# OATML-Markslab/ProteinGym

Measured on AMD Instinct MI355X. Metric: mutants scored/sec (ESM-1v 650M masked-marginal), higher is better.
Workload: dtype f16x3 (fp32 operands split into 2 fp16 planes, 3 fp16 MFMAs per product, fp32 accumulate)

## Files before the change

### proteingym_amd/csrc/api_esm.hip

```cpp
#include "model.h"

namespace pgmi {

int create_esm(pgmi_model* m, const pgmi_config* cfg, const float* w, int64_t n_weights) {
    const size_t D = cfg->embed_dim, F = cfg->ffn_dim, V = cfg->vocab, dh = m->dh, Da = m->Da;
    BlobCursor c(m, w, n_weights);
    c.upload(&m->embed_tokens, V * D);
    if (cfg->arch == PGMI_ARCH_ESM1B) c.upload(&m->embed_positions, (size_t)(cfg->max_positions + 2) * D);
    if (cfg->emb_layer_norm_before) {
        c.upload(&m->lnb_w, D);
        c.upload(&m->lnb_b, D);
    }
    auto slot = [&](size_t col) -> size_t { return rotate_half_slot(col, dh); };
    const float qscale = 1.0f / sqrtf((float)dh);
    m->layers.resize(cfg->layers);
    std::vector<float> wq(3 * Da * D, 0.0f), bq(3 * Da, 0.0f), wo_r(D * Da, 0.0f);
    for (int l = 0; l < cfg->layers; ++l) {
        Layer& L = m->layers[l];
        c.upload(&L.ln1_w, D);
        c.upload(&L.ln1_b, D);
        pack_qkv_slots(c.take(3 * (D * D + D)), D, Da, slot, qscale, wq.data(), bq.data());
        c.linear(&L.wqkv, &L.wqkv16, wq.data(), wq.size(), D);
        c.upload(&L.bqkv, bq.data(), bq.size());
        pack_out_cols(c.take(D * D), D, Da, slot, wo_r.data());
        c.linear(&L.wo, &L.wo16, wo_r.data(), wo_r.size(), Da);
        c.upload(&L.bo, D);
        c.upload(&L.ln2_w, D);
        c.upload(&L.ln2_b, D);
        c.linear(&L.w1, &L.w116, F * D, D);
        c.upload(&L.b1, F);
        c.linear(&L.w2, &L.w216, D * F, F);
        c.upload(&L.b2, D);
    }
    c.upload(&m->lna_w, D);
    c.upload(&m->lna_b, D);
    c.linear(&m->hd_w, &m->hd16, D * D, D);
    c.upload(&m->hd_b, D);
    c.upload(&m->hln_w, D);
    c.upload(&m->hln_b, D);
    c.upload(&m->head_b, V);
    m->head_w = m->embed_tokens;
    return c.finish();
}

int ensure_rotary(pgmi_model* m, int T) {
    if ((m->cfg.arch != PGMI_ARCH_ESM2 && m->cfg.arch != PGMI_ARCH_ESMC) || T <= m->rot_len) return PGMI_OK;
    return upload_rotate_half(m, std::max(T, 1026));
}

int upload_rotate_half(pgmi_model* m, int n) {
    const int rh = m->rot_halves;
    float inv[64];
    const int half = m->dh / 2;
    for (int i = 0; i < half; ++i) inv[i] = 1.0f / powf(10000.0f, (float)(2 * i) / (float)m->dh);
    return upload_rotary(m, n, rh, [&](int t, int g, int i) {
        const int j = (rh == 1) ? i : 32 * g + i;
        return j < half ? (float)t * inv[j] : 0.0f;
    });
}

int run_encoder(pgmi_model* m, int B, int T, const int32_t* keep, int n_keep, bool* compacted) {
    const pgmi_config& c = m->cfg;
    const int M = B * T, D = c.embed_dim, F = c.ffn_dim, N1 = m->fc1_cols, H = c.heads, Da = m->Da;
    hipStream_t s = m->stream;
    if (c.arch == PGMI_ARCH_ESM1B && T > c.max_positions) {
        set_error("Sequence length %d above maximum sequence length of %d", T, c.max_positions);
        return PGMI_EINVAL;
    }
    int rc = ensure_rotary(m, T);
    if (!rc) rc = reset_pad_keys(m, B, T);
    if (rc) return rc;
    {
        ProfScope p(m, PGMI_K_EMBED, 0, (double)M * D * 4);
        launch_seq_stats(m->tokens, B, T, m->embed_gather ? 0 : c.token_dropout, m->denom, m->pos_idx, m->kv_len, s);
        if (m->embed_gather) launch_gather_rows(m->embed_tokens, m->tokens, M, D, m->x, s);
        else launch_embed(m->tokens, m->denom, m->pos_idx, m->embed_tokens, m->embed_positions, c.token_dropout, M, T, D, m->x, s);
        if (m->lnb_w) {
            launch_layernorm(m->x, m->lnb_w, m->lnb_b, M, D, 1e-5f, m->x, s);
            launch_zero_pad_rows(m->tokens, M, D, m->x, s);
        }
    }
    const double ln_bytes = 2.0 * M * D * 4;
    const int prec = c.precision;
    const int mode16 = (prec == PGMI_PREC_F16X3) ? 1 : 2;
    for (int l = 0; l < c.layers; ++l) {
        const Layer& L = m->layers[l];
        { ProfScope p(m, PGMI_K_LAYERNORM, 0, ln_bytes);
          if (prec == PGMI_PREC_FP32) launch_layernorm(m->x, L.ln1_w, L.ln1_b, M, D, 1e-5f, m->h, s);
          else launch_layernorm16(m->x, L.ln1_w, L.ln1_b, M, D, 1e-5f, m->h16, m->h16_plane, mode16, s); }
        const bool fused_qkv = prec != PGMI_PREC_FP32 && !L.q_ln;
        { ProfScope p(m, PGMI_K_GEMM_QKV, 2.0 * M * 3 * D * D, 0);
          if (fused_qkv)
              rc = launch_gemm16_qkv(m->h16, m->h16_plane, L.wqkv16.p, L.wqkv16.plane, L.bqkv, M, Da, D, L.wqkv16.out_scale,
                                     m->qk16, m->qk16_plane, m->vt16, m->vt16_plane, m->rot_cos, m->rot_sin,
                                     c.arch == PGMI_ARCH_ESM2, T, m->Hs, m->gemm_variant, s, m->rot_halves, prec == PGMI_PREC_BF16);
          else
              rc = linear(m, m->h, m->h16, m->h16_plane, L.wqkv, L.wqkv16, L.bqkv, nullptr, m->qkv, nullptr, 0, M, 3 * Da, D, EPI_NONE);
          if (rc) return rc; }
        { ProfScope p(m, PGMI_K_ATTENTION, 4.0 * M * T * D, L.q_ln ? (double)M * D * 20 : 0);
          if (L.q_ln && (rc = launch_qkln_prep(m->qkv, L.q_ln, L.k_ln, 1e-5f, m->rot_cos, m->rot_sin, B, T, H, m->qk16, m->qk16_plane,
                                               m->vt16, m->vt16_plane, s)))
              return rc;
          const bool v2 = prec != PGMI_PREC_FP32;
          if (c.arch == PGMI_ARCH_ESM2 && !v2) launch_rotary(m->qkv, m->rot_cos, m->rot_sin, M, T, m->Hs, s, m->rot_halves);
          if (prec == PGMI_PREC_F16X3)
              rc = launch_attention_f16x3_v2(nullptr, m->kv_len, m->rot_cos, m->rot_sin, c.arch == PGMI_ARCH_ESM2, B, T, H,
                                             m->qk16, m->qk16_plane, m->vt16, m->vt16_plane, nullptr, m->h16,
                                             m->h16_plane, 1, s, nullptr, nullptr, m->rot_halves * kHeadDim);
          else if (v2)
              rc = launch_attention_f16x3_v2(nullptr, m->kv_len, m->rot_cos, m->rot_sin, c.arch == PGMI_ARCH_ESM2, B, T, H,
                                             m->qk16, m->qk16_plane, m->vt16, m->vt16_plane, nullptr, m->h16, m->h16_plane, 2, s, nullptr, nullptr,
                                             m->rot_halves * kHeadDim);
          else
              rc = launch_attention_f32(m->qkv, m->kv_len, B, T, H, m->h, m->h16, m->h16_plane,
                                        prec == PGMI_PREC_FP32 ? 0 : mode16, s, m->rot_halves * kHeadDim);
          if (rc) return rc; }
        if (keep && m->keep_rows && l == c.layers - 1) {
            const int R = n_keep;
            ProfScope p(m, PGMI_K_KEPT_ROWS, 2.0 * R * D * (Da + N1 + F), 0);
            launch_gather_rows(m->x, keep, R, D, m->qkv, s);
            if (prec == PGMI_PREC_FP32) launch_gather_rows(m->h, keep, R, Da, m->g, s);
            else
                launch_gather_rows(reinterpret_cast<const float*>(m->h16), keep, R, prec == PGMI_PREC_F16X3 ? Da : Da / 2,
                                   reinterpret_cast<float*>(m->g16), s);
            rc = linear(m, m->g, m->g16, m->g16_plane, L.wo, L.wo16, L.bo, m->qkv, m->x, nullptr, 0, R, D, Da, EPI_NONE);
            if (rc) return rc;
            if (prec == PGMI_PREC_FP32) launch_layernorm(m->x, L.ln2_w, L.ln2_b, R, D, 1e-5f, m->h, s);
            else launch_layernorm16(m->x, L.ln2_w, L.ln2_b, R, D, 1e-5f, m->h16, m->h16_plane, mode16, s);
            rc = linear(m, m->h, m->h16, m->h16_plane, L.w1, L.w116, L.b1, nullptr,
                        prec == PGMI_PREC_FP32 ? m->g : nullptr, prec == PGMI_PREC_FP32 ? nullptr : m->g16, m->g16_plane,
                        R, N1, D, m->fc1_epi);
            if (rc) return rc;
            rc = linear(m, m->g, m->g16, m->g16_plane, L.w2, L.w216, L.b2, m->x, m->x, nullptr, 0, R, D, F, EPI_NONE);
            if (rc) return rc;
            if (compacted) *compacted = true;
            break;
        }
        { ProfScope p(m, PGMI_K_GEMM_OUT, 2.0 * M * D * D, 0);
          rc = linear(m, m->h, m->h16, m->h16_plane, L.wo, L.wo16, L.bo, m->x, m->x, nullptr, 0, M, D, Da, EPI_NONE);
          if (rc) return rc; }
        { ProfScope p(m, PGMI_K_LAYERNORM, 0, ln_bytes);
          if (prec == PGMI_PREC_FP32) launch_layernorm(m->x, L.ln2_w, L.ln2_b, M, D, 1e-5f, m->h, s);
          else launch_layernorm16(m->x, L.ln2_w, L.ln2_b, M, D, 1e-5f, m->h16, m->h16_plane, mode16, s); }
        { ProfScope p(m, PGMI_K_GEMM_FC1, 2.0 * M * N1 * D, 0);
          rc = linear(m, m->h, m->h16, m->h16_plane, L.w1, L.w116, L.b1, nullptr,
                      prec == PGMI_PREC_FP32 ? m->g : nullptr, prec == PGMI_PREC_FP32 ? nullptr : m->g16, m->g16_plane,
                      M, N1, D, m->fc1_epi);
          if (rc) return rc; }
        { ProfScope p(m, PGMI_K_GEMM_FC2, 2.0 * M * F * D, 0);
          rc = linear(m, m->g, m->g16, m->g16_plane, L.w2, L.w216, L.b2, m->x, m->x, nullptr, 0, M, D, F, EPI_NONE);
          if (rc) return rc; }
    }
    PGMI_HIP(hipGetLastError());
    return PGMI_OK;
}

int run_head(pgmi_model* m, int R, const int32_t* row_idx) {
    const pgmi_config& c = m->cfg;
    const int D = c.embed_dim;
    hipStream_t s = m->stream;
    ProfScope p(m, PGMI_K_HEAD, 2.0 * R * D * (D + c.vocab), 0);
    const int prec = c.precision;
    const float* src = m->x;
    if (row_idx) {
        launch_gather_rows(m->x, row_idx, R, D, m->h, s);
        src = m->h;
    }
    if (prec == PGMI_PREC_FP32) launch_layernorm(src, m->lna_w, m->lna_b, R, D, 1e-5f, m->h, s);
    else launch_layernorm16(src, m->lna_w, m->lna_b, R, D, 1e-5f, m->h16, m->h16_plane, prec == PGMI_PREC_F16X3 ? 1 : 2, s);
    int rc = linear(m, m->h, m->h16, m->h16_plane, m->hd_w, m->hd16, m->hd_b, nullptr, m->g, nullptr, 0, R, D, D, EPI_GELU);
    if (rc) return rc;
    launch_layernorm(m->g, m->hln_w, m->hln_b, R, D, 1e-5f, m->g, s);
    launch_vocab_logsoftmax(m->g, m->head_w, m->head_b, R, D, c.vocab, m->lp, m->nonfinite, s);
    PGMI_HIP(hipGetLastError());
    return PGMI_OK;
}


int run_rows(pgmi_model* m, int B, int T, int R, const int32_t* row_idx) {
    bool compacted = false;
    int rc = run_encoder(m, B, T, row_idx, R, &compacted);
    if (rc) return rc;
    return run_head(m, R, compacted ? nullptr : row_idx);
}

}

extern "C" {

int pgmi_token_logprobs(pgmi_model* m, const int32_t* tokens, int B, int T, float* out) {
    if (!m || !tokens || !out || B <= 0 || T <= 0) { set_error("bad argument"); return PGMI_EINVAL; }
    if (T + 31 > m->max_rows) { set_error("T=%d exceeds workspace rows %d", T, m->max_rows); return PGMI_EINVAL; }
    int rc = check_tokens(tokens, B, T);
    if (rc) return rc;
    PGMI_HIP(hipSetDevice(m->device));
    const int V = m->cfg.vocab;
    rc = for_each_chunk(m, B, T, [&](int b0, int bc) {
        PGMI_HIP(hipMemcpyAsync(m->tokens, tokens + (size_t)b0 * T, (size_t)bc * T * 4, hipMemcpyHostToDevice, m->stream));
        int rc = run_rows(m, bc, T, bc * T, nullptr);
        if (rc) return rc;
        PGMI_HIP(hipMemcpyAsync(out + (size_t)b0 * T * V, m->lp, (size_t)bc * T * V * 4, hipMemcpyDeviceToHost, m->stream));
        return PGMI_OK;
    });
    return rc ? rc : check_nonfinite(m);
}

int pgmi_masked_logprobs(pgmi_model* m, const int32_t* tokens, const int32_t* mask_pos, int B, int T, float* out) {
    if (!m || !tokens || !mask_pos || !out || B <= 0 || T <= 0) { set_error("bad argument"); return PGMI_EINVAL; }
    if (m->cfg.arch == PGMI_ARCH_ESMC && T + 31 > m->max_rows) { set_error("T=%d exceeds workspace rows %d", T, m->max_rows); return PGMI_EINVAL; }
    if (T > m->max_rows) { set_error("T=%d exceeds workspace rows %d", T, m->max_rows); return PGMI_EINVAL; }
    int rc = check_tokens(tokens, B, T);
    if (rc) return rc;
    for (int b = 0; b < B; ++b)
        if (mask_pos[b] < 0 || mask_pos[b] >= T) { set_error("mask_pos[%d]=%d out of range", b, mask_pos[b]); return PGMI_EINVAL; }
    PGMI_HIP(hipSetDevice(m->device));
    const int V = m->cfg.vocab;
    std::vector<int32_t> ridx;
    rc = for_each_chunk(m, B, T, [&](int b0, int bc) {
        ridx.resize(bc);
        for (int b = 0; b < bc; ++b) ridx[b] = b * T + mask_pos[b0 + b];
        PGMI_HIP(hipMemcpyAsync(m->tokens, tokens + (size_t)b0 * T, (size_t)bc * T * 4, hipMemcpyHostToDevice, m->stream));
        PGMI_HIP(hipMemcpyAsync(m->aux_i, mask_pos + b0, (size_t)bc * 4, hipMemcpyHostToDevice, m->stream));
        PGMI_HIP(hipMemcpyAsync(m->row_idx, ridx.data(), (size_t)bc * 4, hipMemcpyHostToDevice, m->stream));
        launch_apply_mask(m->tokens, m->aux_i, bc, T, m->stream);
        int rc = run_rows(m, bc, T, bc, m->row_idx);
        if (rc) return rc;
        PGMI_HIP(hipMemcpyAsync(out + (size_t)b0 * V, m->lp, (size_t)bc * V * 4, hipMemcpyDeviceToHost, m->stream));
        return PGMI_OK;
    });
    return rc ? rc : check_nonfinite(m);
}

int pgmi_assay_create(pgmi_model* m, const int32_t* wt_tokens, int n_tok, const int32_t* positions, int P,
                      int window, const int32_t* sub_pos, const int32_t* sub_wt, const int32_t* sub_mt,
                      const int64_t* mut_off, int64_t n_mut, pgmi_assay** out) {
    if (!out) { set_error("null out"); return PGMI_EINVAL; }
    *out = nullptr;
    if (!m || !wt_tokens || n_tok <= 0 || P < 0 || (P > 0 && !positions) || window <= 0 || n_mut < 0) { set_error("bad argument"); return PGMI_EINVAL; }
    if (m->cfg.arch == PGMI_ARCH_ESMC) { set_error("ESM C assays run through pgmi_masked_logprobs (their window rule is not pgmi_optimal_window)"); return PGMI_EINVAL; }
    for (int i = 0; i < n_tok; ++i)
        if (wt_tokens[i] < 0 || wt_tokens[i] >= PGMI_VOCAB || wt_tokens[i] == PGMI_TOK_PAD) { set_error("wt token %d invalid at %d", wt_tokens[i], i); return PGMI_EINVAL; }
    const int T = std::min(n_tok, window);
    if (T > m->max_rows) { set_error("T=%d exceeds workspace rows %d", T, m->max_rows); return PGMI_EINVAL; }
    std::vector<int32_t> ws(P), mr(P);
    for (int i = 0; i < P; ++i) {
        if (positions[i] < 0 || positions[i] >= n_tok) { set_error("position %d out of range", positions[i]); return PGMI_EINVAL; }
        int s, e;
        pgmi_optimal_window(positions[i], n_tok, window, &s, &e);
        if (e - s != T) { set_error("internal: window length %d != %d", e - s, T); return PGMI_EINVAL; }
        ws[i] = s;
        mr[i] = positions[i] - s;
    }
    const int64_t n_sub = n_mut ? mut_off[n_mut] : 0;
    for (int64_t k = 0; k < n_sub; ++k)
        if (sub_pos[k] < 0 || sub_pos[k] >= n_tok || sub_wt[k] < 0 || sub_wt[k] >= PGMI_VOCAB || sub_mt[k] < 0 || sub_mt[k] >= PGMI_VOCAB) {
            set_error("substitution %lld out of range", (long long)k);
            return PGMI_EINVAL;
        }
    PGMI_HIP(hipSetDevice(m->device));
    pgmi_assay* a = new pgmi_assay();
    a->m = m; a->n_tok = n_tok; a->P = P; a->T = T; a->n_mut = n_mut; a->n_sub = n_sub;
    int rc = dev_upload(a->allocs, &a->wt, wt_tokens, (size_t)n_tok);
    if (!rc) rc = dev_upload(a->allocs, &a->positions, positions, (size_t)P);
    if (!rc) rc = dev_upload(a->allocs, &a->win_start, ws.data(), (size_t)P);
    if (!rc) rc = dev_upload(a->allocs, &a->mask_rel, mr.data(), (size_t)P);
    if (!rc) rc = dev_upload(a->allocs, &a->sub_pos, sub_pos, (size_t)n_sub);
    if (!rc) rc = dev_upload(a->allocs, &a->sub_wt, sub_wt, (size_t)n_sub);
    if (!rc) rc = dev_upload(a->allocs, &a->sub_mt, sub_mt, (size_t)n_sub);
    if (!rc) rc = dev_upload(a->allocs, &a->mut_off, mut_off, (size_t)(n_mut + 1));
    if (!rc) rc = dev_alloc(a->allocs, &a->table, (size_t)n_tok * PGMI_VOCAB);
    if (!rc) rc = dev_alloc(a->allocs, &a->scores, (size_t)n_mut);
    if (rc) { pgmi_assay_destroy(a); return rc; }
    m->assays.push_back(a);
    *out = a;
    return PGMI_OK;
}

void pgmi_assay_destroy(pgmi_assay* a) {
    if (!a) return;
    if (a->m) {
        hipSetDevice(a->m->device);
        hipStreamSynchronize(a->m->stream);
        auto& v = a->m->assays;
        v.erase(std::remove(v.begin(), v.end(), a), v.end());
    }
    for (void* p : a->allocs) hipFree(p);
    delete a;
}

int pgmi_assay_run(pgmi_model* m, pgmi_assay* a, double* scores_host, float* table_host, double* scores_dev) {
    if (!m || !a || a->m != m) { set_error("bad model/assay handle (assay belongs to another or a destroyed model)"); return PGMI_EINVAL; }
    PGMI_HIP(hipSetDevice(m->device));
    hipStream_t s = m->stream;
    const int T = a->T, V = m->cfg.vocab;
    const int per = rows_per_chunk(m, T);
    launch_fill_f32(a->table, (int64_t)a->n_tok * V, NAN, s);
    for (int p0 = 0; p0 < a->P; p0 += per) {
        const int bc = std::min(per, a->P - p0);
        launch_make_masked_windows(a->wt, a->win_start + p0, a->mask_rel + p0, bc, T, m->tokens, s);
        launch_row_index(a->mask_rel + p0, bc, T, m->row_idx, s);
        int rc = run_rows(m, bc, T, bc, m->row_idx);
        if (rc) return rc;
        launch_scatter_rows(m->lp, a->positions + p0, bc, V, a->table, s);
    }
    {
        ProfScope p(m, PGMI_K_SCORE, 0, (double)a->n_sub * 20);
        launch_score_mutants(a->table, V, a->sub_pos, a->sub_wt, a->sub_mt, a->mut_off, a->n_mut, a->scores, s);
    }
    PGMI_HIP(hipGetLastError());
    if (scores_dev && a->n_mut) PGMI_HIP(hipMemcpyAsync(scores_dev, a->scores, (size_t)a->n_mut * 8, hipMemcpyDeviceToDevice, s));
    if (scores_host && a->n_mut) PGMI_HIP(hipMemcpyAsync(scores_host, a->scores, (size_t)a->n_mut * 8, hipMemcpyDeviceToHost, s));
    if (table_host) PGMI_HIP(hipMemcpyAsync(table_host, a->table, (size_t)a->n_tok * V * 4, hipMemcpyDeviceToHost, s));
    PGMI_HIP(hipStreamSynchronize(s));
    return check_nonfinite(m);
}

int pgmi_pppl_create(pgmi_model* m, const uint8_t* tokens, const int64_t* seq_off, int64_t n_seq, pgmi_pppl** out) {
    if (!out) { set_error("null out"); return PGMI_EINVAL; }
    *out = nullptr;
    if (!m || !tokens || !seq_off || n_seq <= 0 || n_seq > 0x7fffffff) { set_error("bad argument"); return PGMI_EINVAL; }
    if (m->cfg.arch != PGMI_ARCH_ESM1B && m->cfg.arch != PGMI_ARCH_ESM2) { set_error("pseudo-ppl needs an ESM-1b/1v/ESM2 model"); return PGMI_EINVAL; }
    if (seq_off[0] != 0) { set_error("seq_off[0] must be 0"); return PGMI_EINVAL; }
    for (int64_t n = 0; n < n_seq; ++n) {
        const int64_t len = seq_off[n + 1] - seq_off[n];
        if (len < 2 || len > (1 << 24)) { set_error("sequence %lld has %lld tokens", (long long)n, (long long)len); return PGMI_EINVAL; }
        const uint8_t* t = tokens + seq_off[n];
        for (int64_t i = 0; i < len; ++i)
            if (t[i] >= PGMI_VOCAB || t[i] == PGMI_TOK_PAD) { set_error("token id %d invalid at sequence %lld, position %lld", (int)t[i], (long long)n, (long long)i); return PGMI_EINVAL; }
    }
    PGMI_HIP(hipSetDevice(m->device));
    pgmi_pppl* q = new pgmi_pppl();
    q->m = m;
    q->N = n_seq;
    q->off.assign(seq_off, seq_off + n_seq + 1);
    int rc = dev_upload(q->allocs, &q->tok8, tokens, (size_t)seq_off[n_seq]);
    if (!rc) rc = dev_upload(q->allocs, &q->off_dev, seq_off, (size_t)n_seq + 1);
    if (rc) { for (void* p : q->allocs) hipFree(p); delete q; return rc; }
    m->pppls.push_back(q);
    *out = q;
    return PGMI_OK;
}

void pgmi_pppl_destroy(pgmi_pppl* q) {
    if (!q) return;
    if (q->m) {
        hipSetDevice(q->m->device);
        hipStreamSynchronize(q->m->stream);
        auto& v = q->m->pppls;
        v.erase(std::remove(v.begin(), v.end(), q), v.end());
    }
    for (void* p : q->allocs) hipFree(p);
    delete q;
}

int64_t pgmi_pppl_rows(const pgmi_pppl* q, int64_t first, int64_t count) {
    if (!q || first < 0 || count < 0 || first + count > q->N) return -1;
    int64_t r = 0;
    for (int64_t n = first; n < first + count; ++n) r += std::max<int64_t>(0, q->off[n + 1] - q->off[n] - 4);
    return r;
}

int pgmi_pppl_run(pgmi_model* m, pgmi_pppl* q, int64_t first, int64_t count, double* scores_host, float* terms_host,
                  double* scores_dev) {
    if (!m || !q || q->m != m) { set_error("bad model/library handle (library belongs to another or a destroyed model)"); return PGMI_EINVAL; }
    if (first < 0 || count <= 0 || first + count > q->N) { set_error("sequence range [%lld, %lld) outside the library of %lld", (long long)first, (long long)(first + count), (long long)q->N); return PGMI_EINVAL; }
    PGMI_HIP(hipSetDevice(m->device));
    hipStream_t s = m->stream;
    const int J = (int)count, V = m->cfg.vocab;
    std::vector<int32_t> sid(J);
    for (int j = 0; j < J; ++j) sid[j] = (int32_t)(first + j);
    auto len_of = [&](int32_t n) { return q->off[n + 1] - q->off[n]; };
    std::stable_sort(sid.begin(), sid.end(), [&](int32_t a, int32_t b) { return len_of(a) > len_of(b); });
    std::vector<int64_t> rp((size_t)J + 1);
    rp[0] = 0;
    for (int j = 0; j < J; ++j) rp[j + 1] = rp[j] + std::max<int64_t>(0, len_of(sid[j]) - 4);
    const int64_t R = rp[J];
    const int64_t Tmax = len_of(sid[0]);
    if (R > 0 && Tmax + 31 > m->max_rows) { set_error("T=%lld exceeds workspace rows %d", (long long)Tmax, m->max_rows); return PGMI_EINVAL; }
    if (R > 0 && m->cfg.arch == PGMI_ARCH_ESM1B && Tmax > m->cfg.max_positions) {
        set_error("Sequence length %lld above maximum sequence length of %d", (long long)Tmax, m->cfg.max_positions);
        return PGMI_EINVAL;
    }
    std::vector<void*> pool;
    auto cleanup = [&]() { for (void* p : pool) hipFree(p); };
    int32_t* d_sid = nullptr;
    int64_t* d_rp = nullptr;
    float* d_terms = nullptr;
    double* d_out = nullptr;
    int rc = dev_upload(pool, &d_sid, sid.data(), (size_t)J);
    if (!rc) rc = dev_upload(pool, &d_rp, rp.data(), (size_t)J + 1);
    if (!rc) rc = dev_alloc(pool, &d_terms, (size_t)R);
    if (!rc) rc = dev_alloc(pool, &d_out, (size_t)J);
    if (rc) { cleanup(); return rc; }
    q->last_rows = R; q->last_chunks = 0; q->last_tokens = 0; q->last_padded = 0;
    int j0 = 0;
    for (int64_t g0 = 0; g0 < R;) {
        while (rp[j0 + 1] <= g0) ++j0;
        const int T = (int)len_of(sid[j0]);
        const int bc = (int)std::min<int64_t>(rows_per_chunk(m, T), R - g0);
        launch_make_pppl_rows(q->tok8, q->off_dev, d_sid, d_rp, J, g0, bc, T, m->tokens, m->row_idx, m->aux_i, s);
        rc = run_rows(m, bc, T, bc, m->row_idx);
        if (rc) { hipStreamSynchronize(s); cleanup(); return rc; }
        launch_pppl_pick(m->lp, m->aux_i, bc, V, d_terms + g0, s);
        q->last_chunks += 1;
        q->last_padded += (int64_t)bc * T;
        g0 += bc;
        if ((q->last_chunks & 63) == 0 && g0 < R && (rc = check_nonfinite(m)) != PGMI_OK) { cleanup(); return rc; }
    }
    for (int j = 0; j < J; ++j) q->last_tokens += (rp[j + 1] - rp[j]) * len_of(sid[j]);
    {
        ProfScope p(m, PGMI_K_SCORE, 0, (double)R * 4);
        launch_pppl_sum(d_terms, d_rp, d_sid, J, first, d_out, s);
    }
    hipError_t e = hipGetLastError();
    if (e == hipSuccess && scores_dev) e = hipMemcpyAsync(scores_dev, d_out, (size_t)J * 8, hipMemcpyDeviceToDevice, s);
    if (e == hipSuccess && scores_host) e = hipMemcpyAsync(scores_host, d_out, (size_t)J * 8, hipMemcpyDeviceToHost, s);
    std::vector<float> sorted_terms;
    if (e == hipSuccess && terms_host && R > 0) {
        sorted_terms.resize((size_t)R);
        e = hipMemcpyAsync(sorted_terms.data(), d_terms, (size_t)R * 4, hipMemcpyDeviceToHost, s);
    }
    if (e == hipSuccess) e = hipStreamSynchronize(s);
    cleanup();
    if (e != hipSuccess) { set_error("pseudo-ppl run failed: %s", hipGetErrorString(e)); return PGMI_EHIP; }
    if (terms_host && R > 0) {
        std::vector<int64_t> dst((size_t)J + 1, 0);
        for (int k = 0; k < J; ++k) dst[k + 1] = dst[k] + std::max<int64_t>(0, len_of((int32_t)(first + k)) - 4);
        for (int j = 0; j < J; ++j)
            std::copy(sorted_terms.begin() + rp[j], sorted_terms.begin() + rp[j + 1], terms_host + dst[sid[j] - first]);
    }
    return check_nonfinite(m);
}

int pgmi_pppl_stats(const pgmi_pppl* q, int64_t* rows, int64_t* chunks, int64_t* tokens, int64_t* padded_tokens) {
    if (!q) { set_error("null library"); return PGMI_EINVAL; }
    if (rows) *rows = q->last_rows;
    if (chunks) *chunks = q->last_chunks;
    if (tokens) *tokens = q->last_tokens;
    if (padded_tokens) *padded_tokens = q->last_padded;
    return PGMI_OK;
}

}
```

### proteingym_amd/csrc/api_model.hip

```cpp
#include "model.h"

namespace pgmi {

static thread_local char g_err[1024] = "";
void set_error(const char* fmt, ...) {
    va_list ap;
    va_start(ap, fmt);
    vsnprintf(g_err, sizeof(g_err), fmt, ap);
    va_end(ap);
}

int prof_drain(pgmi_model* m) {
    if (m->events_used == 0) return PGMI_OK;
    PGMI_HIP(hipStreamSynchronize(m->stream));
    for (size_t i = 0; i < m->events_used; ++i) {
        float ms = 0.f;
        PGMI_HIP(hipEventElapsedTime(&ms, m->events[i].start, m->events[i].stop));
        m->prof_ms[m->events[i].cls] += ms;
    }
    m->events_used = 0;
    return PGMI_OK;
}

int check_cfg(const pgmi_config* c) {
// ... 121 lines not shown
        set_error("non-finite log-probabilities: an activation left the fp16/bf16 range in precision mode %d; "
                  "re-run with precision fp32", m->cfg.precision);
        return PGMI_EOVERFLOW;
    }
    return PGMI_OK;
}

int reset_pad_keys(pgmi_model* m, int B, int T) {
    if (!m->vt16 || (B == m->last_B && T == m->last_T)) return PGMI_OK;
    PGMI_HIP(hipMemsetAsync(m->vt16, 0, m->vt16_plane * 2 * sizeof(unsigned short), m->stream));
    m->last_B = B;
    m->last_T = T;
    return PGMI_OK;
}

}

extern "C" {

int pgmi_abi_version(void) { return PGMI_ABI_VERSION; }

const char* pgmi_last_error(void) { return g_err; }

int pgmi_device_count(void) {
    int n = 0;
    if (hipGetDeviceCount(&n) != hipSuccess) return 0;
    return n;
}

int64_t pgmi_weight_count(const pgmi_config* c) {
    if (!c || c->layers <= 0 || c->embed_dim <= 0 || c->ffn_dim <= 0) return -1;
    const int64_t D = c->embed_dim, F = c->ffn_dim, V = c->vocab;
    if (c->arch == PGMI_ARCH_TRANCEPTION) {
        const int64_t conv = 3 * ((64 * 3 + 64) + (64 * 5 + 64) + (64 * 7 + 64));
        return V * D + (int64_t)c->layers * (2 * D + (D * 3 * D + 3 * D) + conv + (D * D + D) + 2 * D + (D * F + F) + (F * D + D)) + 2 * D + V * D;
    }
    if (c->arch == PGMI_ARCH_PROGEN2)
        return V * D + (int64_t)c->layers * (2 * D + 3 * D * D + D * D + (F * D + F) + (D * F + D)) + 2 * D + V * D + V;
    if (c->arch == PGMI_ARCH_GPT) return -1;
    if (c->arch == PGMI_ARCH_ESMC) return esmc_weight_count(c);
    if (c->arch == PGMI_ARCH_MSA) {
        const int64_t attn = 2 * D + 4 * (D * D + D);
        return V * D + (int64_t)(c->max_positions + 2) * D + 1024 * D + 2 * D +
               (int64_t)c->layers * (2 * attn + 2 * D + (F * D + F) + (D * F + D)) + 2 * D + (D * D + D) + 2 * D + V;
    }
    int64_t n = V * D;
    if (c->arch == PGMI_ARCH_ESM1B) n += (int64_t)(c->max_positions + 2) * D;
    if (c->emb_layer_norm_before) n += 2 * D;
    n += (int64_t)c->layers * (2 * D + 4 * (D * D + D) + 2 * D + (F * D + F) + (D * F + D));
    n += 2 * D + (D * D + D) + 2 * D + V;
    return n;
}

int pgmi_model_create(const pgmi_config* cfg, const float* w, int64_t n_weights, int device, pgmi_model** out) {
    if (cfg && cfg->arch == PGMI_ARCH_PROGEN2) {
        if (out) *out = nullptr;
        set_error("ProGen2 models are created with pgmi_pg2_model_create (it takes rotary_dim)");
        return PGMI_EINVAL;
    }
    if (cfg && cfg->arch == PGMI_ARCH_GPT) {
        if (out) *out = nullptr;
        set_error("causal decoder models are created with pgmi_gpt_model_create (it takes pos_kind)");
        return PGMI_EINVAL;
    }
    return model_create(cfg, w, n_weights, device, out, 0);
}

}

namespace pgmi {

static int alloc_workspace(pgmi_model* m) {
    const pgmi_config& c = m->cfg;
    const size_t R = m->max_rows, D = c.embed_dim, F = c.ffn_dim, V = c.vocab, Da = m->Da;
    const size_t Dw = std::max(D, Da);
    const bool f32mode = c.precision == PGMI_PREC_FP32;
    int rc = PGMI_OK;
    auto alloc = [&](auto** p, size_t n) { if (!rc) rc = dev_alloc(m->allocs, p, n); };
    alloc(&m->x, R * D);
    alloc(&m->h, R * Dw);
    alloc(&m->qkv, R * 3 * Da);
    alloc(&m->g, R * (f32mode ? std::max(F, D) : D));
    if (!f32mode) {
        const size_t planes = c.precision == PGMI_PREC_F16X3 ? 2 : 1;
        m->h16_plane = R * Dw;
        m->g16_plane = R * F;
        alloc(&m->h16, m->h16_plane * planes);
        alloc(&m->g16, m->g16_plane * planes);
    }
    alloc(&m->nonfinite, (size_t)1);
    if (!f32mode) {
        m->qk16_plane = R * 2 * Da;
        m->vt16_plane = R * Da;
        alloc(&m->qk16, m->qk16_plane * 2);
        alloc(&m->vt16, m->vt16_plane * 2);
    }
    if (c.arch == PGMI_ARCH_MSA) {
        alloc(&m->xt, R * D);
        alloc(&m->msa_kv_len, (size_t)2048);
    }
    alloc(&m->lp, (c.arch == PGMI_ARCH_GPT && V > kWave ? (size_t)m->gpt_head_rows : R) * V);
    alloc(&m->denom, R);
    alloc(&m->tokens, R);
    alloc(&m->pos_idx, R);
    alloc(&m->kv_len, R);
    alloc(&m->row_idx, R);
    alloc(&m->aux_i, R);
    if (rc) return rc;
    PGMI_HIP(hipMemset(m->nonfinite, 0, 4));
    if (m->vt16) PGMI_HIP(hipMemset(m->vt16, 0, m->vt16_plane * 2 * sizeof(unsigned short)));
    return PGMI_OK;
}

int model_create(const pgmi_config* cfg, const float* w, int64_t n_weights, int device, pgmi_model** out, int arch_arg) {
    if (!out) { set_error("null out"); return PGMI_EINVAL; }
    *out = nullptr;
    int rc = check_cfg(cfg);
    if (rc) return rc;
    const int64_t need = cfg->arch == PGMI_ARCH_GPT ? gpt_weight_count(cfg, arch_arg) : pgmi_weight_count(cfg);
    if (need < 0) { set_error("causal decoder pos_kind %d: must be PGMI_GPT_POS_ROTARY or PGMI_GPT_POS_LEARNED", arch_arg); return PGMI_EINVAL; }
    if (!w || n_weights != need) {
        set_error("weight blob has %lld elements, config needs %lld", (long long)n_weights, (long long)need);
        return PGMI_EINVAL;
    }
    const int ndev = pgmi_device_count();
    if (ndev <= 0) { set_error("no HIP device visible (libpgmi has no CPU fallback)"); return PGMI_ENODEV; }
    if (device < 0 || device >= ndev) { set_error("device %d out of range (%d visible)", device, ndev); return PGMI_EINVAL; }
    PGMI_HIP(hipSetDevice(device));
    pgmi_model* m = new pgmi_model();
    m->cfg = *cfg;
    m->device = device;
    if (hipStreamCreateWithFlags(&m->stream, hipStreamNonBlocking) != hipSuccess) { set_error("hipStreamCreate failed"); delete m; return PGMI_EHIP; }
    m->dh = cfg->embed_dim / cfg->heads;
    m->rot_halves = m->dh > 2 * kHeadDim ? 4 : m->dh > kHeadDim ? 2 : 1;
    m->Hs = cfg->heads * m->rot_halves;
    m->Da = m->Hs * kHeadDim;
    m->ln_eps = cfg->ln_eps > 0.f ? cfg->ln_eps : 1e-5f;
    m->max_rows = std::max(cfg->max_rows > 0 ? cfg->max_rows : 98304, 2048);
    const size_t V = cfg->vocab;
    const std::vector<float> zeros(std::max({3 * (size_t)m->Da, (V + 63) / 64 * 64, (size_t)cfg->embed_dim, V, (size_t)cfg->heads}), 0.0f);
    rc = dev_upload(m->allocs, &m->zeros, zeros.data(), zeros.size());
    m->fc1_cols = cfg->ffn_dim;
    if (!rc) switch (cfg->arch) {
        case PGMI_ARCH_TRANCEPTION: rc = create_tranception(m, cfg, w, n_weights); break;
        case PGMI_ARCH_MSA: rc = create_msa(m, cfg, w, n_weights); break;
        case PGMI_ARCH_PROGEN2: rc = create_progen2(m, cfg, w, n_weights, arch_arg); break;
        case PGMI_ARCH_GPT: rc = create_gpt(m, cfg, w, n_weights, arch_arg); break;
        case PGMI_ARCH_ESMC: rc = create_esmc(m, cfg, w, n_weights); break;
        default: rc = create_esm(m, cfg, w, n_weights);
    }
    if (!rc) rc = alloc_workspace(m);
    if (rc) { pgmi_model_destroy(m); return rc; }
    m->keep_rows = env_int("PGMI_KEEP_ROWS", 1);
    gemm_options_from_env();
    m->gemm_variant = env_int("PGMI_GEMM_VARIANT", 0);
    *out = m;
    return PGMI_OK;
}

}

extern "C" {

void pgmi_model_destroy(pgmi_model* m) {
    if (!m) return;
    hipSetDevice(m->device);
    if (m->stream) hipStreamSynchronize(m->stream);
    for (pgmi_assay* a : m->assays) {
        for (void* p : a->allocs) hipFree(p);
        a->allocs.clear();
        a->m = nullptr;
    }
    m->assays.clear();
    for (pgmi_pppl* q : m->pppls) {
        for (void* p : q->allocs) hipFree(p);
        q->allocs.clear();
        q->m = nullptr;
    }
    m->pppls.clear();
    for (auto& e : m->events) { hipEventDestroy(e.start); hipEventDestroy(e.stop); }
    for (void* p : m->allocs) hipFree(p);
    if (m->stream) hipStreamDestroy(m->stream);
    delete m;
}

int pgmi_model_device(const pgmi_model* m) { return m ? m->device : -1; }

int pgmi_set_option(const char* name, int64_t value) {
    if (!name) { set_error("null option name"); return PGMI_EINVAL; }
    int rc = gemm_set_option(name, (long long)value);
    if (rc) rc = att_set_option(name, (long long)value);
    if (rc) set_error("unknown option '%s' (gemm_half_tail, gemm_max_rows, att_xcd_local, att_v3)", name);
    return rc;
}

int pgmi_synchronize(pgmi_model* m) {
    if (!m) { set_error("null model"); return PGMI_EINVAL; }
    PGMI_HIP(hipStreamSynchronize(m->stream));
    return PGMI_OK;
}

int pgmi_profile_enable(pgmi_model* m, int on) {
    if (!m) { set_error("null model"); return PGMI_EINVAL; }
    int rc = prof_drain(m);
    m->prof = on != 0;
    return rc;
}

int pgmi_profile_reset(pgmi_model* m) {
    if (!m) { set_error("null model"); return PGMI_EINVAL; }
    int rc = prof_drain(m);
    for (int i = 0; i < PGMI_K_COUNT; ++i) { m->prof_ms[i] = 0; m->prof_n[i] = 0; m->prof_flops[i] = 0; m->prof_bytes[i] = 0; }
    return rc;
}

int pgmi_profile_get(pgmi_model* m, int k, double* ms, int64_t* launches, double* flops, double* bytes) {
    if (!m || k < 0 || k >= PGMI_K_COUNT) { set_error("bad argument"); return PGMI_EINVAL; }
    int rc = prof_drain(m);
    if (rc) return rc;
    if (ms) *ms = m->prof_ms[k];
    if (launches) *launches = m->prof_n[k];
    if (flops) *flops = m->prof_flops[k];
    if (bytes) *bytes = m->prof_bytes[k];
    return PGMI_OK;
}

}
```

### proteingym_amd/csrc/attention_f16.hip

```cpp
#include <stdlib.h>
#include <string.h>
#include <algorithm>

#include "attention_f16_common.h"

namespace pgmi {

template <int WPB, int OUT, int NSTG, int DH = 64, bool RAG = false, int DO = DH>
__global__ __launch_bounds__(WPB * 64) void attention_f16x3_v2_kernel(
    const unsigned short* __restrict__ qk16, size_t qk_plane, const unsigned short* __restrict__ vt16,
    size_t vt_plane, const int32_t* __restrict__ kv_len, const float* __restrict__ slopes, int T, int H,
    int Tp, float* __restrict__ ctx, unsigned short* __restrict__ ctx16, size_t plane, RagMap rag, int dense_nblk, int nseq) {
    constexpr float defer_thr = kAttDefer;
    constexpr int NT = WPB * 64;
    constexpr int KCPR = DH / 8;
    constexpr int KCH = AKT * KCPR, VCH = DO * 4;
    constexpr int NSL = DH / DO;
    static_assert(NSL == 1 || (OUT == 1 && !RAG), "sliced context: split-plane output of dense launches only");
    constexpr int STG_CH = 2 * KCH + 2 * VCH;
    constexpr int NWI = STG_CH / 64;
    constexpr int NDMA = (NWI + WPB - 1) / WPB;
    constexpr int NS = DH / 16, ND = DO / 32;
    extern __shared__ __attribute__((aligned(16))) u32x4 lds[];

// ... 208 lines not shown
            }
            const float mb = m_run - 10.0f;
            typedef float f32x2 __attribute__((ext_vector_type(2)));
#pragma unroll
            for (int v = 0; v < 16; v += 2) {
                const f32x2 dlt = f32x2{st[v], st[v + 1]} - f32x2{mb, mb};
                st[v] = __builtin_amdgcn_exp2f(dlt[0]);
                st[v + 1] = __builtin_amdgcn_exp2f(dlt[1]);
            }
            l_run += ((st[0] + st[1]) + (st[2] + st[3])) + ((st[4] + st[5]) + (st[6] + st[7])) +
                     (((st[8] + st[9]) + (st[10] + st[11])) + ((st[12] + st[13]) + (st[14] + st[15])));
#pragma unroll
            for (int m = 0; m < 2; ++m) {
                u32x4 ph, pl;
#pragma unroll
                for (int e = 0; e < 4; ++e) {
                    const float p0 = st[8 * m + 2 * e], p1 = st[8 * m + 2 * e + 1];
                    typedef __fp16 fp16x2 __attribute__((ext_vector_type(2)));
                    const fp16x2 hi2 = __builtin_amdgcn_cvt_pkrtz(p0, p1);
                    typedef float f32x2 __attribute__((ext_vector_type(2)));
                    const f32x2 ps = f32x2{p0, p1} * f32x2{kLoScale, kLoScale};
                    const float l0 = fmaf((float)hi2[0], -kLoScale, ps[0]), l1 = fmaf((float)hi2[1], -kLoScale, ps[1]);
                    const fp16x2 lo2 = __builtin_amdgcn_cvt_pkrtz(l0, l1);
                    ph[e] = __builtin_bit_cast(unsigned int, hi2);
                    pl[e] = __builtin_bit_cast(unsigned int, lo2);
                }
#pragma unroll
                for (int dt = 0; dt < ND; ++dt) {
                    const int d = dt * 32 + r;
                    const int ci = d * 4 + ((2 * m + kh) ^ ((d >> 2) & 3));
                    const u32x4 vfh = Vb[ci], vfl = Vb[VCH + ci];
                    oc[dt] = mfma_h(vfh, pl, oc[dt]);
                    oc[dt] = mfma_h(vfl, ph, oc[dt]);
                    om[dt] = mfma_h(vfh, ph, om[dt]);
                }
            }
        }
        cur = (cur == NSTG - 1) ? 0 : cur + 1;
    }

    if (active) {
        const float l_tot = l_run + __shfl_xor(l_run, 32);
        if (OUT == 3) {
            store_ctx_bf16<ND>(om, oc, 1.0f / l_tot, kInvLo, q0 + r < T && q0 + r >= p0,
                               ctx16 + (size_t)(orow0 + max(min(q0 + r, T - 1), p0)) * (size_t)D + (size_t)h * DH, kh);
        } else if (OUT == 1) {
            const float inv = 1.0f / l_tot;
            const bool row_ok = q0 + r < T && q0 + r >= p0;
            unsigned short* rowp = ctx16 + (size_t)(orow0 + max(min(q0 + r, T - 1), p0)) * (size_t)(2 * D) + (size_t)((h * DH + d0) / 32) * 64;
#pragma unroll
            for (int dt = 0; dt < ND; ++dt)
#pragma unroll
                for (int gp = 0; gp < 2; ++gp) {
                    unsigned int w[2][4];
#pragma unroll
                    for (int gi = 0; gi < 2; ++gi) {
                        const int g = 2 * gp + gi;
                        _Float16 hh[4], ll[4];
#pragma unroll
                        for (int e = 0; e < 4; ++e) split_act(fmaf(oc[dt][4 * g + e], kInvLo, om[dt][4 * g + e]) * inv, hh[e], ll[e]);
                        w[gi][0] = pack_h2(hh[0], hh[1]); w[gi][1] = pack_h2(hh[2], hh[3]);
                        w[gi][2] = pack_h2(ll[0], ll[1]); w[gi][3] = pack_h2(ll[2], ll[3]);
                    }
                    unsigned int first[4], second[4];
#pragma unroll
                    for (int k = 0; k < 4; ++k) {
                        const auto sw = __builtin_amdgcn_permlane32_swap(w[0][k], w[1][k], false, false);
                        first[k] = sw[0];
                        second[k] = sw[1];
                    }
                    if (row_ok) {
                        unsigned short* dst = rowp + dt * 64 + 8 * (2 * gp + kh);
                        *reinterpret_cast<u32x4*>(dst) = u32x4{first[0], first[1], second[0], second[1]};
                        *reinterpret_cast<u32x4*>(dst + 32) = u32x4{first[2], first[3], second[2], second[3]};
                    }
                }
        } else if (q0 + r < T && q0 + r >= p0) {
            const float inv = 1.0f / l_tot;
            const size_t off = (size_t)(orow0 + q0 + r) * D + (size_t)h * DH + 4 * kh;
#pragma unroll
            for (int dt = 0; dt < ND; ++dt)
#pragma unroll
                for (int g = 0; g < 4; ++g) {
                    float val[4];
#pragma unroll
                    for (int e = 0; e < 4; ++e) val[e] = fmaf(oc[dt][4 * g + e], kInvLo, om[dt][4 * g + e]) * inv;
                    const size_t oo = off + dt * 32 + 8 * g;
                    if constexpr (OUT == 0) {
                        *reinterpret_cast<f32x4*>(ctx + oo) = f32x4{val[0], val[1], val[2], val[3]};
                    } else {
                        _Float16 hh[4], ll[4];
#pragma unroll
                        for (int e = 0; e < 4; ++e) split_act(val[e], hh[e], ll[e]);
                        unsigned short* dst = ctx16 + (size_t)(orow0 + q0 + r) * (size_t)(2 * D) + (size_t)(ND * h + dt) * 64 + 8 * g + 4 * kh;
                        *reinterpret_cast<u32x2*>(dst) = u32x2{pack_h2(hh[0], hh[1]), pack_h2(hh[2], hh[3])};
                        *reinterpret_cast<u32x2*>(dst + 32) = u32x2{pack_h2(ll[0], ll[1]), pack_h2(ll[2], ll[3])};
                    }
                }
        }
    }
}


template <int WPB, int OUT, int NSTG, int DH, bool RAG = false, int DO = DH>
static int launch_att16v2_one(dim3 grid, const unsigned short* qk16, size_t qk_plane, const unsigned short* vt16, size_t vt_plane,
                              const int32_t* kv_len, const float* slopes, int T, int H, int Tp, float* ctx, unsigned short* ctx16,
                              size_t plane, hipStream_t s, RagMap rag = RagMap{}, int dense_nblk = 0, int nseq = 0) {
    constexpr size_t lds_bytes = (size_t)NSTG * (8 * DH + 8 * DO) * 16;
    auto kfn = attention_f16x3_v2_kernel<WPB, OUT, NSTG, DH, RAG, DO>;
    if (lds_bytes > 65536) {
        hipError_t e = hipFuncSetAttribute(reinterpret_cast<const void*>(kfn), hipFuncAttributeMaxDynamicSharedMemorySize, (int)lds_bytes);
        if (e != hipSuccess) { set_error("hipFuncSetAttribute: %s", hipGetErrorString(e)); return PGMI_EHIP; }
    }
    hipLaunchKernelGGL(kfn, grid, dim3(WPB * 64), lds_bytes, s, qk16, qk_plane, vt16, vt_plane, kv_len, slopes, T, H, Tp, ctx, ctx16, plane, rag, dense_nblk, nseq);
    return PGMI_OK;
}

template <int OUT, int NSTG>
static int launch_att16v2_mode(int wpb, dim3 grid, const unsigned short* qk16, size_t qk_plane,
                               const unsigned short* vt16, size_t vt_plane, const int32_t* kv_len,
                               const float* slopes, int T, int H, int Tp, float* ctx, unsigned short* ctx16,
                               size_t plane, hipStream_t s, int dense_nblk, int nseq) {
    const RagMap none{};
    switch (wpb) {
        case 1: return launch_att16v2_one<1, OUT, NSTG, 64>(grid, qk16, qk_plane, vt16, vt_plane, kv_len, slopes, T, H, Tp, ctx, ctx16, plane, s, none, dense_nblk, nseq);
        case 2: return launch_att16v2_one<2, OUT, NSTG, 64>(grid, qk16, qk_plane, vt16, vt_plane, kv_len, slopes, T, H, Tp, ctx, ctx16, plane, s, none, dense_nblk, nseq);
        case 3: return launch_att16v2_one<3, OUT, NSTG, 64>(grid, qk16, qk_plane, vt16, vt_plane, kv_len, slopes, T, H, Tp, ctx, ctx16, plane, s, none, dense_nblk, nseq);
        default: return launch_att16v2_one<4, OUT, NSTG, 64>(grid, qk16, qk_plane, vt16, vt_plane, kv_len, slopes, T, H, Tp, ctx, ctx16, plane, s, none, dense_nblk, nseq);
    }
}

static int g_att_xcd_local = -1;
int att_set_option(const char* name, long long value) {
    if (!strcmp(name, "att_xcd_local")) { g_att_xcd_local = (int)value; return PGMI_OK; }
    if (!strcmp(name, "att_v3")) { att_v3_set_option((int)value); return PGMI_OK; }
    return PGMI_EINVAL;
}
static dim3 dense_grid(int nblk, int H, int B, int* dense_nblk) {
    if (g_att_xcd_local == 0 || (g_att_xcd_local < 0 && nblk < 2)) { *dense_nblk = 0; return dim3(nblk, H, B); }
    *dense_nblk = nblk;
    const long long pairs = (long long)H * B, groups = (pairs + 7) / 8;
    return dim3((unsigned)(groups * 8 * nblk), 1, 1);
}

int att16_waves_per_block(int T) {
    const int n32 = (T + 31) / 32, nblk = (n32 + 3) / 4;
    const int wpb = (n32 + nblk - 1) / nblk;
    return wpb == 3 ? 4 : wpb;
}

int launch_attention_f16x3_v2(const float* qkv, const int32_t* kv_len, const float* cos_t, const float* sin_t,
                              int rotary, int B, int T, int H, unsigned short* qk16, size_t qk_plane,
                              unsigned short* vt16, size_t vt_plane, float* ctx, unsigned short* ctx16, size_t plane,
                              int out_mode, hipStream_t s, const float* conv, const float* slopes, int head_dim) {
    if (B <= 0 || T <= 0 || H <= 0 || out_mode < 0 || out_mode > 2 || (head_dim != 64 && head_dim != 128 && head_dim != 256)) {
        set_error("attention_f16x3_v2: bad arguments B=%d T=%d H=%d out=%d head_dim=%d", B, T, H, out_mode, head_dim);
        return PGMI_EINVAL;
    }
    const int n32 = (T + 31) / 32, Tp = n32 * 32;
    int rc = PGMI_OK;
    {
        const unsigned long long seq_bytes = (unsigned long long)T * 2ull * (unsigned long long)H * (unsigned long long)head_dim * 2ull;
        const unsigned long long vt_bytes = (unsigned long long)head_dim * (unsigned long long)Tp * 2ull;
        if ((unsigned long long)qk_plane * 2ull + seq_bytes >= (1ull << 32) || (unsigned long long)vt_plane * 2ull + vt_bytes >= (1ull << 32)) {
            set_error("attention_f16x3_v2: operand planes of %zu / %zu halfs exceed the 32-bit offset range of the K / V^T DMA "
                      "(plane stride + one sequence must stay below 4 GiB: create the model with a smaller max_rows)", qk_plane, vt_plane);
            return PGMI_EINVAL;
        }
    }
    if (head_dim == 256) {
        if (qkv || conv || !slopes || out_mode != 1) { set_error("attention_f16x3_v2: head_dim 256 is the causal, fused-QKV, split-plane-output flavour only"); return PGMI_EINVAL; }
        const int nblk = (n32 + 3) / 4;
        int dn = 0;
        const dim3 grid = dense_grid(nblk, 2 * H, B, &dn);
        rc = launch_att16v2_one<4, 1, 2, 256, false, 128>(grid, qk16, qk_plane, vt16, vt_plane, kv_len, slopes, T, H, Tp, ctx, ctx16, plane, s, RagMap{}, dn, B);
        if (rc) return rc;
        PGMI_HIP(hipGetLastError());
        return PGMI_OK;
    }
    if (head_dim == 128) {
        if (qkv || conv) { set_error("attention_f16x3_v2: head_dim 128 needs operands from the fused QKV projection"); return PGMI_EINVAL; }
        const int nblk = (n32 + 3) / 4;
        int dn = 0;
        const dim3 grid = dense_grid(nblk, H, B, &dn);
        if (out_mode == 0) rc = launch_att16v2_one<4, 0, 3, 128>(grid, qk16, qk_plane, vt16, vt_plane, kv_len, slopes, T, H, Tp, ctx, ctx16, plane, s, RagMap{}, dn, B);
        else if (out_mode == 2) rc = launch_att16v2_one<4, 3, 3, 128>(grid, qk16, qk_plane, vt16, vt_plane, kv_len, slopes, T, H, Tp, ctx, ctx16, plane, s, RagMap{}, dn, B);
        else rc = launch_att16v2_one<4, 1, 3, 128>(grid, qk16, qk_plane, vt16, vt_plane, kv_len, slopes, T, H, Tp, ctx, ctx16, plane, s, RagMap{}, dn, B);
        if (rc) return rc;
        PGMI_HIP(hipGetLastError());
        return PGMI_OK;
    }
    if (qkv && conv && rotary) { set_error("attention_f16x3_v2: depth-wise convolution and rotary together are not a model this library knows"); return PGMI_EINVAL; }
    if (qkv && conv)
        launch_qkv_prep_conv(dim3(n32, H, B), s, qkv, conv, T, H, Tp, qk16, qk_plane, vt16, vt_plane, nullptr);
    else if (qkv)
        launch_qkv_prep(dim3(n32, H, B), s, qkv, cos_t, sin_t, rotary, T, H, Tp, qk16, qk_plane, vt16, vt_plane);
    const int wpb = att16_waves_per_block(T), nblk = (n32 + wpb - 1) / wpb;
    int dn = 0;
    const dim3 grid = dense_grid(nblk, H, B, &dn);
    if (att_v3_serves(T, conv, slopes, head_dim)) rc = launch_att16v3(out_mode, wpb, grid, qk16, qk_plane, vt16, vt_plane, kv_len, T, H, Tp, ctx, ctx16, s, dn, B);
    else if (out_mode == 0) rc = launch_att16v2_mode<0, 3>(wpb, grid, qk16, qk_plane, vt16, vt_plane, kv_len, slopes, T, H, Tp, ctx, ctx16, plane, s, dn, B);
    else if (out_mode == 2) rc = launch_att16v2_mode<3, 3>(wpb, grid, qk16, qk_plane, vt16, vt_plane, kv_len, slopes, T, H, Tp, ctx, ctx16, plane, s, dn, B);
    else rc = launch_att16v2_mode<1, 3>(wpb, grid, qk16, qk_plane, vt16, vt_plane, kv_len, slopes, T, H, Tp, ctx, ctx16, plane, s, dn, B);
    if (rc) return rc;
    PGMI_HIP(hipGetLastError());
    return PGMI_OK;
}

int launch_attention_tr_ragged(const float* qkv, const float* conv, const float* slopes, int T, int H, const AttRagged& rg,
                               unsigned short* qk16, size_t qk_plane, unsigned short* vt16, size_t vt_plane, unsigned short* ctx16,
                               size_t plane, hipStream_t s) {
    if (T <= 0 || H <= 0 || !qkv || !conv || !slopes || rg.n_tiles <= 0 || rg.n_blocks <= 0) {
        set_error("attention_tr_ragged: bad arguments T=%d H=%d tiles=%d blocks=%d", T, H, rg.n_tiles, rg.n_blocks);
        return PGMI_EINVAL;
    }
    const int Tp = (T + 31) / 32 * 32;
    {
        const unsigned long long seq_bytes = (unsigned long long)T * 2ull * (unsigned long long)H * 64ull * 2ull;
        const unsigned long long vt_bytes = 64ull * (unsigned long long)Tp * 2ull;
        if ((unsigned long long)qk_plane * 2ull + seq_bytes >= (1ull << 32) || (unsigned long long)vt_plane * 2ull + vt_bytes >= (1ull << 32)) {
            set_error("attention_tr_ragged: operand planes exceed the 32-bit offset range of the K / V^T DMA (create the model with a smaller max_rows)");
            return PGMI_EINVAL;
        }
    }
    const RagMap tiles{rg.seq_off, rg.seq_p, rg.seq_q, rg.seq_root, rg.seq_vt, rg.tile_seq, rg.tile_j};
    launch_qkv_prep_conv(dim3(rg.n_tiles, H, 1), s, qkv, conv, T, H, Tp, qk16, qk_plane, vt16, vt_plane, &tiles);
    const RagMap rag{rg.seq_off, rg.seq_p, rg.seq_q, rg.seq_root, rg.seq_vt, rg.blk_seq, rg.blk_j};
    const dim3 grid(rg.n_blocks, H, 1);
    int rc;
    switch (att16_waves_per_block(T)) {
        case 1: rc = launch_att16v2_one<1, 1, 3, 64, true>(grid, qk16, qk_plane, vt16, vt_plane, nullptr, slopes, T, H, Tp, nullptr, ctx16, plane, s, rag); break;
        case 2: rc = launch_att16v2_one<2, 1, 3, 64, true>(grid, qk16, qk_plane, vt16, vt_plane, nullptr, slopes, T, H, Tp, nullptr, ctx16, plane, s, rag); break;
        default: rc = launch_att16v2_one<4, 1, 3, 64, true>(grid, qk16, qk_plane, vt16, vt_plane, nullptr, slopes, T, H, Tp, nullptr, ctx16, plane, s, rag); break;
    }
    if (rc) return rc;
    PGMI_HIP(hipGetLastError());
    return PGMI_OK;
}

}
```

### proteingym_amd/csrc/attention_f16_common.h

```cpp
#pragma once
#include "common.h"

namespace pgmi {

typedef _Float16 h2 __attribute__((ext_vector_type(2)));
typedef _Float16 h8 __attribute__((ext_vector_type(8)));
typedef unsigned int u32x4 __attribute__((ext_vector_type(4)));
typedef unsigned int u32x2 __attribute__((ext_vector_type(2)));

constexpr int AKT = 32;
constexpr float kAttDefer = 4.0f;
constexpr int K_CH = AKT * 8;
constexpr int V_CH = 64 * 4;
constexpr int A_STAGE = 2 * K_CH + 2 * V_CH;

__device__ __forceinline__ unsigned int pack_h2(_Float16 a, _Float16 b) {
    const h2 t = {a, b};
    return __builtin_bit_cast(unsigned int, t);
}
__device__ __forceinline__ f32x16 mfma_h(u32x4 a, u32x4 b, f32x16 c) {
    return __builtin_amdgcn_mfma_f32_32x32x16_f16(__builtin_bit_cast(h8, a), __builtin_bit_cast(h8, b), c, 0, 0, 0);
}


struct RagMap {
    const int32_t* seq_off;
    const int32_t* seq_p;
    const int32_t* seq_q;
    const int32_t* seq_root;
    const uint32_t* seq_vt;
    const int32_t* ent_seq;
    const int32_t* ent_j;
};

template <int ND>
__device__ __forceinline__ void store_ctx_bf16(const f32x16 (&om)[ND], const f32x16 (&oc)[ND], float inv, float inv_lo, bool row_ok,
                                               unsigned short* row_head, int kh) {
    auto rne = [](float f) -> unsigned int {
        unsigned int u = __builtin_bit_cast(unsigned int, f);
        u += 0x7fffu + ((u >> 16) & 1u);
        return u >> 16;
    };
#pragma unroll
    for (int dt = 0; dt < ND; ++dt)
#pragma unroll
        for (int gp = 0; gp < 2; ++gp) {
            unsigned int w[2][2];
#pragma unroll
            for (int gi = 0; gi < 2; ++gi) {
                const int g = 2 * gp + gi;
                float v[4];
#pragma unroll
                for (int e = 0; e < 4; ++e) v[e] = fmaf(oc[dt][4 * g + e], inv_lo, om[dt][4 * g + e]) * inv;
                w[gi][0] = rne(v[0]) | (rne(v[1]) << 16);
                w[gi][1] = rne(v[2]) | (rne(v[3]) << 16);
            }
            unsigned int first[2], second[2];
#pragma unroll
            for (int k = 0; k < 2; ++k) {
                const auto sw = __builtin_amdgcn_permlane32_swap(w[0][k], w[1][k], false, false);
                first[k] = sw[0];
                second[k] = sw[1];
            }
            if (row_ok) *reinterpret_cast<u32x4*>(row_head + dt * 32 + 8 * (2 * gp + kh)) = u32x4{first[0], first[1], second[0], second[1]};
        }
}

void launch_qkv_prep(dim3 grid, hipStream_t s, const float* qkv, const float* cos_t, const float* sin_t, int rotary, int T, int H, int Tp,
                     unsigned short* qk16, size_t qk_plane, unsigned short* vt16, size_t vt_plane);
void launch_qkv_prep_conv(dim3 grid, hipStream_t s, const float* qkv, const float* conv, int T, int H, int Tp, unsigned short* qk16, size_t qk_plane,
                          unsigned short* vt16, size_t vt_plane, const RagMap* rag);
bool att_v3_serves(int T, const float* conv, const float* slopes, int head_dim);
void att_v3_set_option(int value);
int launch_att16v3(int out_mode, int wpb, dim3 grid, const unsigned short* qk16, size_t qk_plane, const unsigned short* vt16, size_t vt_plane,
                   const int32_t* kv_len, int T, int H, int Tp, float* ctx, unsigned short* ctx16, hipStream_t s, int dense_nblk, int nseq);

}
```

### proteingym_amd/csrc/attention_f16_prep.hip

```cpp
#include <stdlib.h>
#include <string.h>
#include <algorithm>

#include "attention_f16_common.h"

namespace pgmi {

__global__ __launch_bounds__(256) void qkv_prep_kernel(
    const float* __restrict__ qkv, const float* __restrict__ cos_t, const float* __restrict__ sin_t,
    int rotary, int T, int H, int Tp, unsigned short* __restrict__ qk16,
    size_t qk_plane, unsigned short* __restrict__ vt16, size_t vt_plane) {
    const int b = blockIdx.z, h = blockIdx.y, t0 = blockIdx.x * 32;
    const int tid = threadIdx.x;
    const int D = H * kHeadDim;
    const size_t RS = (size_t)3 * D;
#pragma unroll
    for (int it = 0; it < 2; ++it) {
        const int u = tid + 256 * it;
        const int which = u >> 8, tok = (u >> 3) & 31, c = u & 7;
        const int t = t0 + tok;
        if (t < T) {
            const float* src = qkv + ((size_t)b * T + t) * RS + (size_t)which * D + h * kHeadDim + 4 * c;
            f32x4 x1 = *reinterpret_cast<const f32x4*>(src);
            f32x4 x2 = *reinterpret_cast<const f32x4*>(src + 32);
// ... 114 lines not shown
                const f32x4 a2 = *reinterpret_cast<const f32x4*>(&raw[(tok + j) * RSTR + which * 64 + 8 * c + 4]);
#pragma unroll
                for (int e = 0; e < 4; ++e) {
                    x1[e] = fmaf(w1[e], a1[e], x1[e]);
                    x2[e] = fmaf(w2[e], a2[e], x2[e]);
                }
            }
            if (which == 0) {
#pragma unroll
                for (int e = 0; e < 4; ++e) { x1[e] *= kQLog2e; x2[e] *= kQLog2e; }
            }
            _Float16 hh[8], ll[8];
#pragma unroll
            for (int e = 0; e < 4; ++e) {
                const float v1 = x1[e], v2 = x2[e];
                split_act(v1, hh[e], ll[e]);
                split_act(v2, hh[4 + e], ll[4 + e]);
            }
            unsigned short* dst = qk16 + orow(t) * (2 * D) + (size_t)which * D + h * kHeadDim + 8 * c;
            *reinterpret_cast<u32x4*>(dst) = u32x4{pack_h2(hh[0], hh[1]), pack_h2(hh[2], hh[3]), pack_h2(hh[4], hh[5]), pack_h2(hh[6], hh[7])};
            *reinterpret_cast<u32x4*>(dst + qk_plane) = u32x4{pack_h2(ll[0], ll[1]), pack_h2(ll[2], ll[3]), pack_h2(ll[4], ll[5]), pack_h2(ll[6], ll[7])};
        }
    }
    {
        const int d = tid & 63, p = tid >> 6;
        const int k1 = 16 * (p >> 1) + 4 * (p & 1);
        _Float16 hh[8], ll[8];
        float w[8];
#pragma unroll
        for (int j = 0; j < 8; ++j) w[j] = cwl[(2 * 8 + j) * 64 + d];
#pragma unroll
        for (int e = 0; e < 8; ++e) {
            const int key = k1 + (e & 3) + 8 * (e >> 2);
            float y = w[7];
#pragma unroll
            for (int j = 0; j < 7; ++j) y = fmaf(w[j], raw[(key + j) * RSTR + 128 + d], y);
            if (t0 + key >= T) y = 0.0f;
            split_act(y, hh[e], ll[e]);
        }
        unsigned short* row = RAG ? vt16 + (size_t)seq_vt[b] + ((size_t)h * kHeadDim + d) * Tpo + (t0 - a0) + 8 * p
                                  : vt16 + (((size_t)b * H + h) * kHeadDim + d) * Tp + t0 + 8 * p;
        *reinterpret_cast<u32x4*>(row) = u32x4{pack_h2(hh[0], hh[1]), pack_h2(hh[2], hh[3]), pack_h2(hh[4], hh[5]), pack_h2(hh[6], hh[7])};
        *reinterpret_cast<u32x4*>(row + vt_plane) = u32x4{pack_h2(ll[0], ll[1]), pack_h2(ll[2], ll[3]), pack_h2(ll[4], ll[5]), pack_h2(ll[6], ll[7])};
    }
}

template <int NV>
__global__ __launch_bounds__(256) void qkln_prep_kernel(
    const float* __restrict__ qkv, const float* __restrict__ q_w, const float* __restrict__ k_w, float eps,
    const float* __restrict__ cos_t, const float* __restrict__ sin_t, int T, int H, int Tp,
    unsigned short* __restrict__ qk16, size_t qk_plane, unsigned short* __restrict__ vt16, size_t vt_plane) {
    const int b = blockIdx.y, t0 = blockIdx.x * 32;
    const int tid = threadIdx.x, lane = tid & 63, wave = tid >> 6;
    const int D = H * kHeadDim, nv = D >> 2;
    const size_t RS = (size_t)3 * D;
    for (int u = wave; u < 64; u += 4) {
        const int which = u & 1, t = t0 + (u >> 1);
        if (t >= T) break;
        const f32x4* xr = reinterpret_cast<const f32x4*>(qkv + ((size_t)b * T + t) * RS + (size_t)which * D);
        f32x4 v[NV];
        float sum = 0.f;
#pragma unroll
        for (int i = 0; i < NV; ++i) {
            const int c = lane + 64 * i;
            v[i] = (c < nv) ? xr[c] : f32x4{0.f, 0.f, 0.f, 0.f};
            sum += (v[i][0] + v[i][1]) + (v[i][2] + v[i][3]);
        }
#pragma unroll
        for (int o = 32; o > 0; o >>= 1) sum += __shfl_xor(sum, o);
        const float mean = sum / (float)D;
        float q = 0.f;
#pragma unroll
        for (int i = 0; i < NV; ++i) {
            const int c = lane + 64 * i;
            if (c < nv) {
#pragma unroll
                for (int k = 0; k < 4; ++k) {
                    const float d = v[i][k] - mean;
                    q += d * d;
                }
            }
        }
#pragma unroll
        for (int o = 32; o > 0; o >>= 1) q += __shfl_xor(q, o);
        const float rstd = 1.0f / sqrtf(q / (float)D + eps);
        const f32x4* wr = reinterpret_cast<const f32x4*>(which ? k_w : q_w);
        const int j4 = 4 * (lane & 15);
        const f32x4 cs = *reinterpret_cast<const f32x4*>(cos_t + (size_t)t * 64 + j4);
        const f32x4 sn = *reinterpret_cast<const f32x4*>(sin_t + (size_t)t * 64 + j4);
        const bool first_half = (lane & 8) == 0;
#pragma unroll
        for (int i = 0; i < NV; ++i) {
            const int c = lane + 64 * i;
            f32x4 o;
            const f32x4 wv = (c < nv) ? wr[c] : f32x4{0.f, 0.f, 0.f, 0.f};
#pragma unroll
            for (int k = 0; k < 4; ++k) o[k] = (v[i][k] - mean) * rstd * wv[k];
            f32x4 p;
#pragma unroll
            for (int k = 0; k < 4; ++k) p[k] = __shfl_xor(o[k], 8);
            if (c < nv) {
                f32x4 y;
#pragma unroll
                for (int k = 0; k < 4; ++k) y[k] = first_half ? o[k] * cs[k] + (-p[k]) * sn[k] : o[k] * cs[k] + p[k] * sn[k];
                if (which == 0) {
#pragma unroll
                    for (int k = 0; k < 4; ++k) y[k] *= kQLog2e;
                }
                _Float16 hh[4], ll[4];
#pragma unroll
                for (int k = 0; k < 4; ++k) split_act(y[k], hh[k], ll[k]);
                unsigned short* dst = qk16 + ((size_t)b * T + t) * (2 * D) + (size_t)which * D + 4 * c;
                *reinterpret_cast<u32x2*>(dst) = u32x2{pack_h2(hh[0], hh[1]), pack_h2(hh[2], hh[3])};
                *reinterpret_cast<u32x2*>(dst + qk_plane) = u32x2{pack_h2(ll[0], ll[1]), pack_h2(ll[2], ll[3])};
            }
        }
    }
    const int d = tid & 63, kq = tid >> 6;
    for (int h = 0; h < H; ++h) {
        _Float16 hh[8], ll[8];
        const float* vsrc = qkv + ((size_t)b * T) * RS + 2 * D + h * kHeadDim + d;
#pragma unroll
        for (int e = 0; e < 8; ++e) {
            const int t = t0 + 8 * kq + e;
            const float x = (t < T) ? vsrc[(size_t)t * RS] : 0.0f;
            split_act(x, hh[e], ll[e]);
        }
        unsigned short* row = vt16 + (((size_t)b * H + h) * kHeadDim + d) * Tp + t0 + 16 * (kq >> 1) + 4 * (kq & 1);
        *reinterpret_cast<u32x2*>(row) = u32x2{pack_h2(hh[0], hh[1]), pack_h2(hh[2], hh[3])};
        *reinterpret_cast<u32x2*>(row + 8) = u32x2{pack_h2(hh[4], hh[5]), pack_h2(hh[6], hh[7])};
        *reinterpret_cast<u32x2*>(row + vt_plane) = u32x2{pack_h2(ll[0], ll[1]), pack_h2(ll[2], ll[3])};
        *reinterpret_cast<u32x2*>(row + vt_plane + 8) = u32x2{pack_h2(ll[4], ll[5]), pack_h2(ll[6], ll[7])};
    }
}

int launch_qkln_prep(const float* qkv, const float* q_w, const float* k_w, float eps, const float* cos_t, const float* sin_t, int B,
                     int T, int H, unsigned short* qk16, size_t qk_plane, unsigned short* vt16, size_t vt_plane, hipStream_t s) {
    const int nv = H * kHeadDim / 4, Tp = (T + 31) / 32 * 32;
    if (B <= 0 || T <= 0 || H <= 0 || nv > 512) { set_error("qkln_prep: bad shape B=%d T=%d H=%d (D = 64 H <= 2048)", B, T, H); return PGMI_EINVAL; }
    const dim3 grid((T + 31) / 32, B);
#define PGMI_QKLN(NV_) hipLaunchKernelGGL(qkln_prep_kernel<NV_>, grid, dim3(256), 0, s, qkv, q_w, k_w, eps, cos_t, sin_t, T, H, Tp, \
                                          qk16, qk_plane, vt16, vt_plane)
    if (nv <= 64) PGMI_QKLN(1);
    else if (nv <= 128) PGMI_QKLN(2);
    else if (nv <= 192) PGMI_QKLN(3);
    else if (nv <= 256) PGMI_QKLN(4);
    else if (nv <= 320) PGMI_QKLN(5);
    else PGMI_QKLN(8);
#undef PGMI_QKLN
    PGMI_HIP(hipGetLastError());
    return PGMI_OK;
}

void launch_qkv_prep(dim3 grid, hipStream_t s, const float* qkv, const float* cos_t, const float* sin_t, int rotary, int T, int H, int Tp,
                     unsigned short* qk16, size_t qk_plane, unsigned short* vt16, size_t vt_plane) {
    hipLaunchKernelGGL(qkv_prep_kernel, grid, dim3(256), 0, s, qkv, cos_t, sin_t, rotary, T, H, Tp, qk16, qk_plane, vt16, vt_plane);
}
void launch_qkv_prep_conv(dim3 grid, hipStream_t s, const float* qkv, const float* conv, int T, int H, int Tp, unsigned short* qk16, size_t qk_plane,
                          unsigned short* vt16, size_t vt_plane, const RagMap* rag) {
    if (rag)
        hipLaunchKernelGGL(qkv_prep_conv_kernel<true>, grid, dim3(256), 0, s, qkv, conv, T, H, Tp, qk16, qk_plane, vt16, vt_plane,
                           rag->seq_off, rag->seq_p, rag->seq_q, rag->seq_root, rag->seq_vt, rag->ent_seq, rag->ent_j);
    else
        hipLaunchKernelGGL(qkv_prep_conv_kernel<false>, grid, dim3(256), 0, s, qkv, conv, T, H, Tp, qk16, qk_plane, vt16, vt_plane,
                           nullptr, nullptr, nullptr, nullptr, nullptr, nullptr, nullptr);
}

}
```

### proteingym_amd/csrc/attention_f16_v3.hip

```cpp
#include <stdlib.h>
#include <string.h>
#include <algorithm>

#include "attention_f16_common.h"

namespace pgmi {

template <int WPB, int OUT>
__global__ __launch_bounds__(WPB * 64, 2) void attention_f16x3_v3_kernel(
    const unsigned short* __restrict__ qk16, size_t qk_plane, const unsigned short* __restrict__ vt16, size_t vt_plane,
    const int32_t* __restrict__ kv_len, int T, int H, int Tp, float* __restrict__ ctx, unsigned short* __restrict__ ctx16,
    int dense_nblk, int nseq) {
    constexpr float defer_thr = kAttDefer;
    constexpr int DH = 64, NSTG = 3, KCPR = 8, KCH = AKT * KCPR, VCH = DH * 4, STG_CH = 2 * KCH + 2 * VCH;
    constexpr int NWI = STG_CH / 64, NDMA = (NWI + WPB - 1) / WPB, NS = 4, ND = 2;
    extern __shared__ __attribute__((aligned(16))) u32x4 lds[];
    int b, h, qblk;
    if (dense_nblk > 0) {
        const int within = (int)blockIdx.x % (8 * dense_nblk);
        const int pair = ((int)blockIdx.x / (8 * dense_nblk)) * 8 + (within & 7);
        if (pair >= nseq * H) return;
        qblk = within >> 3;
        b = pair / H;
        h = pair - b * H;
    } else {
        b = blockIdx.z;
        h = blockIdx.y;
        qblk = blockIdx.x;
    }
    const int tid = threadIdx.x, lane = tid & 63;
    const int wave = __builtin_amdgcn_readfirstlane(tid >> 6);
    const int r = lane & 31, kh = lane >> 5;
    const int D = H * DH;
    const int Tk = kv_len ? kv_len[b] : T;
    const int q0 = (qblk * WPB + wave) * 32;
    const bool active = q0 < T;
    const int nkt = (Tk + AKT - 1) / AKT;
    const size_t seq_halfs = (size_t)T * (2 * D), vt_halfs = (size_t)DH * Tp;
    const unsigned long long qk_bytes = std::min<unsigned long long>(0xFFFFFFFFull, (unsigned long long)qk_plane * 2ull + seq_halfs * 2ull);
    const unsigned long long vt_bytes = std::min<unsigned long long>(0xFFFFFFFFull, (unsigned long long)vt_plane * 2ull + vt_halfs * 2ull);
    const __amdgpu_buffer_rsrc_t rsQK = __builtin_amdgcn_make_buffer_rsrc(const_cast<unsigned short*>(qk16) + (size_t)b * seq_halfs, 0, (int)(unsigned int)qk_bytes, 0x00020000);
    const __amdgpu_buffer_rsrc_t rsVT = __builtin_amdgcn_make_buffer_rsrc(const_cast<unsigned short*>(vt16) + ((size_t)b * H + h) * vt_halfs, 0, (int)(unsigned int)vt_bytes, 0x00020000);

    static_assert(WPB == 1 || WPB == 2 || WPB == 4, "the DMA map needs WPB to divide 8");
    constexpr int NK = 8 / WPB;
    int kvoff[NK], krow[NK], vvoff[NDMA - NK];
#pragma unroll
    for (int i = 0; i < NK; ++i) {
        const int q4 = (wave + WPB * i) & 3;
        const int key = q4 * 8 + (lane >> 3);
        krow[i] = key;
        kvoff[i] = ((lane & 7) ^ ((key >> 1) & 7)) * 16;
    }
#pragma unroll
    for (int i = 0; i < NDMA - NK; ++i) {
        const int q4 = (wave + WPB * (i + NK)) & 3;
        const int g = q4 * 64 + lane, d = g >> 2, c = (g & 3) ^ ((d >> 2) & 3);
        vvoff[i] = d * Tp * 2 + c * 16;
    }
    auto issue_piece = [&](int i, int m, int stage, bool on) {
        u32x4* base = lds + stage * STG_CH;
        const int kk = min(m, nkt - 1), vv = min(max(m - 2, 0), nkt - 1);
        if (i < NK) {
            const int wi = wave + WPB * i, p = (WPB * i) >> 2;
            const int kr = krow[i < NK ? i : 0], ko = kvoff[i < NK ? i : 0];
            const int vo = on ? min(kk * AKT + kr, T - 1) * (2 * D) * 2 + ko : -16;
            const int so = (int)((unsigned int)p * (unsigned int)qk_plane * 2u + (unsigned int)(D + h * DH) * 2u);
            __builtin_amdgcn_raw_ptr_buffer_load_lds(rsQK, (__attribute__((address_space(3))) void*)(base + wi * 64), 16, vo, so, 0, 0);
        } else {
            const int wi = wave + WPB * i, p = (WPB * i - 8) >> 2;
            const int so = (int)((unsigned int)p * (unsigned int)vt_plane * 2u) + vv * ((AKT / 8) * 16);
            const int vv0 = vvoff[i >= NK ? i - NK : 0];
            const int vo = on ? vv0 : -16;
            __builtin_amdgcn_raw_ptr_buffer_load_lds(rsVT, (__attribute__((address_space(3))) void*)(base + wi * 64), 16, vo, so, 0, 0);
        }
    };
    auto issue_bundle = [&](int m, int stage, bool on) {
#pragma unroll
        for (int i = 0; i < NDMA; ++i) issue_piece(i, m, stage, on);
    };
    const int last_bundle = nkt + 1;

    issue_bundle(0, 0, true);
    u32x4 qh[NS], ql[NS];
    {
        u32x4* qbase = lds + STG_CH + wave * (2 * KCH);
        if (active) {
            constexpr int NQ = 2 * KCH / 64;
#pragma unroll
            for (int i = 0; i < NQ; ++i) {
                const int f = i * 64 + lane, pq = f / KCH, row = (f % KCH) / KCPR;
                const int c = (f % KCPR) ^ ((row >> 1) & 7);
                const int vo = (int)(((unsigned int)min(q0 + row, T - 1) * (unsigned int)(2 * D) + (unsigned int)(h * DH)) * 2u + (unsigned int)c * 16u);
                const int so = (int)((unsigned int)pq * (unsigned int)qk_plane * 2u);
                __builtin_amdgcn_raw_ptr_buffer_load_lds(rsQK, (__attribute__((address_space(3))) void*)(qbase + i * 64), 16, vo, so, 0, 0);
            }
        }
        asm volatile("s_waitcnt vmcnt(0)" ::: "memory");
        if (active) {
#pragma unroll
            for (int s = 0; s < NS; ++s) {
                const int ci = r * KCPR + ((2 * s + kh) ^ ((r >> 1) & 7));
                qh[s] = qbase[ci];
                ql[s] = qbase[KCH + ci];
            }
        }
        asm volatile("s_waitcnt lgkmcnt(0)" ::: "memory");
        __builtin_amdgcn_s_barrier();
        asm volatile("" ::: "memory");
    }
    issue_bundle(1, 1, true);
    issue_bundle(2, 2, true);

    f32x16 om[ND], oc[ND], sm, sc;
#pragma unroll
    for (int dt = 0; dt < ND; ++dt)
#pragma unroll
        for (int v = 0; v < 16; ++v) { om[dt][v] = 0.f; oc[dt][v] = 0.f; }
#pragma unroll
    for (int v = 0; v < 16; ++v) { sm[v] = 0.f; sc[v] = 0.f; }
    u32x4 ph[2], pl[2];
#pragma unroll
    for (int m = 0; m < 2; ++m)
#pragma unroll
        for (int e = 0; e < 4; ++e) { ph[m][e] = 0u; pl[m][e] = 0u; }
    float m_run = -INFINITY, l_run = 0.f;
    constexpr float kInvLo = 1.0f / kLoScale;
    const f32x16 zero16 = {0.f, 0.f, 0.f, 0.f, 0.f, 0.f, 0.f, 0.f, 0.f, 0.f, 0.f, 0.f, 0.f, 0.f, 0.f, 0.f};
    typedef float f32x2 __attribute__((ext_vector_type(2)));
    typedef _Float16 h4 __attribute__((ext_vector_type(4)));

    auto vfrag = [&](const u32x4* Vb, int m, u32x4 (&fh)[ND], u32x4 (&fl)[ND]) {
#pragma unroll
        for (int dt = 0; dt < ND; ++dt) {
            const int d = dt * 32 + r;
            const int ci = d * 4 + ((2 * m + kh) ^ ((d >> 2) & 3));
            fh[dt] = Vb[ci];
            fl[dt] = Vb[VCH + ci];
        }
    };
    auto kfrag = [&](const u32x4* Kb, int s, u32x4& kh_, u32x4& kl_) {
        const int ci = r * KCPR + ((2 * s + kh) ^ ((r >> 1) & 7));
        kh_ = Kb[ci];
        kl_ = Kb[KCH + ci];
    };
    auto pv = [&](int m, const u32x4 (&fh)[ND], const u32x4 (&fl)[ND]) {
#pragma unroll
        for (int dt = 0; dt < ND; ++dt) {
            oc[dt] = mfma_h(fh[dt], pl[m], oc[dt]);
            oc[dt] = mfma_h(fl[dt], ph[m], oc[dt]);
            om[dt] = mfma_h(fh[dt], ph[m], om[dt]);
        }
    };
    auto split_p = [&](const float (&st)[16], int m, int e) {
        const float p0 = st[8 * m + 2 * e], p1 = st[8 * m + 2 * e + 1];
        typedef __fp16 fp16x2 __attribute__((ext_vector_type(2)));
        const fp16x2 hi2 = __builtin_amdgcn_cvt_pkrtz(p0, p1);
        const f32x2 ps = f32x2{p0, p1} * f32x2{kLoScale, kLoScale};
        const float l0 = fmaf((float)hi2[0], -kLoScale, ps[0]), l1 = fmaf((float)hi2[1], -kLoScale, ps[1]);
        const fp16x2 lo2 = __builtin_amdgcn_cvt_pkrtz(l0, l1);
        ph[m][e] = __builtin_bit_cast(unsigned int, hi2);
        pl[m][e] = __builtin_bit_cast(unsigned int, lo2);
    };
    bool pend = false;
    float pend_alpha = 1.0f;
    auto apply_pending = [&]() {
        if (pend) {
#pragma unroll
            for (int dt = 0; dt < ND; ++dt)
#pragma unroll
                for (int v = 0; v < 16; ++v) { om[dt][v] *= pend_alpha; oc[dt][v] *= pend_alpha; }
        }
    };
    auto step = [&](auto MKc, int kt, const u32x4* stage, int dma_stage) {
        constexpr bool MK = decltype(MKc)::value;
        apply_pending();
        const u32x4* Kb = stage;
        const u32x4* Vb = stage + 2 * KCH;
        u32x4 va_h[ND], va_l[ND], vb_h[ND], vb_l[ND];
        u32x4 k0h, k0l, k1h, k1l;
        float st[16];
#define PGMI_SLOT() __builtin_amdgcn_sched_barrier(0)
        vfrag(Vb, 0, va_h, va_l);
        vfrag(Vb, 1, vb_h, vb_l);
#pragma unroll
        for (int v = 0; v < 16; ++v) st[v] = fmaf(sc[v], kInvLo, sm[v]);
        if constexpr (MK) {
#pragma unroll
            for (int v = 0; v < 16; ++v) {
// ... 68 lines not shown
        PGMI_SLOT();
        sc = mfma_h(k0h, ql[0], zero16);
        split_p(st, 0, 3);
        PGMI_SLOT();
        sc = mfma_h(k0l, qh[0], sc);
        split_p(st, 1, 0);
        PGMI_SLOT();
        sm = mfma_h(k0h, qh[0], zero16);
        kfrag(Kb, 2, k0h, k0l);
        split_p(st, 1, 1);
        PGMI_SLOT();
        sc = mfma_h(k1h, ql[1], sc);
        split_p(st, 1, 2);
        PGMI_SLOT();
        sc = mfma_h(k1l, qh[1], sc);
        split_p(st, 1, 3);
        PGMI_SLOT();
        sm = mfma_h(k1h, qh[1], sm);
        kfrag(Kb, 3, k1h, k1l);
        PGMI_SLOT();
        const bool dma_on = kt + 3 <= last_bundle;
        auto dma_slot = [&](int j) {
#pragma unroll
            for (int i = j; i < NDMA; i += 6) issue_piece(i, kt + 3, dma_stage, dma_on);
        };
        sc = mfma_h(k0h, ql[2], sc);
        dma_slot(0);
        PGMI_SLOT();
        sc = mfma_h(k0l, qh[2], sc);
        dma_slot(1);
        PGMI_SLOT();
        sm = mfma_h(k0h, qh[2], sm);
        dma_slot(2);
        PGMI_SLOT();
        sc = mfma_h(k1h, ql[3], sc);
        dma_slot(3);
        PGMI_SLOT();
        sc = mfma_h(k1l, qh[3], sc);
        dma_slot(4);
        PGMI_SLOT();
        sm = mfma_h(k1h, qh[3], sm);
        dma_slot(5);
#undef PGMI_SLOT
    };
    auto closing_pv = [&](const u32x4* stage) {
        apply_pending();
        const u32x4* Vb = stage + 2 * KCH;
        u32x4 va_h[ND], va_l[ND], vb_h[ND], vb_l[ND];
        vfrag(Vb, 0, va_h, va_l);
        vfrag(Vb, 1, vb_h, vb_l);
        pv(0, va_h, va_l);
        pv(1, vb_h, vb_l);
    };
    using T1 = std::integral_constant<bool, true>;
    using T0 = std::integral_constant<bool, false>;

    if (active && nkt > 0) {
#pragma unroll
        for (int s = 0; s < NS; ++s) {
            const int ci = r * KCPR + ((2 * s + kh) ^ ((r >> 1) & 7));
            const u32x4 kfh = lds[ci], kfl = lds[KCH + ci];
            sc = mfma_h(kfh, ql[s], s == 0 ? zero16 : sc);
            sc = mfma_h(kfl, qh[s], sc);
            sm = mfma_h(kfh, qh[s], s == 0 ? zero16 : sm);
        }
    }
    auto wait_bundle = [&](int younger) {
        if (younger >= 1) asm volatile("s_waitcnt vmcnt(%0)" ::"n"(NDMA) : "memory");
        else asm volatile("s_waitcnt vmcnt(0)" ::: "memory");
    };
    int cur = 1;
    auto step_head = [&](int kt) {
        wait_bundle(1);
        __builtin_amdgcn_s_barrier();
        asm volatile("" ::: "memory");
    };
    auto idle_dma = [&](int kt) {
        issue_bundle(kt + 3, cur == 0 ? NSTG - 1 : cur - 1, kt + 3 <= last_bundle);
    };
    for (int kt = 0; kt < nkt - 1; ++kt) {
        step_head(kt);
        if (active) step(T0{}, kt, lds + cur * STG_CH, cur == 0 ? NSTG - 1 : cur - 1);
        else idle_dma(kt);
        cur = (cur == NSTG - 1) ? 0 : cur + 1;
    }
    step_head(nkt - 1);
    if (active) step(T1{}, nkt - 1, lds + cur * STG_CH, cur == 0 ? NSTG - 1 : cur - 1);
    else idle_dma(nkt - 1);
    cur = (cur == NSTG - 1) ? 0 : cur + 1;
    asm volatile("s_waitcnt vmcnt(0)" ::: "memory");
    __builtin_amdgcn_s_barrier();
    asm volatile("" ::: "memory");
    if (active) closing_pv(lds + cur * STG_CH);

    if (active) {
        const float l_tot = l_run + __shfl_xor(l_run, 32);
        const float inv = 1.0f / l_tot;
        if (OUT == 3) {
            store_ctx_bf16<ND>(om, oc, inv, kInvLo, q0 + r < T, ctx16 + (size_t)(b * T + min(q0 + r, T - 1)) * (size_t)D + (size_t)h * DH, kh);
        } else if (OUT == 1) {
            const bool row_ok = q0 + r < T;
            unsigned short* rowp = ctx16 + (size_t)(b * T + min(q0 + r, T - 1)) * (size_t)(2 * D) + (size_t)(ND * h) * 64;
#pragma unroll
            for (int dt = 0; dt < ND; ++dt)
#pragma unroll
                for (int gp = 0; gp < 2; ++gp) {
                    unsigned int w[2][4];
#pragma unroll
                    for (int gi = 0; gi < 2; ++gi) {
                        const int g = 2 * gp + gi;
                        _Float16 hh[4], ll[4];
#pragma unroll
                        for (int e = 0; e < 4; ++e) split_act(fmaf(oc[dt][4 * g + e], kInvLo, om[dt][4 * g + e]) * inv, hh[e], ll[e]);
                        w[gi][0] = pack_h2(hh[0], hh[1]); w[gi][1] = pack_h2(hh[2], hh[3]);
                        w[gi][2] = pack_h2(ll[0], ll[1]); w[gi][3] = pack_h2(ll[2], ll[3]);
                    }
                    unsigned int first[4], second[4];
#pragma unroll
                    for (int k = 0; k < 4; ++k) {
                        const auto sw = __builtin_amdgcn_permlane32_swap(w[0][k], w[1][k], false, false);
                        first[k] = sw[0];
                        second[k] = sw[1];
                    }
                    if (row_ok) {
                        unsigned short* dst = rowp + dt * 64 + 8 * (2 * gp + kh);
                        *reinterpret_cast<u32x4*>(dst) = u32x4{first[0], first[1], second[0], second[1]};
                        *reinterpret_cast<u32x4*>(dst + 32) = u32x4{first[2], first[3], second[2], second[3]};
                    }
                }
        } else if (q0 + r < T) {
            const size_t off = (size_t)(b * T + q0 + r) * D + (size_t)h * DH + 4 * kh;
#pragma unroll
            for (int dt = 0; dt < ND; ++dt)
#pragma unroll
                for (int g = 0; g < 4; ++g) {
                    float val[4];
#pragma unroll
                    for (int e = 0; e < 4; ++e) val[e] = fmaf(oc[dt][4 * g + e], kInvLo, om[dt][4 * g + e]) * inv;
                    *reinterpret_cast<f32x4*>(ctx + off + dt * 32 + 8 * g) = f32x4{val[0], val[1], val[2], val[3]};
                }
        }
    }
}

static int g_att_v3 = -1;
void att_v3_set_option(int value) { g_att_v3 = value; }
bool att_v3_serves(int T, const float* conv, const float* slopes, int head_dim) {
    if (g_att_v3 == 0 || conv || slopes || head_dim != 64) return false;
    return g_att_v3 > 0 || (T + 31) / 32 >= 7;
}

template <int WPB, int OUT>
static void launch_att16v3_one(dim3 grid, const unsigned short* qk16, size_t qk_plane, const unsigned short* vt16, size_t vt_plane, const int32_t* kv_len,
                               int T, int H, int Tp, float* ctx, unsigned short* ctx16, hipStream_t s, int dense_nblk, int nseq) {
    constexpr size_t lds_bytes = (size_t)3 * A_STAGE * 16;
    auto kfn = attention_f16x3_v3_kernel<WPB, OUT>;
    if (lds_bytes > 65536) (void)hipFuncSetAttribute(reinterpret_cast<const void*>(kfn), hipFuncAttributeMaxDynamicSharedMemorySize, (int)lds_bytes);
    hipLaunchKernelGGL((attention_f16x3_v3_kernel<WPB, OUT>), grid, dim3(WPB * 64), lds_bytes, s, qk16, qk_plane, vt16, vt_plane, kv_len, T, H, Tp, ctx, ctx16,
                       dense_nblk, nseq);
}
int launch_att16v3(int out_mode, int wpb, dim3 grid, const unsigned short* qk16, size_t qk_plane, const unsigned short* vt16, size_t vt_plane,
                          const int32_t* kv_len, int T, int H, int Tp, float* ctx, unsigned short* ctx16, hipStream_t s, int dense_nblk, int nseq) {
#define PGMI_V3(W)                                                                                                                          \
    do {                                                                                                                                    \
        if (out_mode == 2) launch_att16v3_one<W, 3>(grid, qk16, qk_plane, vt16, vt_plane, kv_len, T, H, Tp, ctx, ctx16, s, dense_nblk, nseq); \
        else if (out_mode) launch_att16v3_one<W, 1>(grid, qk16, qk_plane, vt16, vt_plane, kv_len, T, H, Tp, ctx, ctx16, s, dense_nblk, nseq);   \
        else launch_att16v3_one<W, 0>(grid, qk16, qk_plane, vt16, vt_plane, kv_len, T, H, Tp, ctx, ctx16, s, dense_nblk, nseq);            \
    } while (0)
    switch (wpb) {
        case 1: PGMI_V3(1); break;
        case 2: PGMI_V3(2); break;
        default: PGMI_V3(4); break;
    }
#undef PGMI_V3
    return PGMI_OK;
}

}
```

### proteingym_amd/csrc/common.h

```cpp
#pragma once
#include <hip/hip_runtime.h>
#include <stdint.h>
#include <stddef.h>

#include "../../include/pgmi.h"

namespace pgmi {

void set_error(const char* fmt, ...);

#define PGMI_HIP(expr)                                                                   \
    do {                                                                                 \
        hipError_t _e = (expr);                                                          \
        if (_e != hipSuccess) {                                                          \
            pgmi::set_error("%s failed: %s (%s:%d)", #expr, hipGetErrorString(_e),       \
                            __FILE__, __LINE__);                                         \
            return PGMI_EHIP;                                                            \
        }                                                                                \
    } while (0)

typedef float f32x4 __attribute__((ext_vector_type(4)));
typedef float f32x16 __attribute__((ext_vector_type(16)));

constexpr int kWave = 64;
constexpr int kHeadDim = 64;

enum Epilogue { EPI_NONE = 0, EPI_GELU = 1, EPI_SQRELU = 2, EPI_GELU_TANH = 3,
                EPI_SWIGLU = 4 };

constexpr float kLoScale = 2048.0f;
constexpr float kQLog2e = 1.4426950408889634f;

__host__ __device__ __forceinline__ size_t ki_off(size_t row, int k, int K) {
    return row * (size_t)(2 * K) + (size_t)(k >> 5) * 64 + (size_t)(k & 31);
}
#if defined(__HIPCC__)
__device__ __forceinline__ void split_act(float x, _Float16& hi, _Float16& lo) {
    hi = (fabsf(x) < 6.103515625e-05f) ? (_Float16)0.0f : (_Float16)x;
    lo = (_Float16)((x - (float)hi) * kLoScale);
}
#endif

void launch_make_masked_windows(const int32_t* wt, const int32_t* win_start, const int32_t* mask_rel,
                                int B, int T, int32_t* tokens_out, hipStream_t s);
void launch_apply_mask(int32_t* tokens, const int32_t* mask_pos, int B, int T, hipStream_t s);
void launch_seq_stats(const int32_t* tokens, int B, int T, int token_dropout, float* scale,
                      int32_t* pos_idx, int32_t* kv_len, hipStream_t s);
void launch_zero_pad_rows(const int32_t* tokens, int rows, int D, float* x, hipStream_t s);
void launch_embed(const int32_t* tokens, const float* scale, const int32_t* pos_idx,
                  const float* embed_tokens, const float* embed_positions, int token_dropout,
                  int rows, int T, int D, float* x, hipStream_t s);
void launch_layernorm(const float* x, const float* w, const float* b, int rows, int D, float eps,
                      float* y, hipStream_t s);
void launch_gather_rows(const float* x, const int32_t* row_idx, int n, int D, float* y, hipStream_t s);
void launch_strided_index(int first, int stride, int n, int32_t* idx, hipStream_t s);
void launch_vocab_logsoftmax(const float* h, const float* E, const float* bias, int rows, int D,
                             int V, float* out, int32_t* nonfinite, hipStream_t s);
void launch_layernorm16(const float* x, const float* w, const float* b, int rows, int D, float eps,
                        unsigned short* y16, size_t plane, int mode, hipStream_t s);
void launch_scatter_rows(const float* src, const int32_t* dst_row, int n, int V, float* table,
                         hipStream_t s);
void launch_row_index(const int32_t* mask_rel, int B, int T, int32_t* out, hipStream_t s);
void launch_fill_f32(float* p, int64_t n, float v, hipStream_t s);
void launch_seq_loglik(const float* lp, const int32_t* tokens, const int32_t* lens, int B, int T, int V,
                       const float* prior, const int32_t* a0, const int32_t* row0, const int32_t* n,
                       const int32_t* flip, float alpha, float* out, hipStream_t s);
void launch_seq_loglik_ragged(const float* lp, const int32_t* tokens, const int32_t* seq_off, const int32_t* seq_p,
                              const int32_t* seq_root, int B, int T, int V, const float* prior, const int32_t* a0,
                              const int32_t* row0, const int32_t* n, const int32_t* flip, float alpha, float* out, hipStream_t s);
void launch_pg2_seq_loglik(const float* lp, const int32_t* col, const int32_t* n_kept, int B, int T, int V, float* out, hipStream_t s);
void launch_embed_learned(const int32_t* tokens, const float* E, const float* P, int rows, int T, int D, float* x, hipStream_t s);
void launch_wide_logsoftmax(const float* logits, int ldl, int rows, int V, const int32_t* tgt, float* out, int32_t* nonfinite,
                            hipStream_t s);
void launch_seq_sum(const float* terms, const int32_t* off, int B, double* out, hipStream_t s);
void launch_score_mutants(const float* table, int V, const int32_t* sub_pos, const int32_t* sub_wt,
                          const int32_t* sub_mt, const int64_t* mut_off, int64_t n_mut,
                          double* scores, hipStream_t s);
void launch_rotary(float* qkv, const float* cos_t, const float* sin_t, int rows, int T, int H,
                   hipStream_t s, int rot_halves = 1);
void launch_make_pppl_rows(const uint8_t* tok8, const int64_t* seq_off, const int32_t* sid, const int64_t* rp, int J,
                           int64_t g0, int bc, int T, int32_t* tokens, int32_t* row_idx, int32_t* target, hipStream_t s);
void launch_pppl_pick(const float* lp, const int32_t* target, int bc, int V, float* terms, hipStream_t s);
void launch_pppl_sum(const float* terms, const int64_t* rp, const int32_t* sid, int J, int64_t first, double* out, hipStream_t s);

void launch_msa_window_tokens(const int32_t* full, int R, int Tfull, int start, int Tw, int mask_col, int32_t* out, hipStream_t s);
void launch_add_row_embedding(float* x, const float* pe, int R, int C, int D, hipStream_t s);
void launch_permute_rows(const float* src, float* dst, int A, int B, int D, hipStream_t s);
void launch_tied_prep_qk(const float* qkv, int64_t M, int D, unsigned short* q16, unsigned short* k16, hipStream_t s);
void launch_pack_vt16(const float* qkv, int R, int C, int Kp, int H, unsigned short* Vt, hipStream_t s);
int launch_tied_softmax16(const float* part, int H, int S, int C, int Kp, float scale, unsigned short* P, hipStream_t s);
float tied_w_scale();

int launch_gemm_f32(const float* A, const float* W, const float* bias, const float* residual,
                    float* C, int M, int N, int K, int epilogue, hipStream_t s);

void gemm_options_from_env();
int gemm_set_option(const char* name, long long value);
int launch_gemm16(const unsigned short* A, size_t a_plane, const unsigned short* W, size_t w_plane,
                  const float* bias, const float* residual, float* Cf, unsigned short* Ch, size_t c_plane,
                  int M, int N, int K, int epilogue, float out_scale, int planes, bool bf, int variant,
                  hipStream_t s);
int launch_gemm16_qkv(const unsigned short* A, size_t a_plane, const unsigned short* W, size_t w_plane,
                      const float* bias, int M, int D, int K, float out_scale, unsigned short* qk16, size_t qk_plane,
                      unsigned short* vt16, size_t vt_plane, const float* cos_t, const float* sin_t, int rotary,
                      int T, int H, int variant, hipStream_t s, int rot_halves = 1, bool bf = false);
struct XMap;
int launch_gemm16_ex(const unsigned short* A, const unsigned short* W, float* Cf, unsigned short* Ch, int M, int N, int K,
                     float out_scale, XMap xm, int nbatch, hipStream_t s);
void launch_split16(const float* x, int64_t n, float scale, int mode, int K, unsigned short* out, hipStream_t s);

int launch_qkln_prep(const float* qkv, const float* q_w, const float* k_w, float eps, const float* cos_t, const float* sin_t, int B,
                     int T, int H, unsigned short* qk16, size_t qk_plane, unsigned short* vt16, size_t vt_plane, hipStream_t s);

int launch_attention_f32(const float* qkv, const int32_t* kv_len, int B, int T, int H, float* ctx,
                         unsigned short* ctx16, size_t plane, int out_mode, hipStream_t s, int head_dim = 64);

int launch_attention_f16x3_v2(const float* qkv, const int32_t* kv_len, const float* cos_t, const float* sin_t,
                              int rotary, int B, int T, int H, unsigned short* qk16, size_t qk_plane,
                              unsigned short* vt16, size_t vt_plane, float* ctx, unsigned short* ctx16, size_t plane,
                              int out_mode, hipStream_t s, const float* conv = nullptr, const float* slopes = nullptr,
                              int head_dim = 64);

struct AttRagged {
    const int32_t* seq_off;
    const int32_t* seq_p;
    const int32_t* seq_q;
    const int32_t* seq_root;
    const uint32_t* seq_vt;
    const int32_t* tile_seq;
    const int32_t* tile_j;
    const int32_t* blk_seq;
    const int32_t* blk_j;
    int n_tiles, n_blocks;
};
int att16_waves_per_block(int T);
int att_set_option(const char* name, long long value);
int launch_attention_tr_ragged(const float* qkv, const float* conv, const float* slopes, int T, int H, const AttRagged& rg,
                               unsigned short* qk16, size_t qk_plane, unsigned short* vt16, size_t vt_plane, unsigned short* ctx16,
                               size_t plane, hipStream_t s);

}
```

### proteingym_amd/csrc/elementwise.hip

```cpp
#include "common.h"

namespace pgmi {

__device__ __forceinline__ float wave_sum(float v) {
#pragma unroll
    for (int o = 32; o > 0; o >>= 1) v += __shfl_xor(v, o);
    return v;
}
__device__ __forceinline__ float wave_max(float v) {
#pragma unroll
    for (int o = 32; o > 0; o >>= 1) v = fmaxf(v, __shfl_xor(v, o));
    return v;
}
__device__ __forceinline__ double wave_sum_d(double v) {
#pragma unroll
    for (int o = 32; o > 0; o >>= 1) v += __shfl_xor(v, o);
    return v;
}
__device__ __forceinline__ int wave_sum_i(int v) {
#pragma unroll
    for (int o = 32; o > 0; o >>= 1) v += __shfl_xor(v, o);
    return v;
}

__global__ void make_masked_windows_kernel(const int32_t* __restrict__ wt,
                                           const int32_t* __restrict__ win_start,
                                           const int32_t* __restrict__ mask_rel, int B, int T,
                                           int32_t* __restrict__ out) {
    const int64_t i = (int64_t)blockIdx.x * blockDim.x + threadIdx.x;
    if (i >= (int64_t)B * T) return;
    const int b = (int)(i / T), t = (int)(i % T);
    out[i] = (t == mask_rel[b]) ? PGMI_TOK_MASK : wt[win_start[b] + t];
}
void launch_make_masked_windows(const int32_t* wt, const int32_t* win_start, const int32_t* mask_rel,
                                int B, int T, int32_t* out, hipStream_t s) {
    const int64_t n = (int64_t)B * T;
    hipLaunchKernelGGL(make_masked_windows_kernel, dim3((unsigned)((n + 255) / 256)), dim3(256), 0, s,
                       wt, win_start, mask_rel, B, T, out);
}

__global__ void apply_mask_kernel(int32_t* tokens, const int32_t* __restrict__ mask_pos, int B, int T) {
    const int b = blockIdx.x * blockDim.x + threadIdx.x;
    if (b < B) tokens[(int64_t)b * T + mask_pos[b]] = PGMI_TOK_MASK;
}
void launch_apply_mask(int32_t* tokens, const int32_t* mask_pos, int B, int T, hipStream_t s) {
    hipLaunchKernelGGL(apply_mask_kernel, dim3((B + 255) / 256), dim3(256), 0, s, tokens, mask_pos, B, T);
}

__global__ void seq_stats_kernel(const int32_t* __restrict__ tokens, int B, int T, int token_dropout,
                                 float* __restrict__ denom, int32_t* __restrict__ pos_idx,
                                 int32_t* __restrict__ kv_len) {
    const int b = blockIdx.x * (blockDim.x >> 6) + (threadIdx.x >> 6);
    const int lane = threadIdx.x & 63;
    if (b >= B) return;
    const int32_t* tk = tokens + (int64_t)b * T;
    int running = 0, n_mask = 0, last_valid = -1;
    for (int t0 = 0; t0 < T; t0 += 64) {
        const int t = t0 + lane;
        const int tok = (t < T) ? tk[t] : PGMI_TOK_PAD;
        const int valid = (t < T) && (tok != PGMI_TOK_PAD);
        const unsigned long long bal = __ballot(valid);
        const unsigned long long below = bal & ((lane == 63) ? ~0ull : ((1ull << (lane + 1)) - 1ull));
        const int incl = __popcll(below);
        if (t < T) pos_idx[(int64_t)b * T + t] = valid ? (running + incl + PGMI_TOK_PAD) : PGMI_TOK_PAD;
        running += __popcll(bal);
        n_mask += __popcll(__ballot((t < T) && tok == PGMI_TOK_MASK));
        if (bal) last_valid = t0 + 63 - __clzll(bal);
    }
    if (lane == 0) {
        float d = 1.0f;
        if (token_dropout) d = 1.0f - (float)n_mask / (float)running;
        denom[b] = d;
        kv_len[b] = last_valid + 1;
    }
}
void launch_seq_stats(const int32_t* tokens, int B, int T, int token_dropout, float* denom,
                      int32_t* pos_idx, int32_t* kv_len, hipStream_t s) {
    hipLaunchKernelGGL(seq_stats_kernel, dim3((B + 3) / 4), dim3(256), 0, s, tokens, B, T, token_dropout,
                       denom, pos_idx, kv_len);
}

__global__ void embed_kernel(const int32_t* __restrict__ tokens, const float* __restrict__ denom,
                             const int32_t* __restrict__ pos_idx, const float* __restrict__ E,
                             const float* __restrict__ P, int token_dropout, int rows, int T, int D,
                             float* __restrict__ x) {
    const int row = blockIdx.x * (blockDim.x >> 6) + (threadIdx.x >> 6);
    const int lane = threadIdx.x & 63;
    if (row >= rows) return;
    const int tok = tokens[row];
    const int b = row / T;
    const float dn = denom[b];
    const f32x4* e = reinterpret_cast<const f32x4*>(E + (size_t)tok * D);
    const f32x4* p = P ? reinterpret_cast<const f32x4*>(P + (size_t)pos_idx[row] * D) : nullptr;
    f32x4* xo = reinterpret_cast<f32x4*>(x + (size_t)row * D);
    const bool is_pad = tok == PGMI_TOK_PAD;
    const bool zero_emb = token_dropout && tok == PGMI_TOK_MASK;
    for (int i = lane; i < D / 4; i += 64) {
        f32x4 v = zero_emb ? f32x4{0.f, 0.f, 0.f, 0.f} : e[i];
        if (token_dropout) {
#pragma unroll
            for (int c = 0; c < 4; ++c) v[c] = (v[c] * 0.88f) / dn;
        }
        if (p) {
            const f32x4 pv = p[i];
#pragma unroll
            for (int c = 0; c < 4; ++c) v[c] += pv[c];
        }
        if (is_pad) v = f32x4{0.f, 0.f, 0.f, 0.f};
        xo[i] = v;
    }
}
void launch_embed(const int32_t* tokens, const float* denom, const int32_t* pos_idx, const float* E,
                  const float* P, int token_dropout, int rows, int T, int D, float* x, hipStream_t s) {
    hipLaunchKernelGGL(embed_kernel, dim3((rows + 3) / 4), dim3(256), 0, s, tokens, denom, pos_idx, E, P,
                       token_dropout, rows, T, D, x);
}

__global__ void zero_pad_rows_kernel(const int32_t* __restrict__ tokens, int rows, int D, float* __restrict__ x) {
    const int row = blockIdx.x * 4 + (threadIdx.x >> 6);
    const int lane = threadIdx.x & 63;
    if (row >= rows || tokens[row] != PGMI_TOK_PAD) return;
    for (int i = lane; i < D; i += 64) x[(size_t)row * D + i] = 0.f;
}
void launch_zero_pad_rows(const int32_t* tokens, int rows, int D, float* x, hipStream_t s) {
    hipLaunchKernelGGL(zero_pad_rows_kernel, dim3((rows + 3) / 4), dim3(256), 0, s, tokens, rows, D, x);
}

template <int NV, int OUTMODE>
__global__ __launch_bounds__(256) void layernorm_kernel(const float* x,
                                                        const float* __restrict__ w,
                                                        const float* __restrict__ bsh, int rows, int D,
                                                        float eps, float* y, unsigned short* y16,
                                                        size_t plane) {
    const int row = blockIdx.x * 4 + (threadIdx.x >> 6);
    const int lane = threadIdx.x & 63;
    if (row >= rows) return;
    const int nv = D >> 2;
    const f32x4* xr = reinterpret_cast<const f32x4*>(x + (size_t)row * D);
    f32x4 v[NV];
    float s = 0.f;
#pragma unroll
    for (int i = 0; i < NV; ++i) {
        const int c = lane + 64 * i;
        v[i] = (c < nv) ? xr[c] : f32x4{0.f, 0.f, 0.f, 0.f};
        s += (v[i][0] + v[i][1]) + (v[i][2] + v[i][3]);
    }
    const float mean = wave_sum(s) / (float)D;
    float q = 0.f;
#pragma unroll
    for (int i = 0; i < NV; ++i) {
        const int c = lane + 64 * i;
        if (c < nv) {
#pragma unroll
            for (int k = 0; k < 4; ++k) {
                const float d = v[i][k] - mean;
                q += d * d;
            }
        }
    }
    const float rstd = 1.0f / sqrtf(wave_sum(q) / (float)D + eps);
    const f32x4* wr = reinterpret_cast<const f32x4*>(w);
    const f32x4* br = reinterpret_cast<const f32x4*>(bsh);
#pragma unroll
    for (int i = 0; i < NV; ++i) {
        const int c = lane + 64 * i;
        if (c < nv) {
            const f32x4 wv = wr[c], bv = br[c];
            f32x4 o;
#pragma unroll
            for (int k = 0; k < 4; ++k) o[k] = (v[i][k] - mean) * rstd * wv[k] + bv[k];
            if constexpr (OUTMODE == 0) {
                reinterpret_cast<f32x4*>(y + (size_t)row * D)[c] = o;
            } else if constexpr (OUTMODE == 1) {
                typedef _Float16 h4 __attribute__((ext_vector_type(4)));
                h4 hi, lo;
#pragma unroll
                for (int k = 0; k < 4; ++k) {
                    _Float16 a, b2;
                    split_act(o[k], a, b2);
                    hi[k] = a;
                    lo[k] = b2;
                }
                typedef unsigned int u32x2 __attribute__((ext_vector_type(2)));
                typedef unsigned int u32x4 __attribute__((ext_vector_type(4)));
                const u32x2 H = __builtin_bit_cast(u32x2, hi), L = __builtin_bit_cast(u32x2, lo);
                const bool odd = lane & 1;
                const unsigned int s0 = odd ? H[0] : L[0], s1 = odd ? H[1] : L[1];
                const unsigned int r0 = __shfl_xor(s0, 1), r1 = __shfl_xor(s1, 1);
                const u32x4 out = odd ? u32x4{r0, r1, L[0], L[1]} : u32x4{H[0], H[1], r0, r1};
                unsigned short* dst = y16 + ki_off((size_t)row, 4 * (c & ~1), D) + (odd ? 32 : 0);
                *reinterpret_cast<u32x4*>(dst) = out;
// ... 395 lines not shown
```

### proteingym_amd/csrc/gemm16x_kernel.h

```cpp
#pragma once
#include <type_traits>

#include "common.h"

namespace pgmi {

typedef _Float16 h8 __attribute__((ext_vector_type(8)));
typedef _Float16 h4 __attribute__((ext_vector_type(4)));
typedef __bf16 b8 __attribute__((ext_vector_type(8)));
typedef unsigned int u32x4 __attribute__((ext_vector_type(4)));
typedef unsigned int u32x2 __attribute__((ext_vector_type(2)));

__device__ __forceinline__ f32x4 gelu_erf16(f32x4 x) {
    auto all = [](float v) { return f32x4{v, v, v, v}; };
    const f32x4 b = __builtin_elementwise_max(-__builtin_elementwise_abs(x), all(-6.0f));
    f32x4 q = __builtin_elementwise_fma(x, all(0.0f), all(3.309269596e-05f));
    q = __builtin_elementwise_fma(q, b, all(7.692188374e-04f));
    q = __builtin_elementwise_fma(q, b, all(8.080714382e-03f));
    q = __builtin_elementwise_fma(q, b, all(5.341210216e-02f));
    q = __builtin_elementwise_fma(q, b, all(-4.587709904e-01f));
    q = __builtin_elementwise_fma(q, b, all(1.151201725e+00f));
    q = __builtin_elementwise_fma(q, b, all(-9.999930859e-01f));
    const f32x4 e = {__builtin_amdgcn_exp2f(q[0]), __builtin_amdgcn_exp2f(q[1]), __builtin_amdgcn_exp2f(q[2]), __builtin_amdgcn_exp2f(q[3])};
    return __builtin_elementwise_fma(b, e, __builtin_elementwise_max(x, all(0.0f)));
}

__device__ __forceinline__ f32x4 gelu_tanh16(f32x4 x) {
    constexpr float c = -2.0f * 0.7978845608028654f * 1.4426950408889634f;
    f32x4 r;
#pragma unroll
    for (int e = 0; e < 4; ++e) {
        const float u = fmaf(0.044715f * x[e], x[e] * x[e], x[e]);
        r[e] = x[e] / (1.0f + __builtin_amdgcn_exp2f(c * u));
    }
    return r;
}

__device__ __forceinline__ f32x4 silu16(f32x4 x) {
    constexpr float c = -1.4426950408889634f;
    f32x4 r;
#pragma unroll
    for (int e = 0; e < 4; ++e) r[e] = x[e] / (1.0f + __builtin_amdgcn_exp2f(c * x[e]));
    return r;
}

struct QkvOut {
    unsigned short* vt16;
    size_t vt_plane;
    const float* cos_t;
    const float* sin_t;
    int T, H, Tp, rotary;
    int rot_halves;
};

template <bool BF>
__device__ __forceinline__ f32x16 mfma16(u32x4 a, u32x4 b, f32x16 c) {
    if constexpr (BF) {
        return __builtin_amdgcn_mfma_f32_32x32x16_bf16(__builtin_bit_cast(b8, a), __builtin_bit_cast(b8, b), c, 0, 0, 0);
    } else {
        return __builtin_amdgcn_mfma_f32_32x32x16_f16(__builtin_bit_cast(h8, a), __builtin_bit_cast(h8, b), c, 0, 0, 0);
    }
}

template <bool BF>
__device__ __forceinline__ f32x4 mfma16x16(u32x4 a, u32x4 b, f32x4 c) {
    if constexpr (BF) {
        return __builtin_amdgcn_mfma_f32_16x16x32_bf16(__builtin_bit_cast(b8, a), __builtin_bit_cast(b8, b), c, 0, 0, 0);
    } else {
        return __builtin_amdgcn_mfma_f32_16x16x32_f16(__builtin_bit_cast(h8, a), __builtin_bit_cast(h8, b), c, 0, 0, 0);
    }
}

template <typename T>
__device__ __forceinline__ void lds_put(unsigned char* p, T v) {
    *(__attribute__((address_space(3))) T*)(p) = v;
}

__device__ __forceinline__ unsigned short f32_to_bf16_rne(float f) {
    unsigned int u = __builtin_bit_cast(unsigned int, f);
    u += 0x7fffu + ((u >> 16) & 1u);
    return (unsigned short)(u >> 16);
}

struct TilePlan {
    int tiles_m, tiles_n;
    int n_main;
    int n_tail;
    int half;
    int group_m;
};

struct XMap {
    unsigned int a_row_bytes, w_row_bytes;
    unsigned int a_bytes, w_bytes;
    int k_run_log2;
    unsigned int a_run_bytes, w_run_bytes;
    int tiles_per_batch, batch_inner;
    unsigned int a_b0, a_b1, w_b0, w_b1;
    long long c_b0, c_b1;
    int ldc;
    int o_ld;
    int o_rows_per_n64;
    int o_col_per_batch;
};

constexpr int XBM = 256, XBN = 256, XNT = 512, XCPR = 8;
constexpr int X_OP_CH = XBM * XCPR;
constexpr int X_STAGE = 2 * X_OP_CH;
constexpr int X_PATCH_BYTES = 72 * 1024;
constexpr size_t X_LDS_BYTES = (size_t)(X_STAGE * 16 + X_PATCH_BYTES);

__device__ __forceinline__ void x_tile_coords(int wgid, int tiles_m, int tiles_n, int& tm, int& tn, int GROUP_M) {
    const int width = GROUP_M * tiles_n;
    const int group = wgid / width, first_m = group * GROUP_M;
    const int gsz = min(tiles_m - first_m, GROUP_M);
    tm = first_m + (wgid % width) % gsz;
    tn = (wgid % width) / gsz;
}

template <int EPI, int OUT, bool XM = false, bool BF = false>
__global__ __launch_bounds__(XNT, 2) void gemm16x_kernel(
    const unsigned short* __restrict__ A, const unsigned short* __restrict__ W, const float* __restrict__ bias,
    const float* residual, float* Cf, unsigned short* Ch, size_t c_plane, int M, int N, int K, float out_scale,
    TilePlan tp, QkvOut qo, XMap xm_arg) {
    static_assert(!(XM && BF), "the batched / strided form is f16x3 only");
    constexpr unsigned int EB = BF ? 2u : 4u;
    const XMap xm = XM ? xm_arg : XMap{};
    constexpr int WN = 4, TMX = 8, TN = 4, LD = 4;
    extern __shared__ __attribute__((aligned(16))) u32x4 lds[];
    const int tid = threadIdx.x, lane = tid & 63;
    const int wave = __builtin_amdgcn_readfirstlane(tid >> 6);
    const int wm = wave / WN, wn = wave % WN;
    const int r = lane & 15, kq = lane >> 4;
    const bool late = wave >= 4;
    unsigned char* const patches = reinterpret_cast<unsigned char*>(lds + X_STAGE);

    const int row_lo = tid >> 3, c8 = tid & 7, sw8 = (row_lo >> 1) & 7;
    const int csrc = c8 ^ sw8;
    const unsigned int a_row_bytes = xm.a_row_bytes ? xm.a_row_bytes : (unsigned int)K * EB;
    const unsigned int w_row_bytes = xm.w_row_bytes ? xm.w_row_bytes : (unsigned int)K * EB;
    const __amdgpu_buffer_rsrc_t rsA = __builtin_amdgcn_make_buffer_rsrc(const_cast<unsigned short*>(A), 0, (int)(xm.a_bytes ? xm.a_bytes : (unsigned int)M * (unsigned int)K * EB), 0x00020000);
    const __amdgpu_buffer_rsrc_t rsW = __builtin_amdgcn_make_buffer_rsrc(const_cast<unsigned short*>(W), 0, (int)(xm.w_bytes ? xm.w_bytes : (unsigned int)N * (unsigned int)K * EB), 0x00020000);
    unsigned int a_off[LD], w_off[LD];
    int m0 = 0, n0 = 0, a_ld = LD, batch = 0;
    unsigned int a_base = 0, w_base = 0;
    bool half_item = false;
    const int nk = BF ? K / 64 : K / 32;
    const int n_items = tp.n_main + tp.n_tail;
    auto decode = [&](int item) {
        const bool all_half = tp.half == 2;
        int wgid;
        if (item < tp.n_main || all_half) {
            const int nwg = all_half ? n_items : tp.n_main, xcd = item & 7, q = nwg >> 3, r8 = nwg & 7;
            wgid = (xcd < r8 ? xcd * (q + 1) : r8 * (q + 1) + (xcd - r8) * q) + (item >> 3);
        } else {
            wgid = tp.n_main + ((item - tp.n_main) >> 1);
        }
        batch = 0;
        if (xm.tiles_per_batch) {
            batch = wgid / xm.tiles_per_batch;
            wgid -= batch * xm.tiles_per_batch;
            const int bi = batch % xm.batch_inner, bo = batch / xm.batch_inner;
            a_base = __builtin_amdgcn_readfirstlane((unsigned int)bi * xm.a_b0 + (unsigned int)bo * xm.a_b1);
            w_base = __builtin_amdgcn_readfirstlane((unsigned int)bi * xm.w_b0 + (unsigned int)bo * xm.w_b1);
            batch = __builtin_amdgcn_readfirstlane(batch);
        }
        int tm, tn;
        x_tile_coords(wgid, tp.tiles_m, tp.tiles_n, tm, tn, tp.group_m);
        half_item = all_half || (tp.half && item >= tp.n_main);
        a_ld = half_item ? LD / 2 : LD;
        m0 = __builtin_amdgcn_readfirstlane(all_half ? tm * (XBM / 2) : tm * XBM + (half_item ? ((item - tp.n_main) & 1) * (XBM / 2) : 0));
        n0 = __builtin_amdgcn_readfirstlane(tn * XBN);
#pragma unroll
        for (int i = 0; i < LD; ++i) {
            a_off[i] = (unsigned int)min(m0 + row_lo + 64 * i, M - 1) * a_row_bytes + (unsigned int)csrc * 16u;
            w_off[i] = (unsigned int)min(n0 + row_lo + 64 * i, N - 1) * w_row_bytes + (unsigned int)csrc * 16u;
        }
    };
    auto issue_tile = [&](int kt, int buf) {
        u32x4* base = lds + buf * X_STAGE + wave * 64;
        const int run = kt >> xm.k_run_log2, in_run = kt - (run << xm.k_run_log2);
        const int ka = (int)(a_base + (xm.a_run_bytes ? (unsigned int)run * xm.a_run_bytes + (unsigned int)in_run * 128u : (unsigned int)kt * 128u));
        const int kw = (int)(w_base + (xm.w_run_bytes ? (unsigned int)run * xm.w_run_bytes + (unsigned int)in_run * 128u : (unsigned int)kt * 128u));
#pragma unroll
        for (int i = 0; i < LD; ++i)
            if (i < a_ld)
                __builtin_amdgcn_raw_ptr_buffer_load_lds(rsA, (__attribute__((address_space(3))) void*)(base + XNT * i), 16, (int)a_off[i], ka, 0, 0);
#pragma unroll
        for (int i = 0; i < LD; ++i)
            __builtin_amdgcn_raw_ptr_buffer_load_lds(rsW, (__attribute__((address_space(3))) void*)(base + X_OP_CH + XNT * i), 16, (int)w_off[i], kw, 0, 0);
    };
    auto phase = [&]() {
        __builtin_amdgcn_sched_barrier(0);
        __builtin_amdgcn_s_waitcnt(0xC07F);
        __builtin_amdgcn_s_barrier();
        __builtin_amdgcn_sched_barrier(0);
    };
    auto phase_vm = [&]() {
        __builtin_amdgcn_sched_barrier(0);
        __builtin_amdgcn_s_waitcnt(0x0070);
        __builtin_amdgcn_s_barrier();
        __builtin_amdgcn_sched_barrier(0);
    };

    f32x4 acc[TN][TMX];
    u32x4 af[2][TMX / 2], wf[2][TN], whs[TN];
    const int fsw = (r >> 1) & 7;
    auto read_frags = [&](auto tmc, auto hc, const u32x4* Ab, const u32x4* Wb) {
        constexpr int TM = decltype(tmc)::value, TH = TM / 2, H = decltype(hc)::value;
#pragma unroll
        for (int p = 0; p < 2; ++p) {
            const int c = (p * 4 + kq) ^ fsw;
#pragma unroll
            for (int i = 0; i < TH; ++i) af[p][i] = Ab[((wm * TM + H * TH + i) * 16 + r) * XCPR + c];
            if constexpr (H == 0)
#pragma unroll
                for (int j = 0; j < TN; ++j) wf[p][j] = Wb[((wn * TN + j) * 16 + r) * XCPR + c];
        }
    };
    auto scale_whi = [&]() {
        typedef _Float16 h2 __attribute__((ext_vector_type(2)));
        const h2 sc = {(_Float16)(1.0f / kLoScale), (_Float16)(1.0f / kLoScale)};
#pragma unroll
        for (int j = 0; j < TN; ++j)
#pragma unroll
            for (int e = 0; e < 4; ++e) {
                const unsigned int u = wf[0][j][e];
                const h2 t = __builtin_bit_cast(h2, u) * sc;
                whs[j][e] = __builtin_bit_cast(unsigned int, t);
            }
    };
    auto mfmas = [&](auto tmc, auto hc) {
        constexpr int TM = decltype(tmc)::value, TH = TM / 2, H = decltype(hc)::value;
        if constexpr (BF) {
#pragma unroll
            for (int p = 0; p < 2; ++p)
#pragma unroll
                for (int j = 0; j < TN; ++j)
#pragma unroll
                    for (int i = 0; i < TH; ++i) acc[j][H * TH + i] = mfma16x16<true>(wf[p][j], af[p][i], acc[j][H * TH + i]);
            return;
        }
        if constexpr (H == 0) scale_whi();
#pragma unroll
        for (int j = 0; j < TN; ++j)
#pragma unroll
            for (int i = 0; i < TH; ++i) acc[j][H * TH + i] = mfma16x16<false>(wf[1][j], af[0][i], acc[j][H * TH + i]);
#pragma unroll
        for (int j = 0; j < TN; ++j)
#pragma unroll
            for (int i = 0; i < TH; ++i) acc[j][H * TH + i] = mfma16x16<false>(whs[j], af[1][i], acc[j][H * TH + i]);
#pragma unroll
        for (int j = 0; j < TN; ++j)
#pragma unroll
            for (int i = 0; i < TH; ++i) acc[j][H * TH + i] = mfma16x16<false>(wf[0][j], af[0][i], acc[j][H * TH + i]);
        if constexpr (H == 0) {
#pragma unroll
            for (int k = 0; k < 4 * TN; ++k) {
                __builtin_amdgcn_sched_group_barrier(0x008, 1, 0);
                __builtin_amdgcn_sched_group_barrier(0x002, 1, 0);
            }
            __builtin_amdgcn_sched_group_barrier(0x008, 3 * TN * TH - 4 * TN, 0);
        }
    };
    using H0 = std::integral_constant<int, 0>;
    using H1 = std::integral_constant<int, 1>;

    int item = blockIdx.x;
    if (item >= n_items) return;
    decode(item);
    issue_tile(0, 0);
    auto run_item = [&](auto tmc) -> bool {
        constexpr int TM = decltype(tmc)::value;
        phase_vm();
#pragma unroll
        for (int j = 0; j < TN; ++j)
#pragma unroll
            for (int i = 0; i < TM; ++i)
#pragma unroll
                for (int v = 0; v < 4; ++v) acc[j][i][v] = 0.0f;
        int cur = 0;
        if (late) phase();
        for (int kt = 0; kt < nk; ++kt) {
            const u32x4* Ab = lds + cur * X_STAGE;
            const u32x4* Wb = Ab + X_OP_CH;
            __builtin_amdgcn_s_setprio(0);
            if (kt + 1 < nk) issue_tile(kt + 1, cur ^ 1);
            read_frags(tmc, H0{}, Ab, Wb);
            phase();
            __builtin_amdgcn_s_setprio(1);
            mfmas(tmc, H0{});
            phase();
            __builtin_amdgcn_s_setprio(0);
            read_frags(tmc, H1{}, Ab, Wb);
            if (late) phase_vm(); else phase();
            __builtin_amdgcn_s_setprio(1);
            mfmas(tmc, H1{});
            if (!late) phase_vm(); else phase();
            cur ^= 1;
        }
        __builtin_amdgcn_s_setprio(0);
        if (!late) phase();

        const int em0 = m0, en0 = n0, eb = batch;
        item += gridDim.x;
        const bool more = item < n_items;
        if (more) {
            decode(item);
            issue_tile(0, 0);
        }

        if constexpr (OUT == 2) {
            const int Dm = N / 3;
            const int nb = en0 + wn * 64;
            if (nb < N) {
            const int which = nb / Dm, hcol = nb - which * Dm, hh = hcol >> 6;
            constexpr int SPQ = 144;
            unsigned char* patch_q = patches + wave * (2 * 32 * SPQ);
            const bool staged_q = which < 2;
            f32x4 bq0[2], bq1[2];
#pragma unroll
            for (int g = 0; g < 2; ++g) {
                bq0[g] = *reinterpret_cast<const f32x4*>(bias + nb + 16 * g + 4 * kq);
                bq1[g] = *reinterpret_cast<const f32x4*>(bias + nb + 32 + 16 * g + 4 * kq);
            }
#pragma unroll
            for (int g = 0; g < 2; ++g) asm volatile("" :: "v"(bq0[g]), "v"(bq1[g]));
#pragma unroll
            for (int ib = 0; ib < TM / 2; ++ib) {
#pragma unroll
            for (int s = 0; s < 2; ++s) {
                const int i = 2 * ib + s, prow = 16 * s + r;
                const int m = em0 + (wm * TM + i) * 16 + r;
                const bool row_ok = m < M;
                if (!row_ok) continue;
                const int bb = m / qo.T, t = m - bb * qo.T;
                f32x4 rc[2], rs[2];
                if (which < 2 && qo.rotary) {
                    const int tr = (min(t, qo.T - 1) * qo.rot_halves + (hh % qo.rot_halves)) * 64;
#pragma unroll
                    for (int g = 0; g < 2; ++g) {
                        rc[g] = *reinterpret_cast<const f32x4*>(qo.cos_t + tr + 16 * g + 4 * kq);
                        rs[g] = *reinterpret_cast<const f32x4*>(qo.sin_t + tr + 16 * g + 4 * kq);
                    }
                }
#pragma unroll
                for (int g = 0; g < 2; ++g) {
                    const int d0 = 16 * g + 4 * kq;
                    const f32x4 b0 = bq0[g], b1 = bq1[g];
                    float x0[4], x1[4];
#pragma unroll
                    for (int e = 0; e < 4; ++e) {
                        x0[e] = fmaf(acc[g][i][e], out_scale, b0[e]);
                        x1[e] = fmaf(acc[g + 2][i][e], out_scale, b1[e]);
                    }
                    if (which == 0) {
#pragma unroll
                        for (int e = 0; e < 4; ++e) { x0[e] *= kQLog2e; x1[e] *= kQLog2e; }
                    }
                    if (which < 2) {
                        if (qo.rotary) {
                            const f32x4 c1 = rc[g], s1 = rs[g], c2 = rc[g], s2 = rs[g];
#pragma unroll
                            for (int e = 0; e < 4; ++e) {
                                const float y0 = fmaf(x0[e], c1[e], (-x1[e]) * s1[e]);
                                const float y1 = fmaf(x1[e], c2[e], x0[e] * s2[e]);
                                x0[e] = y0;
                                x1[e] = y1;
                            }
                        }
                        h4 hi0, lo0, hi1, lo1;
#pragma unroll
                        for (int e = 0; e < 4; ++e) {
                            _Float16 a, b2;
                            split_act(x0[e], a, b2); hi0[e] = a; lo0[e] = b2;
                            split_act(x1[e], a, b2); hi1[e] = a; lo1[e] = b2;
                        }
                        unsigned char* cell = patch_q + prow * SPQ + d0 * 2;
                        lds_put(cell, hi0);
                        lds_put(cell + 32 * SPQ, lo0);
                        lds_put(cell + 64, hi1);
                        lds_put(cell + 32 * SPQ + 64, lo1);
                    } else {
                        const int tk = t & 31;
                        const int pos = (t & ~31) + ((tk & 0x13) | ((tk & 4) << 1) | ((tk & 8) >> 1));
                        unsigned short* col = qo.vt16 + (((size_t)bb * qo.H + hh) * kHeadDim + d0) * qo.Tp + pos;
#pragma unroll
                        for (int e = 0; e < 4; ++e) {
                            _Float16 a0, l0, a1, l1;
                            split_act(x0[e], a0, l0);
                            split_act(x1[e], a1, l1);
                            unsigned short* c0 = col + (size_t)e * qo.Tp;
                            unsigned short* c1p = c0 + (size_t)32 * qo.Tp;
                            c0[0] = __builtin_bit_cast(unsigned short, a0);
                            c0[qo.vt_plane] = __builtin_bit_cast(unsigned short, l0);
                            c1p[0] = __builtin_bit_cast(unsigned short, a1);
                            c1p[qo.vt_plane] = __builtin_bit_cast(unsigned short, l1);
                        }
                    }
                }
            }
                if (staged_q) {
                    __builtin_amdgcn_wave_barrier();
                    const int m_base = em0 + (wm * TM + 2 * ib) * 16;
#pragma unroll
                    for (int k = 0; k < 4; ++k) {
                        const int q = lane + 64 * k, row = q >> 3, cc = q & 7;
                        const u32x4 vh = *reinterpret_cast<const u32x4*>(patch_q + row * SPQ + cc * 16);
                        const u32x4 vl = *reinterpret_cast<const u32x4*>(patch_q + (32 + row) * SPQ + cc * 16);
                        if (m_base + row < M) {
                            unsigned short* dst = Ch + (size_t)(m_base + row) * (2 * Dm) + (size_t)which * Dm + hcol + cc * 8;
                            *reinterpret_cast<u32x4*>(dst) = vh;
                            *reinterpret_cast<u32x4*>(dst + c_plane) = vl;
                        }
                    }
                    __builtin_amdgcn_wave_barrier();
                }
            }
            }
        } else if constexpr (OUT == 0) {
            unsigned char* patch = patches + wave * (32 * 128);
            const int cc = lane & 7, rq = lane >> 3;
            const unsigned int kOob = 0x80000000u;
            const unsigned int ldc = xm.ldc ? (unsigned int)xm.ldc : (unsigned int)N;
            const long long cb = xm.tiles_per_batch ? (long long)(eb % xm.batch_inner) * xm.c_b0 + (long long)(eb / xm.batch_inner) * xm.c_b1 : 0;
            const __amdgpu_buffer_rsrc_t rsC = __builtin_amdgcn_make_buffer_rsrc(Cf + cb, 0, (int)((unsigned int)M * ldc * 4u), 0x00020000);
            const __amdgpu_buffer_rsrc_t rsR = __builtin_amdgcn_make_buffer_rsrc(const_cast<float*>(residual ? residual : Cf) + cb, 0, (int)((unsigned int)M * ldc * 4u), 0x00020000);
            constexpr int NB = TN / 2;
            unsigned int coff[NB];
            f32x4 bv[NB];
#pragma unroll
            for (int j = 0; j < NB; ++j) {
                const int n = en0 + wn * 64 + j * 32 + cc * 4;
                coff[j] = n < N ? (unsigned int)n * 4u : kOob;
                bv[j] = (bias && n < N) ? *reinterpret_cast<const f32x4*>(bias + n) : f32x4{0.f, 0.f, 0.f, 0.f};
            }
#pragma unroll
            for (int j = 0; j < NB; ++j) asm volatile("" :: "v"(bv[j]));
            auto c_off = [&](int m, int j) -> int {
                return (int)((m < M && coff[j] != kOob) ? (unsigned int)m * ldc * 4u + coff[j] : kOob);
            };
            u32x4 rv[2][NB][4];
            auto load_residual = [&](int i, u32x4 (&dst)[NB][4]) {
                const int m_base = em0 + (wm * TM + 2 * i) * 16;
#pragma unroll
                for (int j = 0; j < NB; ++j)
#pragma unroll
                    for (int k = 0; k < 4; ++k)
                        dst[j][k] = __builtin_bit_cast(u32x4, __builtin_amdgcn_raw_buffer_load_b128(rsR, c_off(m_base + rq + 8 * k, j), 0, 0));
            };
            if (residual) load_residual(0, rv[0]);
#pragma unroll
            for (int i = 0; i < TM / 2; ++i) {
                const int m_base = em0 + (wm * TM + 2 * i) * 16;
                if (residual && i + 1 < TM / 2) load_residual(i + 1, rv[(i + 1) & 1]);
#pragma unroll
                for (int j = 0; j < NB; ++j) {
#pragma unroll
                    for (int s = 0; s < 2; ++s)
#pragma unroll
                        for (int u = 0; u < 2; ++u) {
                            const int prow = 16 * s + r;
                            *reinterpret_cast<f32x4*>(patch + prow * 128 + (((4 * u + kq) ^ (prow & 7)) << 4)) = acc[2 * j + u][2 * i + s];
                        }
                    __builtin_amdgcn_wave_barrier();
#pragma unroll
                    for (int k = 0; k < 4; ++k) {
                        const int row = rq + 8 * k;
                        const f32x4 a = *reinterpret_cast<const f32x4*>(patch + row * 128 + ((cc ^ (row & 7)) << 4));
                        f32x4 val;
#pragma unroll
                        for (int e = 0; e < 4; ++e) val[e] = fmaf(a[e], out_scale, bv[j][e]);
                        if (EPI == EPI_GELU) val = gelu_erf16(val);
                        if (EPI == EPI_GELU_TANH) val = gelu_tanh16(val);
                        if (EPI == EPI_SQRELU)
#pragma unroll
                        for (int e = 0; e < 4; ++e) { const float t = fmaxf(val[e], 0.0f); val[e] = t * t; }
                        if (residual) {
                            const f32x4 rr = __builtin_bit_cast(f32x4, rv[i & 1][j][k]);
#pragma unroll
                            for (int e = 0; e < 4; ++e) val[e] = rr[e] + val[e];
                        }
                        __builtin_amdgcn_raw_buffer_store_b128(__builtin_bit_cast(u32x4, val), rsC, c_off(m_base + row, j), 0, 0);
                    }
                    __builtin_amdgcn_wave_barrier();
                }
            }
        } else {
            if constexpr (BF) {
                constexpr int SPB = 144;
                const bool staged = (N % 8 == 0) && (en0 + (wn + 1) * 64 <= N);
                unsigned char* patch = patches + wave * (32 * SPB);
                f32x4 bvs[TN];
#pragma unroll
                for (int j = 0; j < TN; ++j) {
                    const int n = en0 + wn * 64 + 16 * j + 4 * kq;
                    bvs[j] = (bias && n < N) ? *reinterpret_cast<const f32x4*>(bias + n) : f32x4{0.f, 0.f, 0.f, 0.f};
                }
#pragma unroll
                for (int j = 0; j < TN; ++j) asm volatile("" :: "v"(bvs[j]));
#pragma unroll
                for (int ib = 0; ib < TM / 2; ++ib) {
#pragma unroll
                    for (int s = 0; s < 2; ++s) {
                    const int i = 2 * ib + s, prow = 16 * s + r;
                    const int m = em0 + (wm * TM + i) * 16 + r;
                    if (m >= M) continue;
#pragma unroll
                    for (int j = 0; j < TN; ++j) {
                            const int n = en0 + wn * 64 + 16 * j + 4 * kq;
                            if (n >= N) continue;
                            const f32x4 bv = bvs[j];
                            f32x4 val;
#pragma unroll
                            for (int e = 0; e < 4; ++e) val[e] = fmaf(acc[j][i][e], out_scale, bv[e]);
                            if (EPI == EPI_GELU) val = gelu_erf16(val);
                            if (EPI == EPI_GELU_TANH) val = gelu_tanh16(val);
                            if (EPI == EPI_SQRELU)
#pragma unroll
                            for (int e = 0; e < 4; ++e) { const float t = fmaxf(val[e], 0.0f); val[e] = t * t; }
                            u32x2 pk;
                            pk[0] = (unsigned int)f32_to_bf16_rne(val[0]) | ((unsigned int)f32_to_bf16_rne(val[1]) << 16);
                            pk[1] = (unsigned int)f32_to_bf16_rne(val[2]) | ((unsigned int)f32_to_bf16_rne(val[3]) << 16);
                            if (staged) lds_put(patch + prow * SPB + (16 * j + 4 * kq) * 2, pk);
                            else *reinterpret_cast<u32x2*>(Ch + (size_t)m * (size_t)N + n) = pk;
                        }
                    }
                    if (staged) {
                        __builtin_amdgcn_wave_barrier();
                        const int m_base = em0 + (wm * TM + 2 * ib) * 16;
                        const size_t ncol0 = (size_t)en0 + (size_t)wn * 64;
#pragma unroll
                        for (int k = 0; k < 4; ++k) {
                            const int q = lane + 64 * k, row = q >> 3, cc = q & 7;
                            const u32x4 v = *reinterpret_cast<const u32x4*>(patch + row * SPB + cc * 16);
                            if (m_base + row < M) *reinterpret_cast<u32x4*>(Ch + (size_t)(m_base + row) * (size_t)N + ncol0 + cc * 8) = v;
                        }
                        __builtin_amdgcn_wave_barrier();
                    }
                }
            } else if constexpr (EPI == EPI_SWIGLU) {
            constexpr int SPS = 144;
            const int Nh = N >> 1, nw = en0 + wn * 64;
            if (nw < N) {
            unsigned char* patch = patches + wave * (32 * SPS);
            f32x4 bvs[TN];
#pragma unroll
            for (int j = 0; j < TN; ++j)
                bvs[j] = bias ? *reinterpret_cast<const f32x4*>(bias + nw + 16 * j + 4 * kq) : f32x4{0.f, 0.f, 0.f, 0.f};
#pragma unroll
            for (int j = 0; j < TN; ++j) asm volatile("" :: "v"(bvs[j]));
#pragma unroll
            for (int ib = 0; ib < TM / 2; ++ib) {
#pragma unroll
                for (int s = 0; s < 2; ++s) {
                    const int i = 2 * ib + s, prow = 16 * s + r;
                    if (em0 + (wm * TM + i) * 16 + r >= M) continue;
#pragma unroll
                    for (int j = 0; j < 2; ++j) {
                        f32x4 g, u;
#pragma unroll
                        for (int e = 0; e < 4; ++e) {
                            g[e] = fmaf(acc[j][i][e], out_scale, bvs[j][e]);
                            u[e] = fmaf(acc[j + 2][i][e], out_scale, bvs[j + 2][e]);
                        }
                        const f32x4 val = silu16(g) * u;
                        h4 hi, lo;
#pragma unroll
                        for (int e = 0; e < 4; ++e) {
                            _Float16 a, b;
                            split_act(val[e], a, b);
                            hi[e] = a;
                            lo[e] = b;
                        }
                        unsigned char* cell = patch + prow * SPS + (16 * j + 4 * kq) * 2;
                        lds_put(cell, hi);
                        lds_put(cell + 64, lo);
                    }
                }
                __builtin_amdgcn_wave_barrier();
                const int m_base = em0 + (wm * TM + 2 * ib) * 16;
#pragma unroll
                for (int k = 0; k < 4; ++k) {
                    const int q = lane + 64 * k, row = q >> 3, cc = q & 7;
                    const u32x4 v = *reinterpret_cast<const u32x4*>(patch + row * SPS + cc * 16);
                    if (m_base + row < M) *reinterpret_cast<u32x4*>(Ch + (size_t)(m_base + row) * (2 * (size_t)Nh) + (size_t)nw + cc * 8) = v;
                }
                __builtin_amdgcn_wave_barrier();
            }
            }
            } else {
            constexpr int SP = 272;
            const bool staged = (N % 8 == 0) && (en0 + (wn + 1) * 64 <= N);
            unsigned char* patch = patches + wave * (32 * SP);
            f32x4 bvs[TN];
#pragma unroll
            for (int j = 0; j < TN; ++j) {
                const int n = en0 + wn * 64 + 16 * j + 4 * kq;
                bvs[j] = (bias && n < N) ? *reinterpret_cast<const f32x4*>(bias + n) : f32x4{0.f, 0.f, 0.f, 0.f};
            }
#pragma unroll
            for (int j = 0; j < TN; ++j) asm volatile("" :: "v"(bvs[j]));
#pragma unroll
            for (int ib = 0; ib < TM / 2; ++ib) {
#pragma unroll
                for (int s = 0; s < 2; ++s) {
                const int i = 2 * ib + s, prow = 16 * s + r;
                const int m = em0 + (wm * TM + i) * 16 + r;
                if (m >= M) continue;
#pragma unroll
                for (int j = 0; j < TN; ++j) {
                    {
                        const int c = 16 * j + 4 * kq;
                        const int n = en0 + wn * 64 + c;
                        if (n >= N) continue;
                        const f32x4 bv = bvs[j];
                        f32x4 val;
#pragma unroll
                        for (int e = 0; e < 4; ++e) val[e] = fmaf(acc[j][i][e], out_scale, bv[e]);
                        if (EPI == EPI_GELU) val = gelu_erf16(val);
                        if (EPI == EPI_GELU_TANH) val = gelu_tanh16(val);
                        if (EPI == EPI_SQRELU)
#pragma unroll
                        for (int e = 0; e < 4; ++e) { const float t = fmaxf(val[e], 0.0f); val[e] = t * t; }
                        {
                            h4 hi, lo;
#pragma unroll
                            for (int e = 0; e < 4; ++e) {
                                _Float16 a, b;
                                split_act(val[e], a, b);
                                hi[e] = a;
                                lo[e] = b;
                            }
                            if (staged) {
                                unsigned char* cell = patch + prow * SP + (c >> 5) * 128 + (c & 31) * 2;
                                lds_put(cell, hi);
                                lds_put(cell + 64, lo);
                            } else {
                                unsigned short* dst = Ch + ki_off((size_t)m, n, N);
                                *reinterpret_cast<h4*>(dst) = hi;
                                *reinterpret_cast<h4*>(dst + 32) = lo;
                            }
                        }
                    }
                }
                }
                if (staged) {
                    __builtin_amdgcn_wave_barrier();
                    const int m_base = em0 + (wm * TM + 2 * ib) * 16;
                    const size_t ncol0 = (size_t)en0 + (size_t)wn * 64;
#pragma unroll
                    for (int k = 0; k < 8; ++k) {
                        const int q = lane + 64 * k;
                        const int row = q >> 4, cc = q & 15;
                        const u32x4 v = *reinterpret_cast<const u32x4*>(patch + row * SP + cc * 16);
                        if (m_base + row < M) {
                            if (xm.o_ld)
                                *reinterpret_cast<u32x4*>(Ch + ((size_t)(m_base + row) + (ncol0 >> 6) * (size_t)xm.o_rows_per_n64) * (2 * (size_t)xm.o_ld) +
                                                          (size_t)eb * (size_t)xm.o_col_per_batch * 2 + cc * 8) = v;
                            else
                                *reinterpret_cast<u32x4*>(Ch + (size_t)(m_base + row) * (2 * (size_t)N) + ncol0 * 2 + cc * 8) = v;
                        }
                    }
                    __builtin_amdgcn_wave_barrier();
                }
            }
            }
        }
        return more;
    };
    using Full = std::integral_constant<int, TMX>;
    using Half = std::integral_constant<int, TMX / 2>;
    while (true) {
        bool more;
        if constexpr (OUT != 2) more = half_item ? run_item(Half{}) : run_item(Full{});
        else more = run_item(Full{});
        if (!more) break;
    }
}

}
```

### proteingym_amd/csrc/gemm_f16.hip

```cpp
#include <stdio.h>
#include <stdlib.h>
#include <string.h>
#include <algorithm>
#include <mutex>
#include <type_traits>
#include <vector>

#include "common.h"
#include "gemm16x_kernel.h"

namespace pgmi {

template <int WM, int WN, int TM, int TN, int EPI, int OUT>
__global__ __launch_bounds__(WM * WN * 64, 2) void gemm_bf16_kernel(
    const unsigned short* __restrict__ A, const unsigned short* __restrict__ W, const float* __restrict__ bias,
    const float* residual, float* Cf, unsigned short* Ch, int M, int N, int K, int tiles_m, int tiles_n) {
    constexpr int BK = 32, CPR = 4;
    constexpr int NT = WM * WN * 64;
    constexpr int BM = WM * TM * 32, BN = WN * TN * 32;
    constexpr int A_CH = BM * CPR, W_CH = BN * CPR;
    constexpr int A_LD = (A_CH + NT - 1) / NT, W_LD = (W_CH + NT - 1) / NT;
    constexpr int STAGE = A_CH + W_CH;
    extern __shared__ __attribute__((aligned(16))) u32x4 lds[];

// ... 84 lines not shown
                for (int i = 0; i < TM; ++i) acc[j][i] = mfma16<true>(wf[j], af[i], acc[j][i]);
        }
        if (more) stage_store(cur ^ 1);
        __syncthreads();
        cur ^= 1;
    }
#pragma unroll
    for (int i = 0; i < TM; ++i) {
        const int m = m0 + (wm * TM + i) * 32 + r;
        if (m >= M) continue;
#pragma unroll
        for (int j = 0; j < TN; ++j) {
#pragma unroll
            for (int g = 0; g < 4; ++g) {
                const int n = n0 + (wn * TN + j) * 32 + 8 * g + 4 * kh;
                if (n >= N) continue;
                const f32x4 bv = bias ? *reinterpret_cast<const f32x4*>(bias + n) : f32x4{0.f, 0.f, 0.f, 0.f};
                f32x4 val;
#pragma unroll
                for (int e = 0; e < 4; ++e) val[e] = acc[j][i][4 * g + e] + bv[e];
                if (EPI == EPI_GELU) val = gelu_erf16(val);
                if (EPI == EPI_GELU_TANH) val = gelu_tanh16(val);
                if (EPI == EPI_SQRELU)
#pragma unroll
                        for (int e = 0; e < 4; ++e) { const float t = fmaxf(val[e], 0.0f); val[e] = t * t; }
                const size_t o = (size_t)m * N + n;
                if (residual) {
                    const f32x4 rv = *reinterpret_cast<const f32x4*>(residual + o);
#pragma unroll
                    for (int e = 0; e < 4; ++e) val[e] = rv[e] + val[e];
                }
                if constexpr (OUT == 0) {
                    *reinterpret_cast<f32x4*>(Cf + o) = val;
                } else {
                    u32x2 pk;
                    pk[0] = f32_to_bf16_rne(val[0]) | ((unsigned)f32_to_bf16_rne(val[1]) << 16);
                    pk[1] = f32_to_bf16_rne(val[2]) | ((unsigned)f32_to_bf16_rne(val[3]) << 16);
                    *reinterpret_cast<u32x2*>(Ch + o) = pk;
                }
            }
        }
    }
}

template <int WM, int WN, int TM, int TN>
static int launch_bf16_cfg(const unsigned short* A, const unsigned short* W, const float* bias, const float* residual, float* Cf,
                           unsigned short* Ch, int M, int N, int K, int epilogue, hipStream_t s) {
    constexpr int BM = WM * TM * 32, BN = WN * TN * 32;
    constexpr size_t lds_bytes = (size_t)2 * (BM + BN) * 4 * 16;
    const int tiles_m = (M + BM - 1) / BM, tiles_n = (N + BN - 1) / BN;
    const dim3 grid(tiles_m * tiles_n), block(WM * WN * 64);
#define PGMI_LAUNCH_BF16(EPI_, OUT_)                                                                     \
    do {                                                                                                 \
        auto kfn = gemm_bf16_kernel<WM, WN, TM, TN, EPI_, OUT_>;                                          \
        if (lds_bytes > 65536) {                                                                         \
            hipError_t e = hipFuncSetAttribute(reinterpret_cast<const void*>(kfn),                       \
                                               hipFuncAttributeMaxDynamicSharedMemorySize, (int)lds_bytes); \
            if (e != hipSuccess) { set_error("hipFuncSetAttribute: %s", hipGetErrorString(e)); return PGMI_EHIP; } \
        }                                                                                                \
        hipLaunchKernelGGL(kfn, grid, block, lds_bytes, s, A, W, bias, residual, Cf, Ch, M, N, K, tiles_m, tiles_n); \
    } while (0)
    const int out = Ch ? 1 : 0;
    if (epilogue == EPI_GELU) { if (out) PGMI_LAUNCH_BF16(EPI_GELU, 1); else PGMI_LAUNCH_BF16(EPI_GELU, 0); }
    else if (epilogue == EPI_SQRELU) { if (out) PGMI_LAUNCH_BF16(EPI_SQRELU, 1); else PGMI_LAUNCH_BF16(EPI_SQRELU, 0); }
    else if (epilogue == EPI_GELU_TANH) { if (out) PGMI_LAUNCH_BF16(EPI_GELU_TANH, 1); else PGMI_LAUNCH_BF16(EPI_GELU_TANH, 0); }
    else { if (out) PGMI_LAUNCH_BF16(EPI_NONE, 1); else PGMI_LAUNCH_BF16(EPI_NONE, 0); }
#undef PGMI_LAUNCH_BF16
    PGMI_HIP(hipGetLastError());
    return PGMI_OK;
}

constexpr int kMaxDevices = 64;
static int g_num_cus[kMaxDevices];
static std::mutex g_xdev_mu;

static int x_num_cus() {
    int dev = 0;
    if (hipGetDevice(&dev) != hipSuccess || dev < 0 || dev >= kMaxDevices) dev = 0;
    std::lock_guard<std::mutex> lk(g_xdev_mu);
    int& n = g_num_cus[dev];
    if (!n) {
        hipDeviceProp_t prop;
        if (hipGetDeviceProperties(&prop, dev) == hipSuccess) n = prop.multiProcessorCount;
        if (n <= 0) n = 256;
        n -= n % 8;
        if (n <= 0) n = 8;
    }
    return n;
}

constexpr int kGroupM = 4, kGroupMWide = 8, kWideTilesN = 16;
struct GemmOptions { int half_tail = 1; long long max_rows = 0; bool half_tail_set = false, max_rows_set = false; };
static GemmOptions g_opt;
void gemm_options_from_env() {
    const char* h = getenv("PGMI_GEMM_HALF_TAIL");
    const char* r = getenv("PGMI_GEMM_MAX_ROWS");
    if (!g_opt.half_tail_set) g_opt.half_tail = h ? atoi(h) : 1;
    if (!g_opt.max_rows_set) g_opt.max_rows = r ? atoll(r) : 0;
}
int gemm_set_option(const char* name, long long value) {
    if (!strcmp(name, "gemm_half_tail")) {
        g_opt.half_tail_set = value >= 0;
        if (value >= 0) g_opt.half_tail = (int)value; else gemm_options_from_env();
        return PGMI_OK;
    }
    if (!strcmp(name, "gemm_max_rows")) {
        g_opt.max_rows_set = value >= 0;
        if (value >= 0) g_opt.max_rows = value; else gemm_options_from_env();
        return PGMI_OK;
    }
    return PGMI_EINVAL;
}

struct GemmTune { int group_m = 0; };
static thread_local GemmTune g_tune;

static int launch_gemm16x_one(const unsigned short* A, const unsigned short* W,
                              const float* bias, const float* residual, float* Cf, unsigned short* Ch, size_t c_plane,
                              int M, int N, int K, int epilogue, float out_scale, hipStream_t s, const QkvOut* qkv, bool bf = false) {
    const unsigned long long eb = bf ? 2ull : 4ull;
    const GemmTune tune = g_tune;
    TilePlan tp{};
    tp.group_m = tune.group_m > 0 ? tune.group_m : ((N + XBN - 1) / XBN >= kWideTilesN ? kGroupMWide : kGroupM);
    tp.tiles_m = (M + XBM - 1) / XBM;
    tp.tiles_n = (N + XBN - 1) / XBN;
    const int T = tp.tiles_m * tp.tiles_n, G = x_num_cus();
    tp.n_main = T;
    if ((unsigned long long)std::max(M, N) * (unsigned long long)K * eb >= (1ull << 32) ||
        (Cf && (unsigned long long)M * (unsigned long long)N * 4ull >= (1ull << 31))) {
        set_error("gemm16x: operand of %d x %d split elements (or %d x %d outputs) exceeds the 32-bit offset range", std::max(M, N), K, M, N);
        return PGMI_EINVAL;
    }
    const int rem = T % G;
    const int want_half = g_opt.half_tail;
    if (want_half && !qkv && rem > 0 && 2 * rem <= G) {
        tp.n_main = T - rem; tp.half = 1; tp.n_tail = 2 * rem;
    }
    const int n_items = tp.n_main + tp.n_tail;
    const dim3 grid(std::min(G, n_items)), block(XNT);
    QkvOut qo{};
    if (qkv) qo = *qkv;
    const XMap xmap{};
#define PGMI_LAUNCH16X(EPI_, OUT_)                                                                        \
    do {                                                                                                 \
        auto kfn = bf ? gemm16x_kernel<EPI_, OUT_, false, true> : gemm16x_kernel<EPI_, OUT_>;             \
        const size_t lds_bytes = X_LDS_BYTES;                                                            \
        hipError_t e = hipFuncSetAttribute(reinterpret_cast<const void*>(kfn),                           \
                                           hipFuncAttributeMaxDynamicSharedMemorySize, (int)lds_bytes);  \
        if (e != hipSuccess) { set_error("hipFuncSetAttribute: %s", hipGetErrorString(e)); return PGMI_EHIP; } \
        hipLaunchKernelGGL(kfn, grid, block, lds_bytes, s, A, W, bias, residual, Cf, Ch, c_plane, M, N, K,  \
                           out_scale, tp, qo, xmap);                                                     \
    } while (0)
#define PGMI_LAUNCH16X_O(EPI_) do { if (Ch) PGMI_LAUNCH16X(EPI_, 1); else PGMI_LAUNCH16X(EPI_, 0); } while (0)
    if (qkv) PGMI_LAUNCH16X(EPI_NONE, 2);
    else if (epilogue == EPI_SWIGLU) {
        const auto kfn = gemm16x_kernel<EPI_SWIGLU, 1>;
        hipError_t e = hipFuncSetAttribute(reinterpret_cast<const void*>(kfn), hipFuncAttributeMaxDynamicSharedMemorySize, (int)X_LDS_BYTES);
        if (e != hipSuccess) { set_error("hipFuncSetAttribute: %s", hipGetErrorString(e)); return PGMI_EHIP; }
        hipLaunchKernelGGL(kfn, grid, block, X_LDS_BYTES, s, A, W, bias, residual, Cf, Ch, c_plane, M, N, K, out_scale, tp, qo, xmap);
    }
    else if (epilogue == EPI_GELU) PGMI_LAUNCH16X_O(EPI_GELU);
    else if (epilogue == EPI_SQRELU) PGMI_LAUNCH16X_O(EPI_SQRELU);
    else if (epilogue == EPI_GELU_TANH) PGMI_LAUNCH16X_O(EPI_GELU_TANH);
    else PGMI_LAUNCH16X_O(EPI_NONE);
#undef PGMI_LAUNCH16X_O
#undef PGMI_LAUNCH16X
    PGMI_HIP(hipGetLastError());
    return PGMI_OK;
}

int launch_gemm16_ex(const unsigned short* A, const unsigned short* W, float* Cf, unsigned short* Ch, int M, int N, int K,
                     float out_scale, XMap xm, int nbatch, hipStream_t s) {
    if (M <= 0 || N <= 0 || K <= 0 || (K % 64) != 0 || (N % 4) != 0 || (!Cf && !Ch) || (Cf && Ch) || nbatch < 1 ||
        (Ch && (N % 64) != 0) || (xm.a_run_bytes && (K / 32) % (1 << xm.k_run_log2) != 0)) {
        set_error("gemm16_ex: unsupported shape/args M=%d N=%d K=%d batches=%d", M, N, K, nbatch);
        return PGMI_EINVAL;
    }
    TilePlan tp{};
    tp.group_m = kGroupM;
    const int rows_last = M % XBM;
    const bool all_half = rows_last > 0 && rows_last <= XBM / 2;
    tp.tiles_m = all_half ? (M + XBM / 2 - 1) / (XBM / 2) : (M + XBM - 1) / XBM;
    tp.tiles_n = (N + XBN - 1) / XBN;
    const int per = tp.tiles_m * tp.tiles_n, T = per * nbatch, G = x_num_cus();
    xm.tiles_per_batch = per;
    if (xm.batch_inner < 1) xm.batch_inner = 1;
    if (all_half) { tp.half = 2; tp.n_main = 0; tp.n_tail = T; } else { tp.n_main = T; }
    const dim3 grid(std::min(G, T)), block(XNT);
    QkvOut qo{};
    const float* nobias = nullptr;
    const size_t lds_bytes = X_LDS_BYTES;
#define PGMI_LAUNCH16X_EX(OUT_)                                                                           \
    do {                                                                                                 \
        auto kfn = gemm16x_kernel<EPI_NONE, OUT_, true>;                                                  \
        hipError_t e = hipFuncSetAttribute(reinterpret_cast<const void*>(kfn),                           \
                                           hipFuncAttributeMaxDynamicSharedMemorySize, (int)lds_bytes);  \
        if (e != hipSuccess) { set_error("hipFuncSetAttribute: %s", hipGetErrorString(e)); return PGMI_EHIP; } \
        hipLaunchKernelGGL(kfn, grid, block, lds_bytes, s, A, W, nobias, nobias, Cf, Ch, (size_t)0, M, N, K,  \
                           out_scale, tp, qo, xm);                                                       \
    } while (0)
    if (Ch) PGMI_LAUNCH16X_EX(1); else PGMI_LAUNCH16X_EX(0);
#undef PGMI_LAUNCH16X_EX
    PGMI_HIP(hipGetLastError());
    return PGMI_OK;
}

static int launch_gemm16x(const unsigned short* A, const unsigned short* W,
                          const float* bias, const float* residual, float* Cf, unsigned short* Ch, size_t c_plane,
                          int M, int N, int K, int epilogue, float out_scale, hipStream_t s, const QkvOut* qkv = nullptr, bool bf = false) {
    const unsigned long long lim = (1ull << 32) - 1;
    const unsigned long long eb = bf ? 2ull : 4ull;
    if ((unsigned long long)N * (unsigned long long)K * eb > lim) {
        set_error("gemm16x: weight of %d x %d split elements exceeds the 32-bit offset range", N, K);
        return PGMI_EINVAL;
    }
    const long long test_rows = g_opt.max_rows;
    long long max_rows = (long long)(lim / ((unsigned long long)K * eb));
    if (Cf) max_rows = std::min(max_rows, (long long)(((1ull << 31) - 1) / ((unsigned long long)N * 4ull)));
    if (test_rows > 0) max_rows = std::min(max_rows, test_rows);
    if (M <= max_rows) return launch_gemm16x_one(A, W, bias, residual, Cf, Ch, c_plane, M, N, K, epilogue, out_scale, s, qkv, bf);
    long long per = qkv ? (max_rows / qkv->T) * qkv->T : (max_rows / XBM) * XBM;
    if (per <= 0) per = qkv ? 0 : max_rows;
    if (per <= 0) { set_error("gemm16x: one sequence of %d tokens x K = %d exceeds the 32-bit offset range", qkv->T, K); return PGMI_EINVAL; }
    for (long long m0 = 0; m0 < M; m0 += per) {
        const int mc = (int)std::min<long long>(per, M - m0);
        const unsigned short* Ac = A + (size_t)m0 * (size_t)K * (bf ? 1 : 2);
        int rc;
        if (qkv) {
            QkvOut q = *qkv;
            q.vt16 = qkv->vt16 + (size_t)(m0 / qkv->T) * (size_t)qkv->H * kHeadDim * (size_t)qkv->Tp;
            rc = launch_gemm16x_one(Ac, W, bias, nullptr, nullptr, Ch + (size_t)m0 * (size_t)(2 * (N / 3)), c_plane, mc, N, K, epilogue,
                                    out_scale, s, &q, bf);
        } else {
            const size_t n_out = epilogue == EPI_SWIGLU ? (size_t)N / 2 : (size_t)N;
            rc = launch_gemm16x_one(Ac, W, bias, residual ? residual + (size_t)m0 * N : nullptr, Cf ? Cf + (size_t)m0 * N : nullptr,
                                    Ch ? Ch + (size_t)m0 * (size_t)(bf ? 1 : 2) * n_out : nullptr, c_plane, mc, N, K, epilogue, out_scale, s, nullptr, bf);
        }
        if (rc) return rc;
    }
    return PGMI_OK;
}

static void set_tune(int variant) {
    g_tune = GemmTune{};
    if (variant >= 1000) {
        const int t = variant - 1000;
        g_tune.group_m = t & 15;
    }
}

int launch_gemm16(const unsigned short* A, size_t a_plane, const unsigned short* W, size_t w_plane,
                  const float* bias, const float* residual, float* Cf, unsigned short* Ch, size_t c_plane,
                  int M, int N, int K, int epilogue, float out_scale, int planes, bool bf, int variant,
                  hipStream_t s) {
    (void)a_plane; (void)w_plane;
    const int k_step = (planes == 2 && !bf) ? 32 : 64;
    if (M <= 0 || N <= 0 || K <= 0 || (K % k_step) != 0 || (N % 4) != 0 || (!Cf && !Ch) || (Cf && Ch)) {
        set_error("gemm16: unsupported shape/args M=%d N=%d K=%d (K %% %d == 0, N %% 4 == 0 required)", M, N, K, k_step);
        return PGMI_EINVAL;
    }
    if (epilogue == EPI_SWIGLU && (planes != 2 || bf || !Ch || residual || (N % 64) != 0)) {
        set_error("gemm16: the SwiGLU epilogue is f16x3 with split-plane output, no residual and N %% 64 == 0 (N = %d)", N);
        return PGMI_EINVAL;
    }
    if (planes == 2 && !bf) {
        if (Ch && (N % 32) != 0) { set_error("gemm16: split output needs N %% 32 == 0 (K-interleaved operand of the next GEMM), got %d", N); return PGMI_EINVAL; }
        set_tune(variant);
        const int rc = launch_gemm16x(A, W, bias, residual, Cf, Ch, c_plane, M, N, K, epilogue, out_scale, s);
        g_tune = GemmTune{};
        return rc;
    }
    if (planes == 1 && bf) {
        if (out_scale != 1.0f) { set_error("gemm16: bf16 weights are not pre-scaled"); return PGMI_EINVAL; }
        if (Ch && (N % 4) != 0) { set_error("gemm16: bf16 plane output needs N %% 4 == 0, got %d", N); return PGMI_EINVAL; }
        if (variant != 2000) {
            set_tune(variant);
            const int rc = launch_gemm16x(A, W, bias, residual, Cf, Ch, c_plane, M, N, K, epilogue, 1.0f, s, nullptr, true);
            g_tune = GemmTune{};
            return rc;
        }
        if ((long long)M * N >= 1 << 22) return launch_bf16_cfg<2, 4, 4, 2>(A, W, bias, residual, Cf, Ch, M, N, K, epilogue, s);
        return launch_bf16_cfg<2, 2, 2, 2>(A, W, bias, residual, Cf, Ch, M, N, K, epilogue, s);
    }
    set_error("gemm16: unsupported mode planes=%d bf=%d", planes, (int)bf);
    return PGMI_EINVAL;
}

int launch_gemm16_qkv(const unsigned short* A, size_t a_plane, const unsigned short* W, size_t w_plane,
                      const float* bias, int M, int D, int K, float out_scale, unsigned short* qk16, size_t qk_plane,
                      unsigned short* vt16, size_t vt_plane, const float* cos_t, const float* sin_t, int rotary,
                      int T, int H, int variant, hipStream_t s, int rot_halves, bool bf) {
    (void)a_plane; (void)w_plane;
    if (M <= 0 || D <= 0 || (K % (bf ? 64 : 32)) || (D % 64) || M % T || rot_halves < 1) {
        set_error("gemm16_qkv: unsupported shape M=%d D=%d K=%d T=%d", M, D, K, T);
        return PGMI_EINVAL;
    }
    QkvOut qo{vt16, vt_plane, cos_t, sin_t, T, H, (T + 31) / 32 * 32, rotary, rot_halves};
    set_tune(variant);
    const int rc = launch_gemm16x(A, W, bias, nullptr, nullptr, qk16, qk_plane, M, 3 * D, K, EPI_NONE, out_scale, s, &qo, bf);
    g_tune = GemmTune{};
    return rc;
}

__global__ void split16_kernel(const float* __restrict__ x, int64_t n, float scale, int mode, int K,
                               unsigned short* __restrict__ out) {
    const int64_t i = (int64_t)blockIdx.x * blockDim.x + threadIdx.x;
    if (i >= n) return;
    const float v = x[i] * scale;
    if (mode == 1) {
        out[i] = f32_to_bf16_rne(v);
        return;
    }
    _Float16 hi, lo;
    if (mode == 2) {
        split_act(v, hi, lo);
    } else {
        hi = (_Float16)v;
        lo = (_Float16)(v - (float)hi);
    }
    const size_t o = ki_off((size_t)(i / K), (int)(i % K), K);
    out[o] = __builtin_bit_cast(unsigned short, hi);
    out[o + 32] = __builtin_bit_cast(unsigned short, lo);
}
void launch_split16(const float* x, int64_t n, float scale, int mode, int K, unsigned short* out, hipStream_t s) {
    hipLaunchKernelGGL(split16_kernel, dim3((unsigned)((n + 255) / 256)), dim3(256), 0, s, x, n, scale, mode, K, out);
}

}
```

### proteingym_amd/csrc/model.h

```cpp
#pragma once
#include <math.h>
#include <stdlib.h>
#include <cmath>
#include <algorithm>
#include <stdarg.h>
#include <stdio.h>
#include <string.h>

#include <string>
#include <vector>

#include "common.h"
#include "gemm16x_kernel.h"

namespace pgmi {

struct W16 {
    unsigned short* p = nullptr;
    size_t plane = 0;
    float out_scale = 1.0f;
};

struct Layer {
    float *ln1_w, *ln1_b, *wqkv, *bqkv, *wo, *bo, *ln2_w, *ln2_b, *w1, *b1, *w2, *b2;
    W16 wqkv16, wo16, w116, w216;
    float* conv = nullptr;
    float *c_ln_w = nullptr, *c_ln_b = nullptr, *c_bqkv = nullptr, *c_bo = nullptr;
    W16 c_wqkv16, c_wo16;
    float *q_ln = nullptr, *k_ln = nullptr;
};

struct ProfEvent {
    hipEvent_t start, stop;
    int cls;
};

}

using namespace pgmi;

struct pgmi_assay;
struct pgmi_pppl;

struct pgmi_model {
    pgmi_config cfg;
    int device = 0;
    hipStream_t stream = nullptr;
    std::vector<void*> allocs;
    std::vector<pgmi_assay*> assays;
    std::vector<pgmi_pppl*> pppls;
    float *embed_tokens = nullptr, *embed_positions = nullptr;
    float *lnb_w = nullptr, *lnb_b = nullptr, *lna_w = nullptr, *lna_b = nullptr;
    float *hd_w = nullptr, *hd_b = nullptr, *hln_w = nullptr, *hln_b = nullptr;
    float *head_w = nullptr, *head_b = nullptr;
    std::vector<Layer> layers;
    W16 hd16;
    int fc1_epi = EPI_GELU, fc1_cols = 0;
    bool embed_gather = false;
    float* slopes = nullptr;
    float* tr_prior = nullptr;
    size_t tr_prior_cap = 0;
    int32_t* tr_meta = nullptr;
    size_t tr_meta_cap = 0;
    int pg2_rotary = 0;
    float *pg2_aa_w = nullptr, *pg2_aa_b = nullptr;
    int gpt_Vp = 0, gpt_head_rows = 0;
    bool parallel_residual = false;
    float* gpt_logits = nullptr;
    W16 gpt_head16;
    double* gpt_sum = nullptr;
    float* msa_pe = nullptr;
    float* xt = nullptr;
    int32_t *msa_full = nullptr, *msa_kv_len = nullptr;
    size_t msa_full_cap = 0;
    float *tied_part = nullptr, *tied_p = nullptr, *tied_vt = nullptr;
    size_t tied_part_cap = 0, tied_p_cap = 0, tied_vt_cap = 0;
    int msa_kv_R = 0, msa_kv_C = 0;
    float ln_eps = 1e-5f;
    unsigned short *h16 = nullptr, *g16 = nullptr;
    size_t h16_plane = 0, g16_plane = 0;
    unsigned short *qk16 = nullptr, *vt16 = nullptr;
    size_t qk16_plane = 0, vt16_plane = 0;
    int32_t* nonfinite = nullptr;
    int gemm_variant = 0;
    int keep_rows = 1;
    int last_B = 0, last_T = 0;
    int dh = kHeadDim;
    int rot_halves = 1;
    int Hs = 0;
    int Da = 0;
    float *rot_cos = nullptr, *rot_sin = nullptr;
    int rot_len = 0;
    float* zeros = nullptr;
    int max_rows = 0;
    float *x = nullptr, *h = nullptr, *qkv = nullptr, *g = nullptr, *lp = nullptr, *denom = nullptr;
    int32_t *tokens = nullptr, *pos_idx = nullptr, *kv_len = nullptr, *row_idx = nullptr, *aux_i = nullptr;
    bool prof = false;
    std::vector<ProfEvent> events;
    size_t events_used = 0;
    double prof_ms[PGMI_K_COUNT] = {0};
    int64_t prof_n[PGMI_K_COUNT] = {0};
    double prof_flops[PGMI_K_COUNT] = {0};
    double prof_bytes[PGMI_K_COUNT] = {0};
};

struct pgmi_assay {
    pgmi_model* m = nullptr;
    int n_tok = 0, P = 0, T = 0;
    int64_t n_mut = 0, n_sub = 0;
    std::vector<void*> allocs;
    int32_t *wt = nullptr, *positions = nullptr, *win_start = nullptr, *mask_rel = nullptr;
    int32_t *sub_pos = nullptr, *sub_wt = nullptr, *sub_mt = nullptr;
    int64_t* mut_off = nullptr;
    float* table = nullptr;
    double* scores = nullptr;
};

struct pgmi_pppl {
    pgmi_model* m = nullptr;
    int64_t N = 0;
    std::vector<int64_t> off;
    std::vector<void*> allocs;
    uint8_t* tok8 = nullptr;
    int64_t* off_dev = nullptr;
    int64_t last_rows = 0, last_chunks = 0, last_tokens = 0, last_padded = 0;
};

namespace pgmi {

template <typename T>
int dev_alloc(std::vector<void*>& pool, T** p, size_t n) {
    void* q = nullptr;
    if (n == 0) n = 1;
    hipError_t e = hipMalloc(&q, n * sizeof(T));
    if (e != hipSuccess) {
        set_error("hipMalloc(%zu bytes) failed: %s", n * sizeof(T), hipGetErrorString(e));
        return PGMI_ENOMEM;
    }
    pool.push_back(q);
    *p = static_cast<T*>(q);
    return PGMI_OK;
}

template <typename T>
int dev_upload(std::vector<void*>& pool, T** p, const T* host, size_t n) {
    int rc = dev_alloc(pool, p, n);
    if (rc) return rc;
    if (n) PGMI_HIP(hipMemcpy(*p, host, n * sizeof(T), hipMemcpyHostToDevice));
    return PGMI_OK;
}

struct ProfScope {
    pgmi_model* m;
    ProfEvent* ev = nullptr;
    ProfScope(pgmi_model* m_, int cls, double flops, double bytes) : m(m_) {
        if (!m->prof) return;
        if (m->events_used == m->events.size()) {
            ProfEvent e;
            if (hipEventCreate(&e.start) != hipSuccess || hipEventCreate(&e.stop) != hipSuccess) return;
            m->events.push_back(e);
        }
        ev = &m->events[m->events_used++];
        ev->cls = cls;
        m->prof_n[cls] += 1;
        m->prof_flops[cls] += flops;
        m->prof_bytes[cls] += bytes;
        hipEventRecord(ev->start, m->stream);
    }
    ~ProfScope() {
        if (ev) hipEventRecord(ev->stop, m->stream);
    }
};

template <typename T>
int ensure_cap(pgmi_model* m, T** p, size_t* cap, size_t need) {
    if (need <= *cap) return PGMI_OK;
    T* q = nullptr;
    int rc = dev_alloc(m->allocs, &q, need);
    if (rc) return rc;
    *p = q;
    *cap = need;
    return PGMI_OK;
}

int prof_drain(pgmi_model* m);
int check_cfg(const pgmi_config* c);
int check_tokens(const int32_t* tokens, int B, int T);
int check_vocab(const int32_t* tokens, int B, int T, int V);
int env_int(const char* name, int dflt);
int make_w16(std::vector<void*>& pool, const float* host, size_t n, size_t K, int precision, hipStream_t s, W16* out);
int linear(pgmi_model* m, const float* in32, const unsigned short* in16, size_t in_plane, const float* W32,
           const W16& w16, const float* bias, const float* residual, float* out32, unsigned short* out16,
           size_t out_plane, int M, int N, int K, int epi);
int check_nonfinite(pgmi_model* m);
int reset_pad_keys(pgmi_model* m, int B, int T);
int model_create(const pgmi_config* cfg, const float* w, int64_t n_weights, int device, pgmi_model** out, int arch_arg);
int create_esm(pgmi_model* m, const pgmi_config* cfg, const float* w, int64_t n_weights);
int ensure_rotary(pgmi_model* m, int T);
int upload_rotate_half(pgmi_model* m, int n);
int run_encoder(pgmi_model* m, int B, int T, const int32_t* keep = nullptr, int n_keep = 0, bool* compacted = nullptr);
int run_head(pgmi_model* m, int R, const int32_t* row_idx);
int run_rows(pgmi_model* m, int B, int T, int R, const int32_t* row_idx);
int create_tranception(pgmi_model* m, const pgmi_config* cfg, const float* w, int64_t n_weights);
int create_progen2(pgmi_model* m, const pgmi_config* cfg, const float* w, int64_t n_weights, int rotary_dim);
int create_gpt(pgmi_model* m, const pgmi_config* cfg, const float* w, int64_t n_weights, int pos_kind);
int64_t gpt_weight_count(const pgmi_config* c, int pos_kind);
int decoder_check(pgmi_model* m, int arch, int T);
int run_decoder(pgmi_model* m, int B, int T, const AttRagged* rg = nullptr, int rows = 0, double att_flops = 0);
int narrow_head(pgmi_model* m, int M);
int decoder_token_logprobs(pgmi_model* m, int arch, const int32_t* tokens, int B, int T, float* out);
int64_t esmc_weight_count(const pgmi_config* c);
int create_esmc(pgmi_model* m, const pgmi_config* cfg, const float* w, int64_t n_weights);
int create_msa(pgmi_model* m, const pgmi_config* cfg, const float* w, int64_t n_weights);
int run_msa(pgmi_model* m, int R, int C, int keep_col = -1, bool* compacted = nullptr);

struct BlobCursor {
    pgmi_model* m;
    const float *p, *end;
    int rc = PGMI_OK;
    BlobCursor(pgmi_model* m_, const float* w, int64_t n_weights) : m(m_), p(w), end(w + n_weights) {}
    const float* take(size_t n) { p += n; return p - n; }
    void upload(float** dst, const float* host, size_t n) { if (!rc) rc = dev_upload(m->allocs, dst, host, n); }
    void upload(float** dst, size_t n) { upload(dst, take(n), n); }
    void w16(W16* dst, const float* host, size_t n, size_t K) { if (!rc) rc = make_w16(m->allocs, host, n, K, m->cfg.precision, m->stream, dst); }
    void w16(W16* dst, size_t n, size_t K) { w16(dst, take(n), n, K); }
    void linear(float** w32, W16* w16_, const float* host, size_t n, size_t K) {
        if (m->cfg.precision == PGMI_PREC_FP32) upload(w32, host, n); else w16(w16_, host, n, K);
    }
    void linear(float** w32, W16* w16_, size_t n, size_t K) { linear(w32, w16_, take(n), n, K); }
    int finish() {
        if (!rc && p != end) { set_error("internal: blob walk mismatch"); rc = PGMI_EINVAL; }
        return rc;
    }
};

inline size_t rotate_half_slot(size_t col, size_t dh) {
    const size_t h = col / dh, j = col % dh;
    if (dh > 64) return (2 * h + ((j >> 5) & 1)) * 64 + ((j >> 6) << 5) + (j & 31);
    return h * 64 + (j < dh / 2 ? j : 32 + (j - dh / 2));
}

template <typename Slot>
void pack_qkv_slots(const float* src, size_t D, size_t Da, Slot slot, float qscale, float* wq, float* bq = nullptr) {
    for (size_t k = 0; k < 3; ++k) {
        const float sc = (k == 0) ? qscale : 1.0f;
        for (size_t o = 0; o < D; ++o) {
            float* dst = &wq[(k * Da + slot(o)) * D];
            for (size_t i = 0; i < D; ++i) dst[i] = src[o * D + i] * sc;
        }
        src += D * D;
        if (!bq) continue;
        for (size_t o = 0; o < D; ++o) bq[k * Da + slot(o)] = src[o] * sc;
        src += D;
    }
}

template <typename Slot>
void pack_out_cols(const float* src, size_t D, size_t Da, Slot slot, float* wo) {
    for (size_t o = 0; o < D; ++o)
        for (size_t i = 0; i < D; ++i) wo[o * Da + slot(i)] = src[o * D + i];
}

template <typename Angle>
int upload_rotary(pgmi_model* m, int n, int groups, Angle angle) {
    std::vector<float> c((size_t)n * groups * 64), s((size_t)n * groups * 64);
    for (int t = 0; t < n; ++t)
        for (int g = 0; g < groups; ++g)
            for (int i = 0; i < 32; ++i) {
                const float f = angle(t, g, i);
                const size_t o = ((size_t)t * groups + g) * 64;
                c[o + i] = c[o + 32 + i] = cosf(f);
                s[o + i] = s[o + 32 + i] = sinf(f);
            }
    int rc = dev_upload(m->allocs, &m->rot_cos, c.data(), c.size());
    if (!rc) rc = dev_upload(m->allocs, &m->rot_sin, s.data(), s.size());
    if (!rc) m->rot_len = n;
    return rc;
}

inline int rows_per_chunk(const pgmi_model* m, int T) { return std::max(1, m->max_rows / ((T + 31) / 32 * 32)); }

template <typename Fn>
int for_each_chunk(pgmi_model* m, int B, int T, Fn fn) {
    const int per = rows_per_chunk(m, T);
    for (int b0 = 0; b0 < B; b0 += per) {
        int rc = fn(b0, std::min(per, B - b0));
        if (rc) return rc;
        PGMI_HIP(hipStreamSynchronize(m->stream));
    }
    return PGMI_OK;
}

}
```

Before: 17980.

## Compute layer-0 QKV on two distinct rows and last-layer queries only for kept rows

In masked-marginal batches every sequence is the same wild-type window with one position masked. Layer 0 therefore runs embed, layernorm and the QKV GEMM on only 2*T distinct rows (the unmasked and fully masked versions) and expands them into per-sequence Q/K/V with a new gather kernel. In the last layer, Q is computed only for the kept (masked) rows through a row-mapped GEMM variant, and attention runs only for those query rows. This removes most of the layer-0 QKV work and two thirds of the last-layer query and attention work, at the cost of extra expand kernels, a new GEMM epilogue path and several correctness preconditions (for example no mask token already in the wild type).

Result: no change. 18030 (median of 6 runs) (+0.3%).

```diff
diff --git a/proteingym_amd/csrc/api_esm.hip b/proteingym_amd/csrc/api_esm.hip
--- a/proteingym_amd/csrc/api_esm.hip
+++ b/proteingym_amd/csrc/api_esm.hip
@@ -59,7 +59,33 @@
     });
 }
 
-int run_encoder(pgmi_model* m, int B, int T, const int32_t* keep, int n_keep, bool* compacted) {
+static int layer0_distinct_rows(pgmi_model* m, int B, int T, const MaskedBatch* mb) {
+    const pgmi_config& c = m->cfg;
+    const Layer& L = m->layers[0];
+    const int D = c.embed_dim, Da = m->Da, Mc = 2 * T, Tp = (T + 31) / 32 * 32, prec = c.precision;
+    hipStream_t s = m->stream;
+    const size_t x_b = (size_t)Mc * D * 4, h_plane = (size_t)Mc * D, qk_plane = (size_t)Mc * 2 * Da, vt_plane = (size_t)2 * Da * Tp;
+    int rc = ensure_cap(m, &m->dw, &m->dw_cap, x_b + 4 * h_plane + 4 * qk_plane + 4 * vt_plane + (size_t)Mc * 4);
+    if (rc) return rc;
+    float* x = reinterpret_cast<float*>(m->dw);
+    unsigned short* h16 = reinterpret_cast<unsigned short*>(m->dw + x_b);
+    unsigned short* qk = h16 + 2 * h_plane;
+    unsigned short* vt = qk + 2 * qk_plane;
+    int32_t* tok = reinterpret_cast<int32_t*>(vt + 2 * vt_plane);
+    { ProfScope p(m, PGMI_K_EMBED, 0, (double)Mc * D * 4);
+      launch_window_and_mask_rows(mb->window, T, tok, s);
+      launch_embed(tok, m->denom, m->pos_idx, m->embed_tokens, m->embed_positions, c.token_dropout, Mc, T, D, x, s);
+      if (m->lnb_w) launch_layernorm(x, m->lnb_w, m->lnb_b, Mc, D, 1e-5f, x, s); }
+    { ProfScope p(m, PGMI_K_LAYERNORM, 0, 2.0 * Mc * D * 4);
+      launch_layernorm16(x, L.ln1_w, L.ln1_b, Mc, D, 1e-5f, h16, h_plane, prec == PGMI_PREC_F16X3 ? 1 : 2, s); }
+    ProfScope p(m, PGMI_K_GEMM_QKV, 2.0 * Mc * 3 * D * D, 4.0 * B * T * 3 * Da);
+    rc = launch_gemm16_qkv(h16, h_plane, L.wqkv16.p, L.wqkv16.plane, L.bqkv, Mc, Da, D, L.wqkv16.out_scale, qk, qk_plane, vt, vt_plane,
+                           m->rot_cos, m->rot_sin, c.arch == PGMI_ARCH_ESM2, T, m->Hs, m->gemm_variant, s, m->rot_halves, prec == PGMI_PREC_BF16);
+    if (rc) return rc;
+    return launch_expand_window(qk, qk_plane, vt, vt_plane, mb->mask_rel, B, T, m->Hs, m->qk16, m->qk16_plane, m->vt16, m->vt16_plane, s);
+}
+
+int run_encoder(pgmi_model* m, int B, int T, const int32_t* keep, int n_keep, bool* compacted, const MaskedBatch* mb) {
     const pgmi_config& c = m->cfg;
     const int M = B * T, D = c.embed_dim, F = c.ffn_dim, N1 = m->fc1_cols, H = c.heads, Da = m->Da;
     hipStream_t s = m->stream;
@@ -85,18 +111,33 @@
     const int mode16 = (prec == PGMI_PREC_F16X3) ? 1 : 2;
     for (int l = 0; l < c.layers; ++l) {
         const Layer& L = m->layers[l];
+        const bool fused_qkv = prec != PGMI_PREC_FP32 && !L.q_ln;
+        const bool last_kept = keep && m->keep_rows && l == c.layers - 1;
+        const bool distinct = l == 0 && mb && mb->window && m->distinct_rows && fused_qkv && !m->embed_gather && B >= 3;
+        const bool kept_q = last_kept && mb && m->kept_queries && fused_qkv && n_keep == B;
+        if (distinct) {
+            if ((rc = layer0_distinct_rows(m, B, T, mb))) return rc;
+        } else {
         { ProfScope p(m, PGMI_K_LAYERNORM, 0, ln_bytes);
           if (prec == PGMI_PREC_FP32) launch_layernorm(m->x, L.ln1_w, L.ln1_b, M, D, 1e-5f, m->h, s);
           else launch_layernorm16(m->x, L.ln1_w, L.ln1_b, M, D, 1e-5f, m->h16, m->h16_plane, mode16, s); }
-        const bool fused_qkv = prec != PGMI_PREC_FP32 && !L.q_ln;
-        { ProfScope p(m, PGMI_K_GEMM_QKV, 2.0 * M * 3 * D * D, 0);
-          if (fused_qkv)
+        { ProfScope p(m, PGMI_K_GEMM_QKV, 2.0 * M * (kept_q ? 2 : 3) * D * D, 0);
+          if (kept_q) {
+              launch_gather_rows(reinterpret_cast<const float*>(m->h16), keep, n_keep, prec == PGMI_PREC_F16X3 ? D : D / 2,
+                                 reinterpret_cast<float*>(m->g16), s);
+              for (int part = QKV_KV; part <= QKV_Q && !rc; ++part)
+                  rc = launch_gemm16_qkv(part == QKV_Q ? m->g16 : m->h16, 0, L.wqkv16.p, L.wqkv16.plane, L.bqkv, part == QKV_Q ? n_keep : M, Da, D,
+                                         L.wqkv16.out_scale, m->qk16, m->qk16_plane, m->vt16, m->vt16_plane, m->rot_cos, m->rot_sin,
+                                         c.arch == PGMI_ARCH_ESM2, T, m->Hs, m->gemm_variant, s, m->rot_halves, prec == PGMI_PREC_BF16, part,
+                                         part == QKV_Q ? keep : nullptr);
+          } else if (fused_qkv)
               rc = launch_gemm16_qkv(m->h16, m->h16_plane, L.wqkv16.p, L.wqkv16.plane, L.bqkv, M, Da, D, L.wqkv16.out_scale,
                                      m->qk16, m->qk16_plane, m->vt16, m->vt16_plane, m->rot_cos, m->rot_sin,
                                      c.arch == PGMI_ARCH_ESM2, T, m->Hs, m->gemm_variant, s, m->rot_halves, prec == PGMI_PREC_BF16);
           else
               rc = linear(m, m->h, m->h16, m->h16_plane, L.wqkv, L.wqkv16, L.bqkv, nullptr, m->qkv, nullptr, 0, M, 3 * Da, D, EPI_NONE);
           if (rc) return rc; }
+        }
         { ProfScope p(m, PGMI_K_ATTENTION, 4.0 * M * T * D, L.q_ln ? (double)M * D * 20 : 0);
           if (L.q_ln && (rc = launch_qkln_prep(m->qkv, L.q_ln, L.k_ln, 1e-5f, m->rot_cos, m->rot_sin, B, T, H, m->qk16, m->qk16_plane,
                                                m->vt16, m->vt16_plane, s)))
@@ -106,16 +147,16 @@
           if (prec == PGMI_PREC_F16X3)
               rc = launch_attention_f16x3_v2(nullptr, m->kv_len, m->rot_cos, m->rot_sin, c.arch == PGMI_ARCH_ESM2, B, T, H,
                                              m->qk16, m->qk16_plane, m->vt16, m->vt16_plane, nullptr, m->h16,
-                                             m->h16_plane, 1, s, nullptr, nullptr, m->rot_halves * kHeadDim);
+                                             m->h16_plane, 1, s, nullptr, nullptr, m->rot_halves * kHeadDim, kept_q ? keep : nullptr);
           else if (v2)
               rc = launch_attention_f16x3_v2(nullptr, m->kv_len, m->rot_cos, m->rot_sin, c.arch == PGMI_ARCH_ESM2, B, T, H,
                                              m->qk16, m->qk16_plane, m->vt16, m->vt16_plane, nullptr, m->h16, m->h16_plane, 2, s, nullptr, nullptr,
-                                             m->rot_halves * kHeadDim);
+                                             m->rot_halves * kHeadDim, kept_q ? keep : nullptr);
           else
               rc = launch_attention_f32(m->qkv, m->kv_len, B, T, H, m->h, m->h16, m->h16_plane,
                                         prec == PGMI_PREC_FP32 ? 0 : mode16, s, m->rot_halves * kHeadDim);
           if (rc) return rc; }
-        if (keep && m->keep_rows && l == c.layers - 1) {
+        if (last_kept) {
             const int R = n_keep;
             ProfScope p(m, PGMI_K_KEPT_ROWS, 2.0 * R * D * (Da + N1 + F), 0);
             launch_gather_rows(m->x, keep, R, D, m->qkv, s);
@@ -177,9 +218,9 @@
 }
 
 
-int run_rows(pgmi_model* m, int B, int T, int R, const int32_t* row_idx) {
+int run_rows(pgmi_model* m, int B, int T, int R, const int32_t* row_idx, const MaskedBatch* mb) {
     bool compacted = false;
-    int rc = run_encoder(m, B, T, row_idx, R, &compacted);
+    int rc = run_encoder(m, B, T, row_idx, R, &compacted, mb);
     if (rc) return rc;
     return run_head(m, R, compacted ? nullptr : row_idx);
 }
@@ -223,7 +264,8 @@
         PGMI_HIP(hipMemcpyAsync(m->aux_i, mask_pos + b0, (size_t)bc * 4, hipMemcpyHostToDevice, m->stream));
         PGMI_HIP(hipMemcpyAsync(m->row_idx, ridx.data(), (size_t)bc * 4, hipMemcpyHostToDevice, m->stream));
         launch_apply_mask(m->tokens, m->aux_i, bc, T, m->stream);
-        int rc = run_rows(m, bc, T, bc, m->row_idx);
+        const MaskedBatch mb{m->aux_i, nullptr};
+        int rc = run_rows(m, bc, T, bc, m->row_idx, &mb);
         if (rc) return rc;
         PGMI_HIP(hipMemcpyAsync(out + (size_t)b0 * V, m->lp, (size_t)bc * V * 4, hipMemcpyDeviceToHost, m->stream));
         return PGMI_OK;
@@ -243,6 +285,7 @@
     const int T = std::min(n_tok, window);
     if (T > m->max_rows) { set_error("T=%d exceeds workspace rows %d", T, m->max_rows); return PGMI_EINVAL; }
     std::vector<int32_t> ws(P), mr(P);
+    const bool wt_has_mask = std::find(wt_tokens, wt_tokens + n_tok, (int32_t)PGMI_TOK_MASK) != wt_tokens + n_tok;
     for (int i = 0; i < P; ++i) {
         if (positions[i] < 0 || positions[i] >= n_tok) { set_error("position %d out of range", positions[i]); return PGMI_EINVAL; }
         int s, e;
@@ -260,6 +303,7 @@
     PGMI_HIP(hipSetDevice(m->device));
     pgmi_assay* a = new pgmi_assay();
     a->m = m; a->n_tok = n_tok; a->P = P; a->T = T; a->n_mut = n_mut; a->n_sub = n_sub;
+    a->win_start_host = ws; a->wt_has_mask = wt_has_mask;
     int rc = dev_upload(a->allocs, &a->wt, wt_tokens, (size_t)n_tok);
     if (!rc) rc = dev_upload(a->allocs, &a->positions, positions, (size_t)P);
     if (!rc) rc = dev_upload(a->allocs, &a->win_start, ws.data(), (size_t)P);
@@ -299,7 +343,10 @@
         const int bc = std::min(per, a->P - p0);
         launch_make_masked_windows(a->wt, a->win_start + p0, a->mask_rel + p0, bc, T, m->tokens, s);
         launch_row_index(a->mask_rel + p0, bc, T, m->row_idx, s);
-        int rc = run_rows(m, bc, T, bc, m->row_idx);
+        const int32_t* w0 = a->win_start_host.data() + p0;
+        const bool one_window = !a->wt_has_mask && std::all_of(w0, w0 + bc, [&](int32_t v) { return v == w0[0]; });
+        const MaskedBatch mb{a->mask_rel + p0, one_window ? a->wt + w0[0] : nullptr};
+        int rc = run_rows(m, bc, T, bc, m->row_idx, &mb);
         if (rc) return rc;
         launch_scatter_rows(m->lp, a->positions + p0, bc, V, a->table, s);
     }
diff --git a/proteingym_amd/csrc/api_model.hip b/proteingym_amd/csrc/api_model.hip
--- a/proteingym_amd/csrc/api_model.hip
+++ b/proteingym_amd/csrc/api_model.hip
@@ -297,6 +297,8 @@
     if (!rc) rc = alloc_workspace(m);
     if (rc) { pgmi_model_destroy(m); return rc; }
     m->keep_rows = env_int("PGMI_KEEP_ROWS", 1);
+    m->distinct_rows = env_int("PGMI_DISTINCT_ROWS", 1);
+    m->kept_queries = env_int("PGMI_KEPT_QUERIES", 1);
     gemm_options_from_env();
     m->gemm_variant = env_int("PGMI_GEMM_VARIANT", 0);
     *out = m;
diff --git a/proteingym_amd/csrc/attention_f16.hip b/proteingym_amd/csrc/attention_f16.hip
--- a/proteingym_amd/csrc/attention_f16.hip
+++ b/proteingym_amd/csrc/attention_f16.hip
@@ -384,7 +384,7 @@
 int launch_attention_f16x3_v2(const float* qkv, const int32_t* kv_len, const float* cos_t, const float* sin_t,
                               int rotary, int B, int T, int H, unsigned short* qk16, size_t qk_plane,
                               unsigned short* vt16, size_t vt_plane, float* ctx, unsigned short* ctx16, size_t plane,
-                              int out_mode, hipStream_t s, const float* conv, const float* slopes, int head_dim) {
+                              int out_mode, hipStream_t s, const float* conv, const float* slopes, int head_dim, const int32_t* q_rows) {
     if (B <= 0 || T <= 0 || H <= 0 || out_mode < 0 || out_mode > 2 || (head_dim != 64 && head_dim != 128 && head_dim != 256)) {
         set_error("attention_f16x3_v2: bad arguments B=%d T=%d H=%d out=%d head_dim=%d", B, T, H, out_mode, head_dim);
         return PGMI_EINVAL;
@@ -427,10 +427,11 @@
         launch_qkv_prep_conv(dim3(n32, H, B), s, qkv, conv, T, H, Tp, qk16, qk_plane, vt16, vt_plane, nullptr);
     else if (qkv)
         launch_qkv_prep(dim3(n32, H, B), s, qkv, cos_t, sin_t, rotary, T, H, Tp, qk16, qk_plane, vt16, vt_plane);
-    const int wpb = att16_waves_per_block(T), nblk = (n32 + wpb - 1) / wpb;
+    const bool v3 = att_v3_serves(T, conv, slopes, head_dim);
+    const int wpb = att16_waves_per_block(T), nblk = (v3 && q_rows) ? 1 : (n32 + wpb - 1) / wpb;
     int dn = 0;
     const dim3 grid = dense_grid(nblk, H, B, &dn);
-    if (att_v3_serves(T, conv, slopes, head_dim)) rc = launch_att16v3(out_mode, wpb, grid, qk16, qk_plane, vt16, vt_plane, kv_len, T, H, Tp, ctx, ctx16, s, dn, B);
+    if (v3) rc = launch_att16v3(out_mode, wpb, grid, qk16, qk_plane, vt16, vt_plane, kv_len, T, H, Tp, ctx, ctx16, s, dn, B, q_rows);
     else if (out_mode == 0) rc = launch_att16v2_mode<0, 3>(wpb, grid, qk16, qk_plane, vt16, vt_plane, kv_len, slopes, T, H, Tp, ctx, ctx16, plane, s, dn, B);
     else if (out_mode == 2) rc = launch_att16v2_mode<3, 3>(wpb, grid, qk16, qk_plane, vt16, vt_plane, kv_len, slopes, T, H, Tp, ctx, ctx16, plane, s, dn, B);
     else rc = launch_att16v2_mode<1, 3>(wpb, grid, qk16, qk_plane, vt16, vt_plane, kv_len, slopes, T, H, Tp, ctx, ctx16, plane, s, dn, B);
diff --git a/proteingym_amd/csrc/attention_f16_common.h b/proteingym_amd/csrc/attention_f16_common.h
--- a/proteingym_amd/csrc/attention_f16_common.h
+++ b/proteingym_amd/csrc/attention_f16_common.h
@@ -73,6 +73,7 @@
 bool att_v3_serves(int T, const float* conv, const float* slopes, int head_dim);
 void att_v3_set_option(int value);
 int launch_att16v3(int out_mode, int wpb, dim3 grid, const unsigned short* qk16, size_t qk_plane, const unsigned short* vt16, size_t vt_plane,
-                   const int32_t* kv_len, int T, int H, int Tp, float* ctx, unsigned short* ctx16, hipStream_t s, int dense_nblk, int nseq);
+                   const int32_t* kv_len, int T, int H, int Tp, float* ctx, unsigned short* ctx16, hipStream_t s, int dense_nblk, int nseq,
+                   const int32_t* q_rows = nullptr);
 
 }
diff --git a/proteingym_amd/csrc/attention_f16_prep.hip b/proteingym_amd/csrc/attention_f16_prep.hip
--- a/proteingym_amd/csrc/attention_f16_prep.hip
+++ b/proteingym_amd/csrc/attention_f16_prep.hip
@@ -290,6 +290,57 @@
     return PGMI_OK;
 }
 
+__global__ __launch_bounds__(256) void expand_window_qk_kernel(const u32x4* __restrict__ src, size_t src_plane, u32x4* __restrict__ dst,
+                                                              size_t dst_plane, const int32_t* __restrict__ mask_rel, int T, int row_ch) {
+    const int row = blockIdx.x, b = row / T, t = row - b * T;
+    const u32x4* s = src + (size_t)(t == mask_rel[b] ? T + t : t) * row_ch;
+    u32x4* d = dst + (size_t)row * row_ch;
+    for (int i = threadIdx.x; i < 2 * row_ch; i += 256) {
+        const int p = i >= row_ch, c = i - p * row_ch;
+        d[p * dst_plane + c] = s[p * src_plane + c];
+    }
+}
+__global__ __launch_bounds__(256) void expand_window_vt_kernel(const unsigned short* __restrict__ src, size_t src_plane,
+                                                              unsigned short* __restrict__ dst, size_t dst_plane,
+                                                              const int32_t* __restrict__ mask_rel, int T, int Tp, int HD) {
+    const int b = blockIdx.y, nch = Tp >> 3;
+    const int i = blockIdx.x * 256 + threadIdx.x;
+    if (i >= HD * nch) return;
+    const int hd = i / nch, c = i - hd * nch;
+    const int tm = mask_rel[b], tk = tm & 31;
+    const int pm = (tm & ~31) + ((tk & 0x13) | ((tk & 4) << 1) | ((tk & 8) >> 1));
+    const size_t so = (size_t)hd * Tp + 8 * c, seq1 = (size_t)HD * Tp;
+#pragma unroll
+    for (int p = 0; p < 2; ++p) {
+        union { u32x4 v; unsigned short h[8]; } u;
+        u.v = *reinterpret_cast<const u32x4*>(src + p * src_plane + so);
+        if ((pm >> 3) == c) u.h[pm & 7] = src[p * src_plane + seq1 + so + (pm & 7)];
+        if (8 * c + 8 > (T & ~31) && (T & 31)) {
+#pragma unroll
+            for (int e = 0; e < 8; ++e) {
+                const int pos = 8 * c + e, k = pos & 31;
+                if ((pos & ~31) + ((k & 0x13) | ((k & 4) << 1) | ((k & 8) >> 1)) >= T) u.h[e] = 0;
+            }
+        }
+        *reinterpret_cast<u32x4*>(dst + p * dst_plane + ((size_t)b * HD + hd) * Tp + 8 * c) = u.v;
+    }
+}
+int launch_expand_window(const unsigned short* src_qk, size_t src_qk_plane, const unsigned short* src_vt, size_t src_vt_plane,
+                         const int32_t* mask_rel, int B, int T, int H, unsigned short* qk16, size_t qk_plane, unsigned short* vt16,
+                         size_t vt_plane, hipStream_t s) {
+    const int Tp = (T + 31) / 32 * 32, HD = H * kHeadDim, row_ch = 2 * HD / 8;
+    if (B <= 0 || T <= 0 || H <= 0 || (src_qk_plane | qk_plane | src_vt_plane | vt_plane) % 8) {
+        set_error("expand_window: bad arguments B=%d T=%d H=%d", B, T, H);
+        return PGMI_EINVAL;
+    }
+    hipLaunchKernelGGL(expand_window_qk_kernel, dim3((unsigned)(B * T)), dim3(256), 0, s, reinterpret_cast<const u32x4*>(src_qk), src_qk_plane / 8,
+                       reinterpret_cast<u32x4*>(qk16), qk_plane / 8, mask_rel, T, row_ch);
+    hipLaunchKernelGGL(expand_window_vt_kernel, dim3((unsigned)((HD * (Tp / 8) + 255) / 256), (unsigned)B), dim3(256), 0, s, src_vt, src_vt_plane,
+                       vt16, vt_plane, mask_rel, T, Tp, HD);
+    PGMI_HIP(hipGetLastError());
+    return PGMI_OK;
+}
+
 void launch_qkv_prep(dim3 grid, hipStream_t s, const float* qkv, const float* cos_t, const float* sin_t, int rotary, int T, int H, int Tp,
                      unsigned short* qk16, size_t qk_plane, unsigned short* vt16, size_t vt_plane) {
     hipLaunchKernelGGL(qkv_prep_kernel, grid, dim3(256), 0, s, qkv, cos_t, sin_t, rotary, T, H, Tp, qk16, qk_plane, vt16, vt_plane);
diff --git a/proteingym_amd/csrc/attention_f16_v3.hip b/proteingym_amd/csrc/attention_f16_v3.hip
--- a/proteingym_amd/csrc/attention_f16_v3.hip
+++ b/proteingym_amd/csrc/attention_f16_v3.hip
@@ -10,7 +10,7 @@
 __global__ __launch_bounds__(WPB * 64, 2) void attention_f16x3_v3_kernel(
     const unsigned short* __restrict__ qk16, size_t qk_plane, const unsigned short* __restrict__ vt16, size_t vt_plane,
     const int32_t* __restrict__ kv_len, int T, int H, int Tp, float* __restrict__ ctx, unsigned short* __restrict__ ctx16,
-    int dense_nblk, int nseq) {
+    int dense_nblk, int nseq, const int32_t* __restrict__ q_rows) {
     constexpr float defer_thr = kAttDefer;
     constexpr int DH = 64, NSTG = 3, KCPR = 8, KCH = AKT * KCPR, VCH = DH * 4, STG_CH = 2 * KCH + 2 * VCH;
     constexpr int NWI = STG_CH / 64, NDMA = (NWI + WPB - 1) / WPB, NS = 4, ND = 2;
@@ -33,8 +33,10 @@
     const int r = lane & 31, kh = lane >> 5;
     const int D = H * DH;
     const int Tk = kv_len ? kv_len[b] : T;
+    const int q_keep = q_rows ? q_rows[b] - b * T : 0;
+    if (q_rows) qblk = q_keep / (32 * WPB);
     const int q0 = (qblk * WPB + wave) * 32;
-    const bool active = q0 < T;
+    const bool active = q0 < T && (!q_rows || (q_keep >> 5) == qblk * WPB + wave);
     const int nkt = (Tk + AKT - 1) / AKT;
     const size_t seq_halfs = (size_t)T * (2 * D), vt_halfs = (size_t)DH * Tp;
     const unsigned long long qk_bytes = std::min<unsigned long long>(0xFFFFFFFFull, (unsigned long long)qk_plane * 2ull + seq_halfs * 2ull);
@@ -409,20 +411,21 @@
 
 template <int WPB, int OUT>
 static void launch_att16v3_one(dim3 grid, const unsigned short* qk16, size_t qk_plane, const unsigned short* vt16, size_t vt_plane, const int32_t* kv_len,
-                               int T, int H, int Tp, float* ctx, unsigned short* ctx16, hipStream_t s, int dense_nblk, int nseq) {
+                               int T, int H, int Tp, float* ctx, unsigned short* ctx16, hipStream_t s, int dense_nblk, int nseq, const int32_t* q_rows) {
     constexpr size_t lds_bytes = (size_t)3 * A_STAGE * 16;
     auto kfn = attention_f16x3_v3_kernel<WPB, OUT>;
     if (lds_bytes > 65536) (void)hipFuncSetAttribute(reinterpret_cast<const void*>(kfn), hipFuncAttributeMaxDynamicSharedMemorySize, (int)lds_bytes);
     hipLaunchKernelGGL((attention_f16x3_v3_kernel<WPB, OUT>), grid, dim3(WPB * 64), lds_bytes, s, qk16, qk_plane, vt16, vt_plane, kv_len, T, H, Tp, ctx, ctx16,
-                       dense_nblk, nseq);
+                       dense_nblk, nseq, q_rows);
 }
 int launch_att16v3(int out_mode, int wpb, dim3 grid, const unsigned short* qk16, size_t qk_plane, const unsigned short* vt16, size_t vt_plane,
-                          const int32_t* kv_len, int T, int H, int Tp, float* ctx, unsigned short* ctx16, hipStream_t s, int dense_nblk, int nseq) {
+                          const int32_t* kv_len, int T, int H, int Tp, float* ctx, unsigned short* ctx16, hipStream_t s, int dense_nblk, int nseq,
+                          const int32_t* q_rows) {
 #define PGMI_V3(W)                                                                                                                          \
     do {                                                                                                                                    \
-        if (out_mode == 2) launch_att16v3_one<W, 3>(grid, qk16, qk_plane, vt16, vt_plane, kv_len, T, H, Tp, ctx, ctx16, s, dense_nblk, nseq); \
-        else if (out_mode) launch_att16v3_one<W, 1>(grid, qk16, qk_plane, vt16, vt_plane, kv_len, T, H, Tp, ctx, ctx16, s, dense_nblk, nseq);   \
-        else launch_att16v3_one<W, 0>(grid, qk16, qk_plane, vt16, vt_plane, kv_len, T, H, Tp, ctx, ctx16, s, dense_nblk, nseq);            \
+        if (out_mode == 2) launch_att16v3_one<W, 3>(grid, qk16, qk_plane, vt16, vt_plane, kv_len, T, H, Tp, ctx, ctx16, s, dense_nblk, nseq, q_rows); \
+        else if (out_mode) launch_att16v3_one<W, 1>(grid, qk16, qk_plane, vt16, vt_plane, kv_len, T, H, Tp, ctx, ctx16, s, dense_nblk, nseq, q_rows);   \
+        else launch_att16v3_one<W, 0>(grid, qk16, qk_plane, vt16, vt_plane, kv_len, T, H, Tp, ctx, ctx16, s, dense_nblk, nseq, q_rows);            \
     } while (0)
     switch (wpb) {
         case 1: PGMI_V3(1); break;
diff --git a/proteingym_amd/csrc/common.h b/proteingym_amd/csrc/common.h
--- a/proteingym_amd/csrc/common.h
+++ b/proteingym_amd/csrc/common.h
@@ -46,6 +46,7 @@
 void launch_apply_mask(int32_t* tokens, const int32_t* mask_pos, int B, int T, hipStream_t s);
 void launch_seq_stats(const int32_t* tokens, int B, int T, int token_dropout, float* scale,
                       int32_t* pos_idx, int32_t* kv_len, hipStream_t s);
+void launch_window_and_mask_rows(const int32_t* window, int T, int32_t* out, hipStream_t s);
 void launch_zero_pad_rows(const int32_t* tokens, int rows, int D, float* x, hipStream_t s);
 void launch_embed(const int32_t* tokens, const float* scale, const int32_t* pos_idx,
                   const float* embed_tokens, const float* embed_positions, int token_dropout,
@@ -100,10 +101,12 @@
                   const float* bias, const float* residual, float* Cf, unsigned short* Ch, size_t c_plane,
                   int M, int N, int K, int epilogue, float out_scale, int planes, bool bf, int variant,
                   hipStream_t s);
+enum QkvPart { QKV_ALL = 0, QKV_KV = 1, QKV_Q = 2 };
 int launch_gemm16_qkv(const unsigned short* A, size_t a_plane, const unsigned short* W, size_t w_plane,
                       const float* bias, int M, int D, int K, float out_scale, unsigned short* qk16, size_t qk_plane,
                       unsigned short* vt16, size_t vt_plane, const float* cos_t, const float* sin_t, int rotary,
-                      int T, int H, int variant, hipStream_t s, int rot_halves = 1, bool bf = false);
+                      int T, int H, int variant, hipStream_t s, int rot_halves = 1, bool bf = false, int part = QKV_ALL,
+                      const int32_t* row_map = nullptr);
 struct XMap;
 int launch_gemm16_ex(const unsigned short* A, const unsigned short* W, float* Cf, unsigned short* Ch, int M, int N, int K,
                      float out_scale, XMap xm, int nbatch, hipStream_t s);
@@ -119,7 +122,12 @@
                               int rotary, int B, int T, int H, unsigned short* qk16, size_t qk_plane,
                               unsigned short* vt16, size_t vt_plane, float* ctx, unsigned short* ctx16, size_t plane,
                               int out_mode, hipStream_t s, const float* conv = nullptr, const float* slopes = nullptr,
-                              int head_dim = 64);
+                              int head_dim = 64,
+                              const int32_t* q_rows = nullptr);
+
+int launch_expand_window(const unsigned short* src_qk, size_t src_qk_plane, const unsigned short* src_vt, size_t src_vt_plane,
+                         const int32_t* mask_rel, int B, int T, int H, unsigned short* qk16, size_t qk_plane, unsigned short* vt16,
+                         size_t vt_plane, hipStream_t s);
 
 struct AttRagged {
     const int32_t* seq_off;
diff --git a/proteingym_amd/csrc/elementwise.hip b/proteingym_amd/csrc/elementwise.hip
--- a/proteingym_amd/csrc/elementwise.hip
+++ b/proteingym_amd/csrc/elementwise.hip
@@ -37,6 +37,14 @@
     const int64_t n = (int64_t)B * T;
     hipLaunchKernelGGL(make_masked_windows_kernel, dim3((unsigned)((n + 255) / 256)), dim3(256), 0, s,
                        wt, win_start, mask_rel, B, T, out);
+}
+
+__global__ void window_and_mask_rows_kernel(const int32_t* __restrict__ window, int T, int32_t* __restrict__ out) {
+    const int i = blockIdx.x * blockDim.x + threadIdx.x;
+    if (i < 2 * T) out[i] = i < T ? window[i] : PGMI_TOK_MASK;
+}
+void launch_window_and_mask_rows(const int32_t* window, int T, int32_t* out, hipStream_t s) {
+    hipLaunchKernelGGL(window_and_mask_rows_kernel, dim3((2 * T + 255) / 256), dim3(256), 0, s, window, T, out);
 }
 
 __global__ void apply_mask_kernel(int32_t* tokens, const int32_t* __restrict__ mask_pos, int B, int T) {
diff --git a/proteingym_amd/csrc/gemm16x_kernel.h b/proteingym_amd/csrc/gemm16x_kernel.h
--- a/proteingym_amd/csrc/gemm16x_kernel.h
+++ b/proteingym_amd/csrc/gemm16x_kernel.h
@@ -51,6 +51,9 @@
     const float* sin_t;
     int T, H, Tp, rotary;
     int rot_halves;
+    int Dm;
+    int col0;
+    const int* row_map;
 };
 
 template <bool BF>
@@ -310,11 +313,12 @@
             issue_tile(0, 0);
         }
 
-        if constexpr (OUT == 2) {
-            const int Dm = N / 3;
+        if constexpr (OUT == 2 || OUT == 3) {
+            constexpr bool RMAP = OUT == 3;
+            const int Dm = qo.Dm;
             const int nb = en0 + wn * 64;
             if (nb < N) {
-            const int which = nb / Dm, hcol = nb - which * Dm, hh = hcol >> 6;
+            const int which = (nb + qo.col0) / Dm, hcol = nb + qo.col0 - which * Dm, hh = hcol >> 6;
             constexpr int SPQ = 144;
             unsigned char* patch_q = patches + wave * (2 * 32 * SPQ);
             const bool staged_q = which < 2;
@@ -334,7 +338,9 @@
                 const int m = em0 + (wm * TM + i) * 16 + r;
                 const bool row_ok = m < M;
                 if (!row_ok) continue;
-                const int bb = m / qo.T, t = m - bb * qo.T;
+                int mt = m;
+                if constexpr (RMAP) mt = qo.row_map[m];
+                const int bb = mt / qo.T, t = mt - bb * qo.T;
                 f32x4 rc[2], rs[2];
                 if (which < 2 && qo.rotary) {
                     const int tr = (min(t, qo.T - 1) * qo.rot_halves + (hh % qo.rot_halves)) * 64;
@@ -409,7 +415,9 @@
                         const u32x4 vh = *reinterpret_cast<const u32x4*>(patch_q + row * SPQ + cc * 16);
                         const u32x4 vl = *reinterpret_cast<const u32x4*>(patch_q + (32 + row) * SPQ + cc * 16);
                         if (m_base + row < M) {
-                            unsigned short* dst = Ch + (size_t)(m_base + row) * (2 * Dm) + (size_t)which * Dm + hcol + cc * 8;
+                            int mo = m_base + row;
+                            if constexpr (RMAP) mo = qo.row_map[mo];
+                            unsigned short* dst = Ch + (size_t)mo * (2 * Dm) + (size_t)which * Dm + hcol + cc * 8;
                             *reinterpret_cast<u32x4*>(dst) = vh;
                             *reinterpret_cast<u32x4*>(dst + c_plane) = vl;
                         }
@@ -673,7 +681,7 @@
     using Half = std::integral_constant<int, TMX / 2>;
     while (true) {
         bool more;
-        if constexpr (OUT != 2) more = half_item ? run_item(Half{}) : run_item(Full{});
+        if constexpr (OUT < 2) more = half_item ? run_item(Half{}) : run_item(Full{});
         else more = run_item(Full{});
         if (!more) break;
     }
diff --git a/proteingym_amd/csrc/gemm_f16.hip b/proteingym_amd/csrc/gemm_f16.hip
--- a/proteingym_amd/csrc/gemm_f16.hip
+++ b/proteingym_amd/csrc/gemm_f16.hip
@@ -260,7 +260,8 @@
                            out_scale, tp, qo, xmap);                                                     \
     } while (0)
 #define PGMI_LAUNCH16X_O(EPI_) do { if (Ch) PGMI_LAUNCH16X(EPI_, 1); else PGMI_LAUNCH16X(EPI_, 0); } while (0)
-    if (qkv) PGMI_LAUNCH16X(EPI_NONE, 2);
+    if (qkv && qkv->row_map) PGMI_LAUNCH16X(EPI_NONE, 3);
+    else if (qkv) PGMI_LAUNCH16X(EPI_NONE, 2);
     else if (epilogue == EPI_SWIGLU) {
         const auto kfn = gemm16x_kernel<EPI_SWIGLU, 1>;
         hipError_t e = hipFuncSetAttribute(reinterpret_cast<const void*>(kfn), hipFuncAttributeMaxDynamicSharedMemorySize, (int)X_LDS_BYTES);
@@ -327,6 +328,7 @@
     if (Cf) max_rows = std::min(max_rows, (long long)(((1ull << 31) - 1) / ((unsigned long long)N * 4ull)));
     if (test_rows > 0) max_rows = std::min(max_rows, test_rows);
     if (M <= max_rows) return launch_gemm16x_one(A, W, bias, residual, Cf, Ch, c_plane, M, N, K, epilogue, out_scale, s, qkv, bf);
+    if (qkv && qkv->row_map) { set_error("gemm16x: a row-mapped QKV launch of %d rows does not fit one launch", M); return PGMI_EINVAL; }
     long long per = qkv ? (max_rows / qkv->T) * qkv->T : (max_rows / XBM) * XBM;
     if (per <= 0) per = qkv ? 0 : max_rows;
     if (per <= 0) { set_error("gemm16x: one sequence of %d tokens x K = %d exceeds the 32-bit offset range", qkv->T, K); return PGMI_EINVAL; }
@@ -337,7 +339,7 @@
         if (qkv) {
             QkvOut q = *qkv;
             q.vt16 = qkv->vt16 + (size_t)(m0 / qkv->T) * (size_t)qkv->H * kHeadDim * (size_t)qkv->Tp;
-            rc = launch_gemm16x_one(Ac, W, bias, nullptr, nullptr, Ch + (size_t)m0 * (size_t)(2 * (N / 3)), c_plane, mc, N, K, epilogue,
+            rc = launch_gemm16x_one(Ac, W, bias, nullptr, nullptr, Ch + (size_t)m0 * (size_t)(2 * qkv->Dm), c_plane, mc, N, K, epilogue,
                                     out_scale, s, &q, bf);
         } else {
             const size_t n_out = epilogue == EPI_SWIGLU ? (size_t)N / 2 : (size_t)N;
@@ -397,15 +399,17 @@
 int launch_gemm16_qkv(const unsigned short* A, size_t a_plane, const unsigned short* W, size_t w_plane,
                       const float* bias, int M, int D, int K, float out_scale, unsigned short* qk16, size_t qk_plane,
                       unsigned short* vt16, size_t vt_plane, const float* cos_t, const float* sin_t, int rotary,
-                      int T, int H, int variant, hipStream_t s, int rot_halves, bool bf) {
+                      int T, int H, int variant, hipStream_t s, int rot_halves, bool bf, int part, const int32_t* row_map) {
     (void)a_plane; (void)w_plane;
-    if (M <= 0 || D <= 0 || (K % (bf ? 64 : 32)) || (D % 64) || M % T || rot_halves < 1) {
-        set_error("gemm16_qkv: unsupported shape M=%d D=%d K=%d T=%d", M, D, K, T);
-        return PGMI_EINVAL;
-    }
-    QkvOut qo{vt16, vt_plane, cos_t, sin_t, T, H, (T + 31) / 32 * 32, rotary, rot_halves};
+    if (M <= 0 || D <= 0 || (K % (bf ? 64 : 32)) || (D % 64) || (!row_map && M % T) || rot_halves < 1 || (row_map && part != QKV_Q)) {
+        set_error("gemm16_qkv: unsupported shape M=%d D=%d K=%d T=%d part=%d", M, D, K, T, part);
+        return PGMI_EINVAL;
+    }
+    const int col0 = part == QKV_KV ? D : 0, N = part == QKV_ALL ? 3 * D : part == QKV_KV ? 2 * D : D;
+    QkvOut qo{vt16, vt_plane, cos_t, sin_t, T, H, (T + 31) / 32 * 32, rotary, rot_halves, D, col0, row_map};
     set_tune(variant);
-    const int rc = launch_gemm16x(A, W, bias, nullptr, nullptr, qk16, qk_plane, M, 3 * D, K, EPI_NONE, out_scale, s, &qo, bf);
+    const int rc = launch_gemm16x(A, W + (size_t)col0 * (size_t)K * (bf ? 1 : 2), bias + col0, nullptr, nullptr, qk16, qk_plane, M, N, K, EPI_NONE,
+                                  out_scale, s, &qo, bf);
     g_tune = GemmTune{};
     return rc;
 }
diff --git a/proteingym_amd/csrc/model.h b/proteingym_amd/csrc/model.h
--- a/proteingym_amd/csrc/model.h
+++ b/proteingym_amd/csrc/model.h
@@ -84,6 +84,9 @@
     int32_t* nonfinite = nullptr;
     int gemm_variant = 0;
     int keep_rows = 1;
+    int distinct_rows = 1, kept_queries = 1;
+    unsigned char* dw = nullptr;
+    size_t dw_cap = 0;
     int last_B = 0, last_T = 0;
     int dh = kHeadDim;
     int rot_halves = 1;
@@ -110,6 +113,8 @@
     int64_t n_mut = 0, n_sub = 0;
     std::vector<void*> allocs;
     int32_t *wt = nullptr, *positions = nullptr, *win_start = nullptr, *mask_rel = nullptr;
+    std::vector<int32_t> win_start_host;
+    bool wt_has_mask = false;
     int32_t *sub_pos = nullptr, *sub_wt = nullptr, *sub_mt = nullptr;
     int64_t* mut_off = nullptr;
     float* table = nullptr;
@@ -198,9 +203,14 @@
 int create_esm(pgmi_model* m, const pgmi_config* cfg, const float* w, int64_t n_weights);
 int ensure_rotary(pgmi_model* m, int T);
 int upload_rotate_half(pgmi_model* m, int n);
-int run_encoder(pgmi_model* m, int B, int T, const int32_t* keep = nullptr, int n_keep = 0, bool* compacted = nullptr);
+struct MaskedBatch {
+    const int32_t* mask_rel;
+    const int32_t* window;
+};
+int run_encoder(pgmi_model* m, int B, int T, const int32_t* keep = nullptr, int n_keep = 0, bool* compacted = nullptr,
+                const MaskedBatch* mb = nullptr);
 int run_head(pgmi_model* m, int R, const int32_t* row_idx);
-int run_rows(pgmi_model* m, int B, int T, int R, const int32_t* row_idx);
+int run_rows(pgmi_model* m, int B, int T, int R, const int32_t* row_idx, const MaskedBatch* mb = nullptr);
 int create_tranception(pgmi_model* m, const pgmi_config* cfg, const float* w, int64_t n_weights);
 int create_progen2(pgmi_model* m, const pgmi_config* cfg, const float* w, int64_t n_weights, int rotary_dim);
 int create_gpt(pgmi_model* m, const pgmi_config* cfg, const float* w, int64_t n_weights, int pos_kind);
```
